# davidea97/Fisher-Nerf-customized

Hardware: AMD Instinct MI355X
Metric: candidate-views/sec (higher is better)
Workload: dtype f32

## Files before the change

### fisher-nerf-customized_amd/csrc/fisher_rast.hip

```cpp
#include <hip/hip_runtime.h>
#include <hip/hip_fp16.h>
#include <stdint.h>
#include <stdio.h>
#include <stdlib.h>
#include <string.h>
#include "fr_math.h"
#include "../../include/fisher_rast.h"
#include "fr_internal.h"

#define FR_THREADS 256
#define FR_G_MAX 32
#define FR_MAX_LDS_TILES 4096
#define FR_PART_MIN_DEFAULT 2048
#define FR_SORT_SMALL_KEYS 2048
#define FR_SORT_MID_KEYS 4096
#define FR_SORT_BIG_KEYS 16384
#define FR_VC_MAX 16
#define FR_BATCH 256
#define FR_BWD_BATCH 128

#include <vector>
#include <utility>
static thread_local char g_err[512] = "";
#if defined(FR_ABLATE) || defined(FR_LOOPSTATS)
// ... 374 lines not shown

__global__ __launch_bounds__(FR_THREADS) void k_tile_lists(const uint32_t* __restrict__ cnt, uint32_t* __restrict__ off, int N, int T, uint32_t tile_cap,
                                                           int* __restrict__ status, uint32_t* __restrict__ big_list,
                                                           uint32_t* __restrict__ view_work, uint32_t* __restrict__ view_perm, int ablate, uint32_t list_min)
{
	const int i0 = (blockIdx.x * FR_THREADS + threadIdx.x) * 4;
	__shared__ uint32_t s_vw[4 * FR_THREADS + 2];
	const int vfirst = (blockIdx.x * 4 * FR_THREADS) / T;
	const int ilast = min(N - 1, (int)(blockIdx.x * 4 * FR_THREADS) + 4 * FR_THREADS - 1);
	const int nvb = view_work ? ilast / T - vfirst + 1 : 0;
	for (int k = threadIdx.x; k < nvb; k += FR_THREADS) s_vw[k] = 0u;
	__syncthreads();
	uint32_t sum = 0, mx = 0;
#pragma unroll
	for (int q = 0; q < 4; q++)
	{
		const int i = i0 + q;
		if (i >= N) break;
		const uint32_t c = cnt[i];
		off[i] = (uint32_t)i * tile_cap;
		sum += c;
		mx = c > mx ? c : mx;
		if (c > list_min) big_list[16 + atomicAdd(&big_list[0], 1u)] = (uint32_t)i;
		if (view_work && c) atomicAdd(&s_vw[i / T - vfirst], c);
	}
	__syncthreads();
	for (int k = threadIdx.x; k < nvb; k += FR_THREADS) if (s_vw[k]) atomicAdd(&view_work[vfirst + k], s_vw[k]);
#pragma unroll
	for (int o = 32; o > 0; o >>= 1)
	{
		sum += (uint32_t)__shfl_xor((int)sum, o, 64);
		const uint32_t t = (uint32_t)__shfl_xor((int)mx, o, 64);
		mx = t > mx ? t : mx;
	}
	if ((threadIdx.x & 63) == 0)
	{
		if (sum) atomicAdd(&status[0], (int)sum);
		if (mx) atomicMax(&status[2], (int)mx);
		if (mx > tile_cap) { atomicOr(&status[1], 1); atomicOr(&status[3], 1); }
		FR_ABL(if (ablate >= 30) atomicOr(&status[1], 1);)
	}
	if (view_perm)
	{
		__shared__ bool s_last;
		__threadfence();
		__syncthreads();
		if (threadIdx.x == 0) s_last = atomicAdd(&big_list[1], 1u) == gridDim.x - 1;
		__syncthreads();
		if (s_last)
		{
			__threadfence();
			fr_deal_views((const uint32_t*)view_work, view_perm, N / T, threadIdx.x, FR_THREADS);
		}
	}
}

__global__ __launch_bounds__(FR_THREADS) void k_scatter_keys(FrParams p)
{
	extern __shared__ uint32_t fr_dyn_lds[];
	uint32_t* s_cnt = fr_dyn_lds;
	uint32_t* s_base = fr_dyn_lds + p.T;
	if (p.status[1]) return;
	const int tid = threadIdx.x;
	const int v = blockIdx.y;
	const size_t vP = (size_t)v * p.P;
	const uint32_t* off = p.tile_off + (size_t)v * p.T;
	uint32_t* fill = p.tile_fill + (size_t)v * p.T;
	const bool lds = p.T <= FR_MAX_LDS_TILES;
	if (lds && p.blk_base)
	{
		const uint32_t* bb = p.blk_base + ((size_t)v * gridDim.x + blockIdx.x) * p.T;
		for (int t = tid; t < p.T; t += FR_THREADS) { s_cnt[t] = 0; s_base[t] = off[t] + bb[t]; }
		__syncthreads();
	}
	else if (lds)
	{
		for (int t = tid; t < p.T; t += FR_THREADS) s_cnt[t] = 0;
		__syncthreads();
		for (int g = 0; g < p.G; g++)
		{
			const int i = (blockIdx.x * p.G + g) * FR_THREADS + tid;
			if (i >= p.P) break;
			const int rad = p.radii[vP + i];
			if (rad > 0)
			{
				const float2 xy = *(const float2*)(p.splat + vP + i);
				const fr_rect rc = fr_get_rect(xy.x, xy.y, rad, p.gx, p.gy);
				for (uint32_t y = rc.y0; y < rc.y1; y++)
					for (uint32_t x = rc.x0; x < rc.x1; x++)
						atomicAdd(&s_cnt[y * p.gx + x], 1u);
			}
		}
		__syncthreads();
		for (int t = tid; t < p.T; t += FR_THREADS)
		{
			const uint32_t c = s_cnt[t];
			if (c) s_base[t] = off[t] + atomicAdd(&fill[t], c);
			s_cnt[t] = 0;
		}
		__syncthreads();
	}
	constexpr int NB = 8;
	for (int g0 = 0; g0 < p.G; g0 += NB)
	{
		int rad[NB];
		float4 q0[NB];
		float dep[NB];
#pragma unroll
		for (int b = 0; b < NB; b++)
		{
			const int i = (blockIdx.x * p.G + g0 + b) * FR_THREADS + tid;
			rad[b] = (g0 + b < p.G && i < p.P) ? p.radii[vP + i] : 0;
		}
#pragma unroll
		for (int b = 0; b < NB; b++)
		{
			const int i = (blockIdx.x * p.G + g0 + b) * FR_THREADS + tid;
			if (rad[b] > 0)
			{
				const float4* sp = (const float4*)(p.splat + vP + i);
				q0[b] = sp[0];
				dep[b] = sp[1].z;
			}
		}
#pragma unroll
		for (int b = 0; b < NB; b++)
		{
			if (rad[b] > 0)
			{
				const int i = (blockIdx.x * p.G + g0 + b) * FR_THREADS + tid;
				const uint64_t hi = ((uint64_t)fr_as_u32(dep[b])) << 32;
				const fr_rect rc = fr_get_rect(q0[b].x, q0[b].y, rad[b], p.gx, p.gy);
				for (uint32_t y = rc.y0; y < rc.y1; y++)
					for (uint32_t x = rc.x0; x < rc.x1; x++)
					{
						const uint32_t t = y * p.gx + x;
						const uint32_t slot = lds ? (s_base[t] + atomicAdd(&s_cnt[t], 1u)) : (off[t] + atomicAdd(&fill[t], 1u));
						p.keys[slot] = hi | (uint32_t)i;
					}
			}
		}
	}
}

struct FrRecordArgs {
	const float* H_inv; long long hinv_stride; const float* packed; float4* recq;
	const float4* mt;
	const float4* grp;
	int early;
	float4* comp;
	uint32_t* slot_idx;
	int stride;
	float* slot_acc;
};
template <int C> struct FrPackSize { static constexpr int value = (C >= 11) ? 32 : 16; };
template <int C, bool REWRITE, bool FORM_A = false, bool FIVE = false, bool IDV = false>
__device__ __forceinline__ void fr_fisher_record_one(const FrParams& p, const float* __restrict__ H_inv, long long hinv_stride,
                                                     const float* __restrict__ packed, float4* __restrict__ recq, int v, uint32_t id,
                                                     const float* vm, const float* pm, const float* wm, bool has_w2c,
                                                     float4* out6 = nullptr, const float4* ab_src = nullptr);
template <int C, int AF, bool DK = false> struct FrRecStride { static constexpr int value = AF == 4 ? 3 : AF >= 2 ? (C >= 11 ? 13 : 7) : ((AF == 0 && DK) ? 5 : 6); };
template <int C, bool POSE = false>
__device__ __forceinline__ void fr_fisher_record_general(const FrParams& p, const float* __restrict__ packed, int v, uint32_t id,
                                                         const float* vm, const float* pm, const float* wm, bool has_w2c,
                                                         float4* out, const float4* ab_src);

template <int RC, bool PHASE_C>
__global__ __launch_bounds__(FR_THREADS) void k_preprocess_views(FrParams p, FrRecordArgs ra)
{
	extern __shared__ uint32_t fr_dyn_lds[];
	const int VC = p.VC;
	uint32_t* hist = fr_dyn_lds;
	uint32_t* pairs = hist + (size_t)VC * p.T;
	float* s_wm = (float*)(pairs + FR_THREADS * VC);
	const int W32 = 8 * p.G;
	uint32_t* s_bm = (uint32_t*)(s_wm + 12 * VC);
	uint32_t* s_pf = s_bm + VC * W32;
	const bool compact = RC != 0 && ra.comp != nullptr;
	__shared__ uint32_t s_np;
	__shared__ uint32_t s_n[FR_VC_MAX];
	__shared__ uint32_t s_ref[FR_VC_MAX];
	const int tid = threadIdx.x, lane = tid & 63;
	const int v0 = blockIdx.y * VC;
	const int nv = min(VC, p.V - v0);
	const uint32_t nblk = gridDim.x;
	const uint32_t cap = (uint32_t)(FR_THREADS * p.G);
	for (int t = tid; t < nv * p.T; t += FR_THREADS) hist[t] = 0;
	const bool has_w2c = p.w2c != nullptr;
	if (has_w2c) for (int t = tid; t < nv * 12; t += FR_THREADS) s_wm[t] = p.w2c[16 * (size_t)(v0 + t / 12) + (t % 12)];
	if (tid < FR_VC_MAX) { s_n[tid] = 0; s_ref[tid] = 0; }
	if (tid == 0) s_np = 0;
	if (compact) for (int t = tid; t < nv * W32; t += FR_THREADS) s_bm[t] = 0u;
	float vm[16], pm[16];
#pragma unroll
	for (int k = 0; k < 16; k++) { vm[k] = p.view[k]; pm[k] = p.proj[k]; }
	__syncthreads();
	for (int g = 0; g < p.G; g++)
	{
		const int i0 = (blockIdx.x * p.G + g) * FR_THREADS;
		if (i0 >= p.P) break;
		{
			const int i = i0 + tid;
			const bool live = i < p.P;
			fr_f3 pw = { 0.f, 0.f, 0.f };
			if (live) pw = fr_f3{ p.means3D[3 * (size_t)i], p.means3D[3 * (size_t)i + 1], p.means3D[3 * (size_t)i + 2] };
			const bool early = RC != 0 && ra.early != 0 && ra.mt != nullptr;
			float tr = 0.f;
			if (early && live) tr = ra.mt[i].w;
			const float lx = 1.3f * p.tanfovx, ly = 1.3f * p.tanfovy;
			float wn;
			{
				const float c0 = fabsf(vm[0]) + fabsf(vm[1]) + fabsf(vm[2]), c1 = fabsf(vm[4]) + fabsf(vm[5]) + fabsf(vm[6]), c2 = fabsf(vm[8]) + fabsf(vm[9]) + fabsf(vm[10]);
				const float r0 = fabsf(vm[0]) + fabsf(vm[4]) + fabsf(vm[8]), r1 = fabsf(vm[1]) + fabsf(vm[5]) + fabsf(vm[9]), r2 = fabsf(vm[2]) + fabsf(vm[6]) + fabsf(vm[10]);
				wn = fmaxf(c0, fmaxf(c1, c2)) * fmaxf(r0, fmaxf(r1, r2));
			}
			const float fx2 = 1.02f * wn * p.focal_x * p.focal_x, fy2 = 1.02f * wn * p.focal_y * p.focal_y;
			const float xmax = (float)(p.gx * FR_BLOCK_X + FR_BLOCK_X), ymax = (float)(p.gy * FR_BLOCK_Y + FR_BLOCK_Y);
			for (int vv = 0; vv < nv; vv++)
			{
				const fr_f3 po = has_w2c ? fr_world_to_cam(pw, s_wm + 12 * vv) : pw;
				const fr_f3 p_view = fr_xform4x3(po, vm);
				bool keep = live && !(p_view.z <= 0.001f);
				if (early)
				{
					const fr_f4 ph = fr_xform4x4(po, pm);
					const float p_w = 1.0f / (ph.w + 0.0000001f);
					const float px = ((ph.x * p_w + 1.0f) * (float)p.W - 1.0f) * 0.5f, py = ((ph.y * p_w + 1.0f) * (float)p.H - 1.0f) * 0.5f;
					const float iz = 1.0f / p_view.z;
					const float jx = fminf(fabsf(p_view.x * iz) * 1.001f, lx), jy = fminf(fabsf(p_view.y * iz) * 1.001f, ly);
					const float kc = fx2 * (1.0f + jx * jx) + fy2 * (1.0f + jy * jy);
					const float rb = 3.0f * sqrtf(kc * tr * (iz * iz) + 0.7f) + 2.0f;
					const bool outside = (px + rb < 0.f) || (px - rb > xmax) || (py + rb < 0.f) || (py - rb > ymax);
					keep = keep && !outside;
				}
				const unsigned long long m = __ballot(keep);
				if (m)
				{
					uint32_t base = 0;
					if (lane == 0) base = atomicAdd(&s_np, (uint32_t)__popcll(m));
					base = __builtin_amdgcn_readfirstlane(base);
					if (keep) pairs[base + __popcll(m & ((1ull << lane) - 1ull))] = (uint32_t)tid | ((uint32_t)vv << 8);
				}
			}
		}
		__syncthreads();
		const uint32_t np = s_np;
		for (uint32_t e = tid; e < np; e += FR_THREADS)
		{
			const uint32_t pr = pairs[e];
			const int i = i0 + (int)(pr & 255u);
			const int vv = (int)(pr >> 8);
			const int v = v0 + vv;
			fr_f3 pw;
			float c3[6];
			float cg = 0.f;
			if constexpr (RC != 0)
			{
				constexpr int PSB = FrPackSize<(RC < 0 ? -RC : RC)>::value;
				const float4* pk = (const float4*)(ra.packed + (size_t)i * PSB);
				const float4 t0 = pk[0], t1 = pk[1], t2 = pk[2];
				pw = fr_f3{ t0.x, t0.y, t0.z };
				c3[0] = t0.w; c3[1] = t1.x; c3[2] = t1.y; c3[3] = t1.z; c3[4] = t1.w; c3[5] = t2.x;
				cg = t2.y + t2.z + t2.w;
			}
			else
			{
				pw = fr_f3{ p.means3D[3 * (size_t)i], p.means3D[3 * (size_t)i + 1], p.means3D[3 * (size_t)i + 2] };
#pragma unroll
				for (int k = 0; k < 6; k++) c3[k] = p.cov3D[6 * (size_t)i + k];
			}
			float wm[12];
			if (has_w2c)
			{
#pragma unroll
				for (int k = 0; k < 12; k++) wm[k] = s_wm[12 * vv + k];
			}
			const fr_f3 po = has_w2c ? fr_world_to_cam(pw, wm) : pw;
			const fr_splat s = fr_preprocess_one(po, c3, vm, pm, p.W, p.H, p.tanfovx, p.tanfovy, p.focal_x, p.focal_y, p.gx, p.gy);
			if (s.radius > 0)
			{
				const float o = p.opac[i];
				const uint32_t ext = fr_alpha_extent(s.conx, s.cony, s.conz, o);
				const uint32_t slot = atomicAdd(&s_n[vv], 1u);
				float4* dst = (float4*)(p.splat + (size_t)v * p.P + i);
				if (compact)
				{
					dst = (float4*)(p.splat + ((size_t)v * nblk + blockIdx.x) * cap + slot);
					const uint32_t local = (uint32_t)(i - (int)(blockIdx.x * cap));
					atomicOr(&s_bm[vv * W32 + (int)(local >> 5)], 1u << (local & 31u));
				}
				if constexpr (RC != 0)
				{
					dst[0] = make_float4(s.px, s.py, __uint_as_float(ext), __builtin_amdgcn_logf(o));
					dst[1] = make_float4(-0.5f * s.conx, -s.cony, -0.5f * s.conz, cg);
				}
				else
				{
					dst[0] = make_float4(s.px, s.py, s.conx, s.cony);
					dst[1] = make_float4(s.conz, o, s.depth, __uint_as_float(ext));
				}
				uint32_t rx0 = s.rect.x0, rx1 = s.rect.x1, ry0 = s.rect.y0, ry1 = s.rect.y1;
				atomicAdd(&s_ref[vv], (rx1 - rx0) * (ry1 - ry0));
				{
					const float hx = __half2float(__ushort_as_half((unsigned short)(ext & 0xffffu)));
					const float hy = __half2float(__ushort_as_half((unsigned short)(ext >> 16)));
					if (hx < 0.f) { rx1 = rx0; ry1 = ry0; }
					else if (hx < 1e30f)
					{
						const float inv = 1.0f / (float)FR_BLOCK_X;
						const int tx0 = (int)floorf((s.px - hx) * inv), tx1 = (int)floorf((s.px + hx) * inv) + 1;
						const int ty0 = (int)floorf((s.py - hy) * inv), ty1 = (int)floorf((s.py + hy) * inv) + 1;
						rx0 = (uint32_t)max((int)rx0, tx0); rx1 = (uint32_t)max((int)rx0, min((int)rx1, tx1));
						ry0 = (uint32_t)max((int)ry0, ty0); ry1 = (uint32_t)max((int)ry0, min((int)ry1, ty1));
					}
				}
				uint32_t* h = hist + (size_t)vv * p.T;
				for (uint32_t y = ry0; y < ry1; y++)
					for (uint32_t x = rx0; x < rx1; x++)
						atomicAdd(&h[y * p.gx + x], 1u);
				FrVisEntry en;
				en.idx = (uint32_t)i; en.depth_bits = fr_as_u32(s.depth);
				en.xy0 = rx0 | (ry0 << 16); en.xy1 = rx1 | (ry1 << 16);
				*(uint4*)(p.vis_list + ((size_t)v * nblk + blockIdx.x) * cap + slot) = *(const uint4*)&en;
			}
		}
		__syncthreads();
		if (tid == 0) s_np = 0;
		__syncthreads();
	}
	for (int vv = 0; vv < nv; vv++)
	{
		const int v = v0 + vv;
		uint32_t* cnt = p.tile_cnt + (size_t)v * p.T;
		const uint32_t* h = hist + (size_t)vv * p.T;
		for (int t = tid; t < p.T; t += FR_THREADS)
		{
			const uint32_t c = h[t];
			if (c) p.blk_base[((size_t)v * nblk + blockIdx.x) * p.T + t] = atomicAdd(&cnt[t], c);
		}
	}
	if (tid < nv)
	{
		const int v = v0 + tid;
		p.vis_n[(size_t)v * nblk + blockIdx.x] = s_n[tid];
		if (p.vis_count && s_n[tid]) atomicAdd(&p.vis_count[v], (int)s_n[tid]);
		if (p.num_rendered && s_ref[tid]) atomicAdd(&p.num_rendered[v], (int)s_ref[tid]);
	}
	if constexpr (RC != 0 && PHASE_C)
	{
		__syncthreads();
		if (compact)
		{
			for (int t = tid; t < nv * W32; t += FR_THREADS)
			{
				const int vv = t / W32, w = t - vv * W32;
				uint32_t acc = 0;
				for (int u = 0; u < w; u++) acc += (uint32_t)__popc(s_bm[vv * W32 + u]);
				s_pf[t] = acc;
			}
			__syncthreads();
		}
		const size_t PV = (size_t)nblk * cap;
		for (int vv = 0; vv < nv; vv++)
		{
			const int v = v0 + vv;
			const uint32_t n = s_n[vv];
			FrVisEntry* list = p.vis_list + ((size_t)v * nblk + blockIdx.x) * cap;
			float wm[12];
#pragma unroll
			for (int k = 0; k < 12; k++) wm[k] = has_w2c ? s_wm[12 * vv + k] : 0.f;
			for (uint32_t e = tid; e < n; e += FR_THREADS)
			{
				const uint32_t idx = list[e].idx;
				if (compact)
				{
					const uint32_t local = idx - blockIdx.x * cap;
					const uint32_t rank = s_pf[vv * W32 + (int)(local >> 5)] + (uint32_t)__popc(s_bm[vv * W32 + (int)(local >> 5)] & ((1u << (local & 31u)) - 1u));
					const uint32_t slot = blockIdx.x * cap + rank;
					const float4* tmp = (const float4*)(p.splat + ((size_t)v * nblk + blockIdx.x) * cap + e);
					fr_fisher_record_one<(RC < 0 ? -RC : RC), false, (RC < 0)>(p, ra.H_inv, ra.hinv_stride, ra.packed, ra.recq, v, idx, vm, pm, wm, has_w2c,
					                                                           ra.comp + ((size_t)v * PV + slot) * 6, tmp);
					list[e].idx = slot;
					if constexpr (RC < 0) ra.slot_idx[(size_t)v * PV + slot] = idx;
				}
				else fr_fisher_record_one<(RC < 0 ? -RC : RC), false, (RC < 0)>(p, ra.H_inv, ra.hinv_stride, ra.packed, ra.recq, v, idx, vm, pm, wm, has_w2c);
			}
		}
	}
}

template <int C, int AF, bool DK, bool IDV = false, bool SLOTS = false>
__global__ __launch_bounds__(FR_THREADS) void k_preprocess_views_c(FrParams p, FrRecordArgs ra)
{
	static_assert(!SLOTS || (AF == 0 && !IDV), "the slot table is an option of the general score form (the out_H forms always write it)");
	static_assert((C == 4 || C == 11) && AF >= 0 && AF <= 4 && !((AF == 1 || AF >= 3) && C != 4), "records modes: score form, A-form (4 columns), general out_H form, pose form (4 columns), render form (4 columns)");
	static_assert(!IDV || (C == 4 && AF == 0 && DK), "the identity-view front end is the 4-column score form's with fixed key segments");
	constexpr int RS = FrRecStride<C, AF, DK>::value;
	extern __shared__ uint32_t fr_dyn_lds[];
	const int VC = p.VC;
	uint32_t* hist = fr_dyn_lds;
	uint32_t* pairs = hist + (size_t)VC * p.T;
	float* s_wm = (float*)(pairs + FR_THREADS * (VC + 1));
	uint32_t* park = (uint32_t*)(s_wm + 12 * VC);
	__shared__ uint32_t s_n[FR_VC_MAX];
	__shared__ uint32_t s_ref[FR_VC_MAX];
	__shared__ uint32_t s_ca[FR_VC_MAX * 4];
	__shared__ uint32_t s_wk2[2][FR_VC_MAX * 4];
	__shared__ uint32_t s_wtot2[2][4];
	uint32_t batch_no = 0;
	const int tid = threadIdx.x, lane = tid & 63;
	const int wave = __builtin_amdgcn_readfirstlane(tid >> 6);
	const int v0 = blockIdx.y * VC;
	const int nv = min(VC, p.V - v0);
	const uint32_t nblk = gridDim.x;
	const uint32_t cap = (uint32_t)(FR_THREADS * p.G);
	for (int t = tid; t < nv * p.T; t += FR_THREADS) hist[t] = 0;
	const bool has_w2c = p.w2c != nullptr;
	if (has_w2c) for (int t = tid; t < nv * 12; t += FR_THREADS) s_wm[t] = p.w2c[16 * (size_t)(v0 + t / 12) + (t % 12)];
	if (tid < FR_VC_MAX) { s_n[tid] = 0; s_ref[tid] = 0; }
	float vm[16], pm[16];
#pragma unroll
	for (int k = 0; k < 16; k++) { vm[k] = IDV ? (k % 5 == 0 ? 1.f : 0.f) : p.view[k]; pm[k] = p.proj[k]; }
	if constexpr (IDV)
	{
		bool id = true;
#pragma unroll
		for (int k = 0; k < 16; k++) id = id && p.view[k] == vm[k];
		if (!id && tid == 0) { atomicOr(&p.status[1], 1); atomicOr(&p.status[3], 2); }
	}
	const size_t PV = (size_t)nblk * cap;
	const unsigned long long lt = (1ull << lane) - 1ull;
	__syncthreads();
	const int iw = blockIdx.x * p.G * FR_THREADS;
	const bool early = ra.early != 0;
	const float lx = 1.3f * p.tanfovx, ly = 1.3f * p.tanfovy;
	float wn;
	{
		const float c0 = fabsf(vm[0]) + fabsf(vm[1]) + fabsf(vm[2]), c1 = fabsf(vm[4]) + fabsf(vm[5]) + fabsf(vm[6]), c2 = fabsf(vm[8]) + fabsf(vm[9]) + fabsf(vm[10]);
		const float r0 = fabsf(vm[0]) + fabsf(vm[4]) + fabsf(vm[8]), r1 = fabsf(vm[1]) + fabsf(vm[5]) + fabsf(vm[9]), r2 = fabsf(vm[2]) + fabsf(vm[6]) + fabsf(vm[10]);
		wn = fmaxf(c0, fmaxf(c1, c2)) * fmaxf(r0, fmaxf(r1, r2));
	}
	const float fx2 = 1.02f * wn * p.focal_x * p.focal_x, fy2 = 1.02f * wn * p.focal_y * p.focal_y;
	const float xmax = (float)(p.gx * FR_BLOCK_X + FR_BLOCK_X), ymax = (float)(p.gy * FR_BLOCK_Y + FR_BLOCK_Y);
	unsigned long long skipm = 0ull;
	if (early && ra.grp != nullptr && p.G * nv <= 64)
	{
		const float wrow = fabsf(pm[3] - vm[2]) + fabsf(pm[7] - vm[6]) + fabsf(pm[11] - vm[10]) + fabsf(pm[15] - vm[14]);
		const float wmag = fabsf(vm[2]) + fabsf(vm[6]) + fabsf(vm[10]) + fabsf(vm[14]);
		const bool pinhole = wrow <= 1e-6f * wmag;
		bool skip = false;
		const int g = lane / nv, vv = lane - g * nv;
		const int blk = blockIdx.x * p.G + g;
		if (pinhole && g < p.G && blk * FR_THREADS < p.P)
		{
#pragma clang fp contract(fast)
			const float4 b0 = ra.grp[2 * (size_t)blk], b1 = ra.grp[2 * (size_t)blk + 1];
			const fr_f3 cw = { 0.5f * (b0.x + b1.x), 0.5f * (b0.y + b1.y), 0.5f * (b0.z + b1.z) };
			const float ex = b1.x - cw.x, ey = b1.y - cw.y, ez = b1.z - cw.z;
			float R = 1.01f * __builtin_amdgcn_sqrtf(ex * ex + ey * ey + ez * ez) + 1e-6f;
			const fr_f3 c = has_w2c ? fr_world_to_cam(cw, s_wm + 12 * vv) : cw;
			if (has_w2c)
			{
				const float* m = s_wm + 12 * vv;
				const float g00 = m[0] * m[0] + m[4] * m[4] + m[8] * m[8], g11 = m[1] * m[1] + m[5] * m[5] + m[9] * m[9], g22 = m[2] * m[2] + m[6] * m[6] + m[10] * m[10];
				const float g01 = fabsf(m[0] * m[1] + m[4] * m[5] + m[8] * m[9]), g02 = fabsf(m[0] * m[2] + m[4] * m[6] + m[8] * m[10]), g12 = fabsf(m[1] * m[2] + m[5] * m[6] + m[9] * m[10]);
				R *= __builtin_amdgcn_sqrtf(fmaxf(g00 + g01 + g02, fmaxf(g01 + g11 + g12, g02 + g12 + g22))) * 1.00001f;
			}
			const float kcm = fx2 * (1.0f + lx * lx) + fy2 * (1.0f + ly * ly);
			const float a2 = 2.0f * 1.01f * 3.0f * __builtin_amdgcn_sqrtf(kcm * b0.w);
			const float c0 = 6.0f;
			const float Wf = (float)p.W, Hf = (float)p.H;
			const float zc = vm[2] * c.x + vm[6] * c.y + vm[10] * c.z + vm[14];
			const float zn = __builtin_amdgcn_sqrtf(vm[2] * vm[2] + vm[6] * vm[6] + vm[10] * vm[10]);
			auto side = [&](float sx, float sy, float sz, float sw, float kz, float add) -> bool {
				const float Ax = sx + kz * vm[2], Ay = sy + kz * vm[6], Az = sz + kz * vm[10];
				const float Lc = Ax * c.x + Ay * c.y + Az * c.z + (sw + kz * vm[14]) + add;
				return Lc + __builtin_amdgcn_sqrtf(Ax * Ax + Ay * Ay + Az * Az) * R < 0.f;
			};
			const bool left = side(Wf * pm[0], Wf * pm[4], Wf * pm[8], Wf * pm[12], Wf - 1.0f + 2.0f * c0, a2);
			const bool right = side(-Wf * pm[0], -Wf * pm[4], -Wf * pm[8], -Wf * pm[12], -(Wf - 1.0f - 2.0f * xmax - 2.0f * c0), a2);
			const bool top = side(Hf * pm[1], Hf * pm[5], Hf * pm[9], Hf * pm[13], Hf - 1.0f + 2.0f * c0, a2);
			const bool bottom = side(-Hf * pm[1], -Hf * pm[5], -Hf * pm[9], -Hf * pm[13], -(Hf - 1.0f - 2.0f * ymax - 2.0f * c0), a2);
			const bool behind = zc + zn * R <= 0.001f;
			skip = left || right || top || bottom || behind;
		}
		skipm = __builtin_amdgcn_ballot_w64(skip);
	}
	uint32_t pend = 0;
	for (int g = 0; g < p.G; g++)
	{
		const int i0 = iw + g * FR_THREADS;
		if (i0 >= p.P) break;
		const bool last_round = g == p.G - 1 || i0 + FR_THREADS >= p.P;
		uint32_t np = 0;
		const uint32_t skipv = (uint32_t)(skipm >> (g * nv)) & ((1u << nv) - 1u);
		if (skipv != (1u << nv) - 1u)
		{
			const int i = i0 + tid;
			const bool live = i < p.P;
			fr_f3 pw = { 0.f, 0.f, 0.f };
			float tr = 0.f;
			if (live) { const float4 m4 = ra.mt[i]; pw = fr_f3{ m4.x, m4.y, m4.z }; tr = m4.w; }
			uint32_t keepbits = 0;
			for (int vv = 0; vv < nv; vv++)
			{
				if ((skipv >> vv) & 1u) { if (lane == 0) s_ca[vv * 4 + wave] = 0u; continue; }
				const fr_f3 po = has_w2c ? fr_world_to_cam(pw, s_wm + 12 * vv) : pw;
				const fr_f3 p_view = IDV ? po : fr_xform4x3(po, vm);
				bool keep = live && !(p_view.z <= 0.001f);
				if (early)
				{
#pragma clang fp contract(fast)
					const float hx = __builtin_fmaf(pm[8], po.z, __builtin_fmaf(pm[4], po.y, __builtin_fmaf(pm[0], po.x, pm[12])));
					const float hy = __builtin_fmaf(pm[9], po.z, __builtin_fmaf(pm[5], po.y, __builtin_fmaf(pm[1], po.x, pm[13])));
					const float hw = __builtin_fmaf(pm[11], po.z, __builtin_fmaf(pm[7], po.y, __builtin_fmaf(pm[3], po.x, pm[15])));
					const float p_w = __builtin_amdgcn_rcpf(hw + 0.0000001f);
					const float px = ((hx * p_w + 1.0f) * (float)p.W - 1.0f) * 0.5f, py = ((hy * p_w + 1.0f) * (float)p.H - 1.0f) * 0.5f;
					const float iz = __builtin_amdgcn_rcpf(p_view.z);
					const float jx = fminf(fabsf(p_view.x * iz) * 1.001f, lx), jy = fminf(fabsf(p_view.y * iz) * 1.001f, ly);
					const float kc = fx2 * (1.0f + jx * jx) + fy2 * (1.0f + jy * jy);
					const float rb = 3.0f * __builtin_amdgcn_sqrtf(kc * tr * (iz * iz) + 0.7f) * 1.000001f + 2.0f;
					const bool outside = (px + rb < 0.f) || (px - rb > xmax) || (py + rb < 0.f) || (py - rb > ymax);
					keep = keep && !outside;
				}
				keepbits |= (keep ? 1u : 0u) << vv;
				const unsigned long long m = __builtin_amdgcn_ballot_w64(keep);
				if (lane == 0) s_ca[vv * 4 + wave] = (uint32_t)__popcll(m);
			}
			__syncthreads();
			uint32_t cnt_l = lane < 4 * nv ? s_ca[lane] : 0u;
			uint32_t inc = cnt_l;
#pragma unroll
			for (int d = 1; d < 64; d <<= 1)
			{
				const uint32_t y = (uint32_t)__shfl_up((int)inc, d, 64);
				if (lane >= d) inc += y;
			}
			const uint32_t exc = inc - cnt_l;
			np = (uint32_t)__builtin_amdgcn_readlane((int)inc, 63);
			for (int vv = 0; vv < nv; vv++)
			{
				const bool keep = (keepbits >> vv) & 1u;
				const unsigned long long m = __builtin_amdgcn_ballot_w64(keep);
				const uint32_t base = (uint32_t)__builtin_amdgcn_readlane((int)exc, vv * 4 + wave);
				if (keep) pairs[pend + base + (uint32_t)__popcll(m & lt)] = (uint32_t)(g * FR_THREADS + tid) | ((uint32_t)vv << 16);
			}
		}
		__syncthreads();
		FR_ABL(if (p.ablate == 35) np = 0;)
		pend += np;
		const uint32_t ndo = last_round ? pend : (pend & ~(uint32_t)(FR_THREADS - 1));
		for (uint32_t e0 = 0; e0 < ndo; e0 += FR_THREADS)
		{
			const uint32_t e = e0 + (uint32_t)tid;
			const bool active = e < ndo;
			int i = 0, vv = 0;
			fr_splat sp;
			sp.radius = 0;
			float o = 0.f, cg = 0.f;
			uint32_t ext = 0;
			if (active)
			{
					const uint32_t pr = pairs[e];
				i = iw + (int)(pr & 0xffffu);
				vv = (int)(pr >> 16);
				constexpr int PSB = FrPackSize<C>::value;
				const float4* pk = (const float4*)(ra.packed + (size_t)i * PSB);
				const float4 t0 = pk[0], t1 = pk[1], t2 = pk[2];
				const float o_pre = p.opac[p.order ? p.order[i] : (uint32_t)i];
				const fr_f3 pw = fr_f3{ t0.x, t0.y, t0.z };
				float c3[6];
				c3[0] = t0.w; c3[1] = t1.x; c3[2] = t1.y; c3[3] = t1.z; c3[4] = t1.w; c3[5] = t2.x;
				cg = t2.y + t2.z + t2.w;
				float wm[12];
				if (has_w2c)
				{
#pragma unroll
					for (int k = 0; k < 12; k++) wm[k] = s_wm[12 * vv + k];
				}
				const fr_f3 po = has_w2c ? fr_world_to_cam(pw, wm) : pw;
				sp = fr_preprocess_one<IDV>(po, c3, vm, pm, p.W, p.H, p.tanfovx, p.tanfovy, p.focal_x, p.focal_y, p.gx, p.gy);
				if (sp.radius > 0) { o = o_pre; ext = fr_alpha_extent(sp.conx, sp.cony, sp.conz, o); }
				if constexpr (AF == 4) cg = po.z;
			}
			const bool vis = sp.radius > 0;
			uint32_t* s_wk = s_wk2[batch_no & 1u];
			uint32_t* s_wtot = s_wtot2[batch_no & 1u];
			batch_no++;
			const unsigned long long mv = __builtin_amdgcn_ballot_w64(vis);
			if (lane == 0) s_wtot[wave] = (uint32_t)__popcll(mv);
			uint32_t below = 0;
			for (int k = 0; k < nv; k++)
			{
				const unsigned long long mk = __builtin_amdgcn_ballot_w64(vis && vv == k);
				if (lane == 0) s_wk[k * 4 + wave] = (uint32_t)__popcll(mk);
				if (vv == k) below = (uint32_t)__popcll(mk & lt);
			}
			__syncthreads();
			uint32_t rank = 0, pos = 0, nvis = 0;
			{
#pragma unroll
				for (int w = 0; w < 4; w++) { const uint32_t c = s_wtot[w]; nvis += c; pos += (w < wave) ? c : 0u; }
				pos += (uint32_t)__popcll(mv & lt);
			}
			if (vis)
			{
				rank = s_n[vv] + below;
				for (int w = 0; w < wave; w++) rank += s_wk[vv * 4 + w];
			}
			if (vis)
			{
				uint32_t rx0 = sp.rect.x0, rx1 = sp.rect.x1, ry0 = sp.rect.y0, ry1 = sp.rect.y1;
				atomicAdd(&s_ref[vv], (rx1 - rx0) * (ry1 - ry0));
				{
					const float hx = __half2float(__ushort_as_half((unsigned short)(ext & 0xffffu)));
					const float hy = __half2float(__ushort_as_half((unsigned short)(ext >> 16)));
					if (hx < 0.f) { rx1 = rx0; ry1 = ry0; }
					else if (hx < 1e30f)
					{
						const float inv = 1.0f / (float)FR_BLOCK_X;
						const int tx0 = (int)floorf((sp.px - hx) * inv), tx1 = (int)floorf((sp.px + hx) * inv) + 1;
						const int ty0 = (int)floorf((sp.py - hy) * inv), ty1 = (int)floorf((sp.py + hy) * inv) + 1;
						rx0 = (uint32_t)max((int)rx0, tx0); rx1 = (uint32_t)max((int)rx0, min((int)rx1, tx1));
						ry0 = (uint32_t)max((int)ry0, ty0); ry1 = (uint32_t)max((int)ry0, min((int)ry1, ty1));
					}
				}
				uint32_t* h = hist + (size_t)vv * p.T;
				if constexpr (DK)
				{
					const float hx = __half2float(__ushort_as_half((unsigned short)(ext & 0xffffu)));
					const float hy = __half2float(__ushort_as_half((unsigned short)(ext >> 16)));
					ry0 *= 4u; ry1 *= 4u;
					if (hx >= 0.f && hx < 1e30f && rx1 > rx0 && ry1 > ry0)
					{
						const int tx0 = (int)ceilf((sp.px - hx - 15.0f) * 0.0625f), sy0 = (int)ceilf((sp.py - hy - 3.0f) * 0.25f);
						const int sy1 = (int)floorf((sp.py + hy) * 0.25f) + 1;
						rx0 = (uint32_t)max((int)rx0, tx0); rx1 = max(rx0, rx1);
						ry0 = (uint32_t)max((int)ry0, sy0); ry1 = (uint32_t)max((int)ry0, min((int)ry1, sy1));
					}
					if (rx1 > rx0 && ry1 > ry0)
						for (uint32_t y = ry0 >> 2; y <= (ry1 - 1u) >> 2; y++)
							for (uint32_t x = rx0; x < rx1; x++)
								atomicAdd(&h[y * p.gx + x], 1u);
				}
				else
				for (uint32_t y = ry0; y < ry1; y++)
					for (uint32_t x = rx0; x < rx1; x++)
						atomicAdd(&h[y * p.gx + x], 1u);
				park[0 * FR_THREADS + pos] = __float_as_uint(sp.px);
				park[1 * FR_THREADS + pos] = __float_as_uint(sp.py);
				park[2 * FR_THREADS + pos] = ext;
				if constexpr (AF == 4)
				{
					park[3 * FR_THREADS + pos] = __float_as_uint(o);
					park[4 * FR_THREADS + pos] = __float_as_uint(sp.conx);
					park[5 * FR_THREADS + pos] = __float_as_uint(sp.cony);
					park[6 * FR_THREADS + pos] = __float_as_uint(sp.conz);
				}
				else
				{
					park[3 * FR_THREADS + pos] = __float_as_uint(__builtin_amdgcn_logf(o));
					park[4 * FR_THREADS + pos] = __float_as_uint(-0.5f * sp.conx);
					park[5 * FR_THREADS + pos] = __float_as_uint(-sp.cony);
					park[6 * FR_THREADS + pos] = __float_as_uint(-0.5f * sp.conz);
				}
				park[7 * FR_THREADS + pos] = __float_as_uint(cg);
				park[8 * FR_THREADS + pos] = (uint32_t)i;
				park[9 * FR_THREADS + pos] = fr_as_u32(sp.depth);
				park[10 * FR_THREADS + pos] = rx0 | (ry0 << 16);
				park[11 * FR_THREADS + pos] = rx1 | (ry1 << 16);
				park[12 * FR_THREADS + pos] = rank | ((uint32_t)vv << 16);
			}
			__syncthreads();
			if (tid < nv) s_n[tid] += (s_wk[tid * 4] + s_wk[tid * 4 + 1]) + (s_wk[tid * 4 + 2] + s_wk[tid * 4 + 3]);
			FR_ABL(if (p.ablate == 36) nvis = 0;)
			if ((uint32_t)tid < nvis)
			{
					const int r = tid;
				float4 ab[2];
				ab[0] = make_float4(__uint_as_float(park[0 * FR_THREADS + r]), __uint_as_float(park[1 * FR_THREADS + r]),
				                    __uint_as_float(park[2 * FR_THREADS + r]), __uint_as_float(park[3 * FR_THREADS + r]));
				ab[1] = make_float4(__uint_as_float(park[4 * FR_THREADS + r]), __uint_as_float(park[5 * FR_THREADS + r]),
				                    __uint_as_float(park[6 * FR_THREADS + r]), __uint_as_float(park[7 * FR_THREADS + r]));
				const uint32_t idx = park[8 * FR_THREADS + r];
				const uint32_t rk = park[12 * FR_THREADS + r];
				const int cvv = (int)(rk >> 16);
				const uint32_t slot = blockIdx.x * cap + (rk & 0xffffu);
				const int v = v0 + cvv;
				float wm[12];
#pragma unroll
				for (int k = 0; k < 12; k++) wm[k] = has_w2c ? s_wm[12 * cvv + k] : 0.f;
				float4* rec_out = ra.comp + ((size_t)v * PV + slot) * RS;
				FR_ABL(if (p.ablate == 37) rec_out = ra.comp + (size_t)tid * RS;)
				if constexpr (AF == 4)
				{
					const float4 t2 = ((const float4*)(ra.packed + (size_t)idx * FrPackSize<C>::value))[2];
					rec_out[0] = ab[0];
					rec_out[1] = make_float4(ab[1].x, ab[1].y, ab[1].z, __uint_as_float(park[9 * FR_THREADS + r]));
// ... 5214 lines not shown
	out[0] = L.geom_bytes; out[1] = L.bin_bytes; out[2] = L.img_bytes;
	return FR_OK;
}

extern "C" int fr_workspace_layout(int32_t P, int32_t W, int32_t H, int64_t max_rendered, size_t o[11])
{
	if (P < 0 || W <= 0 || H <= 0 || max_rendered < 0 || !o) return fr_fail(FR_EINVAL, "fr_workspace_layout: bad argument");
	FrLayout L = fr_layout(P, W, H, 1, max_rendered);
	o[0] = L.splat; o[1] = L.cov3D; o[2] = L.rgb; o[3] = L.clamped;
	o[4] = L.tile_cnt; o[5] = L.tile_off; o[6] = L.tile_fill; o[7] = L.final_T; o[8] = L.n_contrib; o[9] = L.status;
	o[10] = L.keys;
	return FR_OK;
}

extern "C" int fr_mark_visible(int32_t P, const float* means3D, const float* viewmatrix, const float* projmatrix,
                               uint8_t* present, fr_stream_t stream)
{
	(void)projmatrix;
	if (P < 0) return fr_fail(FR_EINVAL, "fr_mark_visible: P < 0");
	if (P == 0) return FR_OK;
	if (!means3D || !viewmatrix || !present) return fr_fail(FR_EINVAL, "fr_mark_visible: null pointer");
	hipLaunchKernelGGL(k_mark_visible, dim3((P + FR_THREADS - 1) / FR_THREADS), dim3(FR_THREADS), 0, (hipStream_t)stream,
	                   P, means3D, viewmatrix, present);
	return fr_check_launch("k_mark_visible");
}

static int fr_validate(const fr_raster_cfg* cfg, const fr_gaussians* g, const char* who, bool need_opacity = true)
{
	static thread_local char buf[256];
	if (!cfg || !g) { snprintf(buf, sizeof(buf), "%s: null cfg/gaussians", who); return fr_fail(FR_EINVAL, buf); }
	if (cfg->P < 0 || cfg->image_width <= 0 || cfg->image_height <= 0) { snprintf(buf, sizeof(buf), "%s: bad P/W/H", who); return fr_fail(FR_EINVAL, buf); }
	if (cfg->P == 0) return FR_OK;
	if (!g->means3D || (need_opacity && !g->opacities) || !cfg->bg || !cfg->viewmatrix || !cfg->projmatrix)
	{ snprintf(buf, sizeof(buf), "%s: null means3D/opacities/bg/viewmatrix/projmatrix", who); return fr_fail(FR_EINVAL, buf); }
	if ((g->colors_precomp == nullptr) == (g->shs == nullptr))
	{ snprintf(buf, sizeof(buf), "%s: provide exactly one of SHs or precomputed colors", who); return fr_fail(FR_EINVAL, buf); }
	if (g->shs && (!cfg->campos || cfg->sh_coeffs <= 0 || (cfg->sh_degree + 1) * (cfg->sh_degree + 1) > cfg->sh_coeffs || cfg->sh_degree > 3 || cfg->sh_degree < 0))
	{ snprintf(buf, sizeof(buf), "%s: bad SH degree / coefficient count / campos", who); return fr_fail(FR_EINVAL, buf); }
	const bool sr = g->scales && g->rotations;
	if ((sr ? 1 : 0) + (g->cov3D_precomp ? 1 : 0) != 1 || ((g->scales != nullptr) != (g->rotations != nullptr)))
	{ snprintf(buf, sizeof(buf), "%s: provide exactly one of scale/rotation pair or precomputed 3D covariance", who); return fr_fail(FR_EINVAL, buf); }
	return FR_OK;
}

static void fr_fill_params(FrParams& p, const fr_raster_cfg* cfg, const fr_gaussians* g, int V)
{
	memset(&p, 0, sizeof(p));
	p.P = cfg->P; p.V = V; p.W = cfg->image_width; p.H = cfg->image_height;
	p.gx = (uint32_t)((p.W + 15) / 16); p.gy = (uint32_t)((p.H + 15) / 16); p.T = (int)(p.gx * p.gy);
	p.tanfovx = cfg->tanfovx; p.tanfovy = cfg->tanfovy;
	p.focal_y = p.H / (2.0f * cfg->tanfovy);
	p.focal_x = p.W / (2.0f * cfg->tanfovx);
	p.mod = cfg->scale_modifier; p.D = cfg->sh_degree; p.M = cfg->sh_coeffs;
	p.prefiltered = cfg->prefiltered;
	p.bg = cfg->bg; p.view = cfg->viewmatrix; p.proj = cfg->projmatrix; p.campos = cfg->campos;
	p.means3D = g->means3D; p.colors = g->colors_precomp; p.shs = g->shs; p.opac = g->opacities;
	p.scales = g->scales; p.rots = g->rotations;
	p.VC = 1;
	p.small_max = FR_SORT_SMALL_KEYS;
	p.order = nullptr;
	p.legacy_sort = fr_debug_mode() == 6;
	FR_ABL(p.ablate = fr_debug_mode();)
}

#define FR_ZERO_MAX 12
struct FrZeroList { uint32_t* ptr[FR_ZERO_MAX]; unsigned long long end[FR_ZERO_MAX]; unsigned long long dwords[FR_ZERO_MAX]; int n; };
__global__ __launch_bounds__(FR_THREADS) void k_zero_many(FrZeroList z)
{
	const unsigned long long total = z.end[z.n - 1];
	for (unsigned long long i = (unsigned long long)blockIdx.x * FR_THREADS + threadIdx.x; i < total; i += (unsigned long long)gridDim.x * FR_THREADS)
	{
		int b = 0;
		while (i >= z.end[b]) b++;
		const unsigned long long u = i - (b ? z.end[b - 1] : 0ull);
		uint32_t* q = z.ptr[b] + 4 * u;
		if (4 * u + 4 <= z.dwords[b] && ((uintptr_t)q & 15u) == 0) *(uint4*)q = make_uint4(0u, 0u, 0u, 0u);
		else
			for (unsigned long long k = 4 * u; k < 4 * u + 4 && k < z.dwords[b]; k++) z.ptr[b][k] = 0u;
	}
}
struct FrZeroer {
	FrZeroList z; unsigned long long run = 0;
	FrZeroer() { z.n = 0; }
	void add(void* p, size_t bytes) { if (!p || bytes == 0) return; z.ptr[z.n] = (uint32_t*)p; z.dwords[z.n] = bytes / 4; run += (bytes / 4 + 3) / 4; z.end[z.n] = run; z.n++; }
	void launch(hipStream_t s)
	{
		if (z.n == 0) return;
		const unsigned long long blocks = (run + FR_THREADS * 4 - 1) / (FR_THREADS * 4);
		hipLaunchKernelGGL(k_zero_many, dim3((unsigned)(blocks > 4096 ? 4096 : (blocks < 1 ? 1 : blocks))), dim3(FR_THREADS), 0, s, z);
	}
};

struct FrSideStream {
	hipStream_t stream = nullptr; hipEvent_t fork = nullptr, join = nullptr; bool ok = false; int device = -1;
};
static FrSideStream& fr_side_stream(int which = 0)
{
	static thread_local FrSideStream sides[3];
	FrSideStream& ss = sides[which];
	int dev = -1;
	(void)hipGetDevice(&dev);
	if (ss.device != dev)
	{
		if (ss.ok) { (void)hipEventDestroy(ss.fork); (void)hipEventDestroy(ss.join); (void)hipStreamDestroy(ss.stream); }
#ifdef FR_AB
		static const int tile_prio = fr_env_int("FR_TILE_PRIO");
#else
		constexpr int tile_prio = 0;
#endif
		int lo = 0, hi = 0;
		(void)hipDeviceGetStreamPriorityRange(&lo, &hi);
		const int prio = (which == 2 && tile_prio > 0) ? lo : (which == 2 && tile_prio < 0) ? hi : 0;
		ss.ok = hipStreamCreateWithPriority(&ss.stream, hipStreamNonBlocking, prio) == hipSuccess
		     && hipEventCreateWithFlags(&ss.fork, hipEventDisableTiming) == hipSuccess
		     && hipEventCreateWithFlags(&ss.join, hipEventDisableTiming) == hipSuccess;
		ss.device = dev;
		(void)hipGetLastError();
	}
	return ss;
}

static int fr_cu_count()
{
	static thread_local int cus = 0, device = -1;
	int dev = -1;
	(void)hipGetDevice(&dev);
	if (device != dev || cus <= 0)
	{
		if (hipDeviceGetAttribute(&cus, hipDeviceAttributeMultiprocessorCount, dev) != hipSuccess || cus <= 0) cus = 256;
		device = dev;
		(void)hipGetLastError();
	}
	return cus;
}

struct FrJoinGuard {
	hipStream_t s; FrSideStream* side[2] = { nullptr, nullptr }; int n = 0;
	explicit FrJoinGuard(hipStream_t caller) : s(caller) {}
	void forked(FrSideStream* ss) { side[n++] = ss; }
	int join()
	{
		int rc = FR_OK;
		for (int i = 0; i < n; i++)
		{
			if (hipEventRecord(side[i]->join, side[i]->stream) != hipSuccess || hipStreamWaitEvent(s, side[i]->join, 0) != hipSuccess)
				rc = fr_fail(FR_ELAUNCH, "side stream join failed");
		}
		n = 0;
		return rc;
	}
	~FrJoinGuard() { if (n) { char keep[sizeof(g_err)]; memcpy(keep, g_err, sizeof(keep)); (void)join(); memcpy(g_err, keep, sizeof(keep)); } }
};

struct FrScorerPlan { int columns; bool form_a; FrRecordArgs ra; bool skip_pack = false; bool general = false; bool pose = false; bool view_identity = false; bool render = false; bool point = false; };
template <int C> __global__ void k_pack_static(FrParams p, const float* __restrict__ H_inv, float* __restrict__ packed, float4* __restrict__ mt, float4* __restrict__ grp);
template <int C, bool LIST, bool FORM_A> __global__ void k_fisher_records(FrParams p, FrRecordArgs ra);

static int fr_bin_pipeline(FrParams& p, const fr_gaussians* g, hipStream_t s, const FrScorerPlan* plan = nullptr)
{
	int rc;
	const int P = p.P;
	{
		FrZeroer z;
		z.add(p.tile_cnt, (size_t)p.V * p.T * 4); z.add(p.status, 16); z.add(p.big_list, 64);
		if (p.part_list) z.add(p.part_list, 4);
		if (p.view_work) z.add(p.view_work, (size_t)p.V * 4);
		if (p.vis_count) z.add(p.vis_count, (size_t)p.V * 4);
		if (p.num_rendered && p.vis_list != nullptr && p.T <= FR_MAX_LDS_TILES) z.add(p.num_rendered, (size_t)p.V * 4);
		z.launch(s);
	}
	const bool multi = p.vis_list != nullptr && p.T <= FR_MAX_LDS_TILES;
	if (g->cov3D_precomp) p.cov3D = g->cov3D_precomp;
	else if (plan && multi) p.cov3D = nullptr;
	else
	{
		hipLaunchKernelGGL(k_cov3d, dim3((P + FR_THREADS - 1) / FR_THREADS), dim3(FR_THREADS), 0, s, P, g->scales, p.mod, g->rotations, p.cov3D_out);
		if ((rc = fr_check_launch("k_cov3d"))) return rc;
		p.cov3D = p.cov3D_out;
	}
	p.G = multi ? fr_pick_G_views(P) : fr_pick_G(P, p.V);
	p.VC = fr_pick_VC(p.T);
	const int per_block = FR_THREADS * p.G;
	dim3 gridP((P + per_block - 1) / per_block, p.V);
	const size_t hist_lds = p.T <= FR_MAX_LDS_TILES ? (size_t)p.T * 4 : 16;
	if (plan && !plan->skip_pack)
	{
		const float* shared_hinv = plan->ra.hinv_stride ? nullptr : plan->ra.H_inv;
		dim3 gp((P + FR_THREADS - 1) / FR_THREADS);
		if (plan->columns == 4) hipLaunchKernelGGL((k_pack_static<4>), gp, dim3(FR_THREADS), 0, s, p, shared_hinv, (float*)plan->ra.packed, (float4*)plan->ra.mt, (float4*)plan->ra.grp);
		else hipLaunchKernelGGL((k_pack_static<11>), gp, dim3(FR_THREADS), 0, s, p, shared_hinv, (float*)plan->ra.packed, (float4*)plan->ra.mt, (float4*)plan->ra.grp);
		if ((rc = fr_check_launch("k_pack_static"))) return rc;
	}
	FrJoinGuard joins(s);
	if (multi)
	{
		const bool once = plan && plan->ra.comp != nullptr && fr_debug_mode() != 20;
		if (!once) p.tile_cap = 0;
		const bool wanted_fixed = p.tile_cap != 0;
		if (once) p.VC = fr_plan_views_c(p.T, p.VC, p.tile_cap);
		if (once && wanted_fixed && !p.tile_cap) return fr_fail(FR_EINVAL, "fr_bin_pipeline: fixed key segments planned, but they do not fit the LDS");
		auto lds_c_of = [&](int vc) { return fr_lds_views_c(vc, p.T, p.tile_cap != 0); };
		dim3 gridV(gridP.x, (p.V + p.VC - 1) / p.VC);
		const size_t lds = ((size_t)p.VC * p.T + (size_t)FR_THREADS * p.VC + 12 * (size_t)p.VC + 2 * (size_t)p.VC * 8 * (size_t)p.G) * 4;
		FrRecordArgs ra = plan ? plan->ra : FrRecordArgs{ nullptr, 0, nullptr, nullptr, nullptr, nullptr, 0, nullptr, nullptr, 6 };
		const bool dk = p.tile_cap != 0;
		const size_t lds_c = lds_c_of(p.VC);
		if (once && plan->render && dk) hipLaunchKernelGGL((k_preprocess_views_c<4, 4, true>), gridV, dim3(FR_THREADS), lds_c, s, p, ra);
		else if (once && plan->render) hipLaunchKernelGGL((k_preprocess_views_c<4, 4, false>), gridV, dim3(FR_THREADS), lds_c, s, p, ra);
		else if (once && plan->pose && dk) hipLaunchKernelGGL((k_preprocess_views_c<4, 3, true>), gridV, dim3(FR_THREADS), lds_c, s, p, ra);
		else if (once && plan->pose) hipLaunchKernelGGL((k_preprocess_views_c<4, 3, false>), gridV, dim3(FR_THREADS), lds_c, s, p, ra);
		else if (once && plan->general && plan->columns == 4 && dk) hipLaunchKernelGGL((k_preprocess_views_c<4, 2, true>), gridV, dim3(FR_THREADS), lds_c, s, p, ra);
		else if (once && plan->general && plan->columns == 4) hipLaunchKernelGGL((k_preprocess_views_c<4, 2, false>), gridV, dim3(FR_THREADS), lds_c, s, p, ra);
		else if (once && plan->general && dk) hipLaunchKernelGGL((k_preprocess_views_c<11, 2, true>), gridV, dim3(FR_THREADS), lds_c, s, p, ra);
		else if (once && plan->general) hipLaunchKernelGGL((k_preprocess_views_c<11, 2, false>), gridV, dim3(FR_THREADS), lds_c, s, p, ra);
		else if (once && plan->form_a && dk) hipLaunchKernelGGL((k_preprocess_views_c<4, 1, true>), gridV, dim3(FR_THREADS), lds_c, s, p, ra);
		else if (once && plan->form_a) hipLaunchKernelGGL((k_preprocess_views_c<4, 1, false>), gridV, dim3(FR_THREADS), lds_c, s, p, ra);
		else if (once && plan->point && plan->columns == 4 && dk) hipLaunchKernelGGL((k_preprocess_views_c<4, 0, true, false, true>), gridV, dim3(FR_THREADS), lds_c, s, p, ra);
		else if (once && plan->point && plan->columns == 4) hipLaunchKernelGGL((k_preprocess_views_c<4, 0, false, false, true>), gridV, dim3(FR_THREADS), lds_c, s, p, ra);
		else if (once && plan->point && dk) hipLaunchKernelGGL((k_preprocess_views_c<11, 0, true, false, true>), gridV, dim3(FR_THREADS), lds_c, s, p, ra);
		else if (once && plan->point) hipLaunchKernelGGL((k_preprocess_views_c<11, 0, false, false, true>), gridV, dim3(FR_THREADS), lds_c, s, p, ra);
		else if (once && plan->columns == 4 && dk && plan->view_identity) hipLaunchKernelGGL((k_preprocess_views_c<4, 0, true, true>), gridV, dim3(FR_THREADS), lds_c, s, p, ra);
		else if (once && plan->columns == 4 && dk) hipLaunchKernelGGL((k_preprocess_views_c<4, 0, true>), gridV, dim3(FR_THREADS), lds_c, s, p, ra);
		else if (once && plan->columns == 4) hipLaunchKernelGGL((k_preprocess_views_c<4, 0, false>), gridV, dim3(FR_THREADS), lds_c, s, p, ra);
		else if (once && dk) hipLaunchKernelGGL((k_preprocess_views_c<11, 0, true>), gridV, dim3(FR_THREADS), lds_c, s, p, ra);
		else if (once) hipLaunchKernelGGL((k_preprocess_views_c<11, 0, false>), gridV, dim3(FR_THREADS), lds_c, s, p, ra);
		else if (!plan) hipLaunchKernelGGL((k_preprocess_views<0, false>), gridV, dim3(FR_THREADS), lds, s, p, ra);
#ifdef FR_AB
		else if (plan->form_a) hipLaunchKernelGGL((k_preprocess_views<-4, true>), gridV, dim3(FR_THREADS), lds, s, p, ra);
		else if (plan->columns == 4) hipLaunchKernelGGL((k_preprocess_views<4, true>), gridV, dim3(FR_THREADS), lds, s, p, ra);
		else hipLaunchKernelGGL((k_preprocess_views<11, true>), gridV, dim3(FR_THREADS), lds, s, p, ra);
#else
		else return fr_fail(FR_EINVAL, "fr_bin_pipeline: a records plan of the multi-view front end needs compact records");
#endif
		if ((rc = fr_check_launch("k_preprocess_views"))) return rc;
	}
	else
	{
		p.tile_cap = 0;
		hipLaunchKernelGGL(k_preprocess, gridP, dim3(FR_THREADS), hist_lds, s, p);
		if ((rc = fr_check_launch("k_preprocess"))) return rc;
	}
	if (multi && p.tile_cap >= 2u * (uint32_t)FR_SORT_SMALL_KEYS + 128u && fr_debug_mode() != 32)
	{
		p.small_max = (uint32_t)FR_PART_MIN_DEFAULT;
		FR_AB_ONLY({ const int e = fr_env_int("FR_PART_MIN"); if (e >= 512 && e <= FR_SORT_SMALL_KEYS) p.small_max = (uint32_t)e; })
	}
	if (multi && p.tile_cap)
		hipLaunchKernelGGL(k_tile_lists, dim3((p.V * p.T + 4 * FR_THREADS - 1) / (4 * FR_THREADS)), dim3(FR_THREADS), 0, s, p.tile_cnt, p.tile_off, p.V * p.T, p.T,
		                   p.tile_cap, p.status, p.big_list, p.view_work, p.view_perm, p.ablate, p.small_max);
	else
	hipLaunchKernelGGL(k_scan_tiles, dim3(1), dim3(1024), 0, s, p.tile_cnt, p.tile_off, p.tile_fill, p.V * p.T, p.T, p.V,
	                   p.key_capacity, p.status, multi ? (int*)nullptr : p.num_rendered, p.big_list, p.view_work, p.view_perm);
	if ((rc = fr_check_launch("k_scan_tiles"))) return rc;
	if (multi && p.tile_cap) {  }
	else if (multi) hipLaunchKernelGGL(k_scatter_vis, gridP, dim3(FR_THREADS), 2 * hist_lds, s, p);
	else hipLaunchKernelGGL(k_scatter_keys, gridP, dim3(FR_THREADS), 2 * hist_lds, s, p);
	if ((rc = fr_check_launch("k_scatter_keys"))) return rc;
	if (plan && !multi)
	{
		FrSideStream& s2 = fr_side_stream(1);
		const bool forked2 = s2.ok && hipEventRecord(s2.fork, s) == hipSuccess && hipStreamWaitEvent(s2.stream, s2.fork, 0) == hipSuccess;
		hipStream_t rs = forked2 ? s2.stream : s;
		if (plan->form_a) hipLaunchKernelGGL((k_fisher_records<4, false, true>), gridP, dim3(FR_THREADS), 0, rs, p, plan->ra);
		else if (plan->columns == 4) hipLaunchKernelGGL((k_fisher_records<4, false, false>), gridP, dim3(FR_THREADS), 0, rs, p, plan->ra);
		else hipLaunchKernelGGL((k_fisher_records<11, false, false>), gridP, dim3(FR_THREADS), 0, rs, p, plan->ra);
		if (forked2) joins.forked(&s2);
		if ((rc = fr_check_launch("k_fisher_records"))) return rc;
	}
	FrSideStream& side = fr_side_stream();
	const bool part_all = p.tile_cap >= 32768u && fr_debug_mode() != 32;
	const bool want_fork = fr_debug_mode() != 7 && (!multi || p.V >= 8) && !part_all;
	const bool forked = want_fork && side.ok && hipEventRecord(side.fork, s) == hipSuccess && hipStreamWaitEvent(side.stream, side.fork, 0) == hipSuccess;
	const int big_blocks = p.T * p.V < 256 ? p.T * p.V : 256;
	if (forked) joins.forked(&side);
	uint32_t part_max = 0;
	if (p.part_list && p.tile_cap >= 2u * (uint32_t)FR_SORT_SMALL_KEYS + 128u && fr_debug_mode() != 32)
	{
		part_max = p.tile_cap / 2u - 64u;
		if (part_max > 16320u) part_max = 16320u;
	}
	hipLaunchKernelGGL(k_sort_big_tiles, dim3(big_blocks), dim3(1024), 0, forked ? side.stream : s, p, part_max);
	if ((rc = fr_check_launch("k_sort_big_tiles"))) return rc;
	const int mid_blocks = p.T * p.V < 2048 ? p.T * p.V : 2048;
	if (part_max)
	{
		uint32_t split_blocks = (4u * (uint32_t)fr_cu_count()) & ~7u;
		if (split_blocks < 8u) split_blocks = 8u;
		if (split_blocks > (uint32_t)(p.T * p.V)) split_blocks = (uint32_t)(p.T * p.V);
		FR_AB_ONLY({ const int e = fr_env_int("FR_SPLIT_BLOCKS"); if (e >= 8 && e <= 8192) split_blocks = (uint32_t)e & ~7u; })
		hipLaunchKernelGGL(k_sort_split, dim3(split_blocks + (uint32_t)(p.T * p.V)), dim3(FR_THREADS), 0, s, p, part_max, split_blocks);
		if ((rc = fr_check_launch("k_sort_split"))) return rc;
		uint32_t part_blocks = 8u * (uint32_t)fr_cu_count();
		FR_AB_ONLY({ const int e = fr_env_int("FR_PART_BLOCKS"); if (e >= 1 && e <= 65536) part_blocks = (uint32_t)e; })
		hipLaunchKernelGGL(k_sort_parts, dim3(part_blocks), dim3(FR_THREADS), 0, s, p);
		if ((rc = fr_check_launch("k_sort_parts"))) return rc;
	}
	else
	{
		hipLaunchKernelGGL(k_sort_tiles, dim3(p.T * p.V), dim3(FR_THREADS), 0, s, p);
		if ((rc = fr_check_launch("k_sort_tiles"))) return rc;
	}
	if (part_max < (uint32_t)FR_SORT_MID_KEYS)
	{
		hipLaunchKernelGGL(k_sort_mid_tiles, dim3(mid_blocks), dim3(FR_THREADS), 0, s, p, part_max);
		if ((rc = fr_check_launch("k_sort_mid_tiles"))) return rc;
	}
	return joins.join();
}

static void fr_carve_single(FrParams& p, const FrLayout& L, char* geom, char* bin, char* img)
{
	p.splat = (FrSplat*)(geom + L.splat);
	p.cov3D_out = (float*)(geom + L.cov3D);
	p.rgb = (float*)(geom + L.rgb);
	p.clamped = (uint8_t*)(geom + L.clamped);
	p.tile_cnt = (uint32_t*)(img + L.tile_cnt);
	p.tile_off = (uint32_t*)(img + L.tile_off);
	p.tile_fill = (uint32_t*)(img + L.tile_fill);
	p.status = (int*)(img + L.status);
	p.big_list = (uint32_t*)(img + L.big_list);
	p.blk_base = p.T <= FR_MAX_LDS_TILES ? (uint32_t*)(img + L.blk_base) : nullptr;
	p.keys = (uint64_t*)(bin + L.keys);
}

static int fr_forward_impl(const fr_raster_cfg* cfg, const fr_gaussians* g, const float* features2,
                           void* geom_ws, void* binning_ws, int64_t binning_capacity, void* image_ws,
                           float* out_color, float* out_features2, float* out_depth, int32_t* radii, int32_t* status, fr_stream_t stream)
{
	int rc = fr_validate(cfg, g, "fr_forward");
	if (rc) return rc;
	hipStream_t s = (hipStream_t)stream;
	const int P = cfg->P, W = cfg->image_width, H = cfg->image_height;
	if (!out_color || !out_depth || !status) return fr_fail(FR_EINVAL, "fr_forward: null output");
	if (P == 0)
	{
		(void)hipMemsetAsync(out_color, 0, (size_t)3 * W * H * 4, s);
		if (out_features2) (void)hipMemsetAsync(out_features2, 0, (size_t)3 * W * H * 4, s);
		(void)hipMemsetAsync(out_depth, 0, (size_t)W * H * 4, s);
		(void)hipMemsetAsync(status, 0, 16, s);
		return FR_OK;
	}
	if (!geom_ws || !binning_ws || !image_ws || !radii || binning_capacity < 0) return fr_fail(FR_EINVAL, "fr_forward: null workspace / radii");
	FrLayout L = fr_layout(P, W, H, 1, binning_capacity);
	FrParams p;
	fr_fill_params(p, cfg, g, 1);
	fr_carve_single(p, L, (char*)geom_ws, (char*)binning_ws, (char*)image_ws);
	p.radii = radii;
	p.key_capacity = binning_capacity;
	if ((rc = fr_bin_pipeline(p, g, s))) return rc;
	const float* feat = g->colors_precomp ? g->colors_precomp : p.rgb;
	FR_AB_ONLY(const bool bcast = fr_debug_mode() == 16;)
	float* fT = (float*)((char*)image_ws + L.final_T);
	uint32_t* nC = (uint32_t*)((char*)image_ws + L.n_contrib);
#ifdef FR_AB
	if (bcast && features2) hipLaunchKernelGGL((k_render_forward<6>), dim3(p.T, 1), dim3(FR_THREADS), 0, s, p, feat, 0, fT, nC, out_color, out_depth, features2, out_features2);
	else if (bcast) hipLaunchKernelGGL((k_render_forward<3>), dim3(p.T, 1), dim3(FR_THREADS), 0, s, p, feat, 0, fT, nC, out_color, out_depth, (const float*)nullptr, (float*)nullptr);
	else
#endif
	if (features2) hipLaunchKernelGGL((k_render_forward_walk<6>), dim3(p.T, 1), dim3(FR_THREADS), 0, s, p, feat, 0, fT, nC, out_color, out_depth, features2, out_features2);
// ... 216 lines not shown
	if (sr && sh) hipLaunchKernelGGL((k_backward_tile<true, true>), grid, block, 0, s, p, b);
	else if (sr) hipLaunchKernelGGL((k_backward_tile<true, false>), grid, block, 0, s, p, b);
	else if (sh) hipLaunchKernelGGL((k_backward_tile<false, true>), grid, block, 0, s, p, b);
	else hipLaunchKernelGGL((k_backward_tile<false, false>), grid, block, 0, s, p, b);
	if ((rc = fr_check_launch("k_backward_tile"))) return rc;
	if (sh)
	{
		hipLaunchKernelGGL(k_finish_sh, dim3((P + FR_THREADS - 1) / FR_THREADS), block, 0, s, p, (const float*)dL_dcolors, (int)power, dL_dsh);
		if ((rc = fr_check_launch("k_finish_sh"))) return rc;
	}
	return FR_OK;
}

extern "C" int fr_forward_features(const fr_raster_cfg* cfg, const float* features,
                                   const void* geom_ws, const void* binning_ws, void* image_ws,
                                   float* out_features, fr_stream_t stream)
{
	if (!cfg || cfg->P < 0 || cfg->image_width <= 0 || cfg->image_height <= 0) return fr_fail(FR_EINVAL, "fr_forward_features: bad cfg");
	hipStream_t s = (hipStream_t)stream;
	const int P = cfg->P, W = cfg->image_width, H = cfg->image_height;
	if (!out_features) return fr_fail(FR_EINVAL, "fr_forward_features: null output");
	if (P == 0)
	{
		(void)hipMemsetAsync(out_features, 0, (size_t)3 * W * H * 4, s);
		return FR_OK;
	}
	if (!features || !geom_ws || !binning_ws || !image_ws || !cfg->bg) return fr_fail(FR_EINVAL, "fr_forward_features: null pointer");
	FrLayout L = fr_layout(P, W, H, 1, 1);
	fr_gaussians g0;
	memset(&g0, 0, sizeof(g0));
	FrParams p;
	fr_fill_params(p, cfg, &g0, 1);
	fr_carve_single(p, L, (char*)geom_ws, (char*)binning_ws, (char*)image_ws);
#ifdef FR_AB
	if (fr_debug_mode() == 16)
		hipLaunchKernelGGL((k_render_forward<3>), dim3(p.T, 1), dim3(FR_THREADS), 0, s, p, features, 0,
		                   (float*)((char*)image_ws + L.final_T), (uint32_t*)((char*)image_ws + L.n_contrib), out_features, (float*)nullptr,
		                   (const float*)nullptr, (float*)nullptr);
	else
#endif
		hipLaunchKernelGGL((k_render_forward_walk<3>), dim3(p.T, 1), dim3(FR_THREADS), 0, s, p, features, 0,
		                   (float*)((char*)image_ws + L.final_T), (uint32_t*)((char*)image_ws + L.n_contrib), out_features, (float*)nullptr,
		                   (const float*)nullptr, (float*)nullptr);
	return fr_check_launch("k_render_forward(features)");
}

extern "C" int fr_backward_pair(const fr_raster_cfg* cfg, const fr_gaussians* g, const int32_t* radii,
                                const void* geom_ws, const void* binning_ws, const void* image_ws,
                                const float* dL_dout_color, const float* features, const float* dL_dout_features,
                                float* dL_dmeans2D, float* dL_dmeans2D_features, float* dL_dcolors, float* dL_dfeatures,
                                float* dL_dopacity, float* dL_dmeans3D, float* dL_dcov3D, float* dL_dscales,
                                float* dL_drotations, float* dL_dconic, fr_stream_t stream)
{
	return fr_backward_pair_ws(cfg, g, radii, geom_ws, binning_ws, image_ws, dL_dout_color, features, dL_dout_features, dL_dmeans2D,
	                           dL_dmeans2D_features, dL_dcolors, dL_dfeatures, dL_dopacity, dL_dmeans3D, dL_dcov3D, dL_dscales, dL_drotations,
	                           dL_dconic, 0, nullptr, 0, stream);
}

extern "C" int fr_backward_pair_ws(const fr_raster_cfg* cfg, const fr_gaussians* g, const int32_t* radii,
                                   const void* geom_ws, const void* binning_ws, const void* image_ws,
                                   const float* dL_dout_color, const float* features, const float* dL_dout_features,
                                   float* dL_dmeans2D, float* dL_dmeans2D_features, float* dL_dcolors, float* dL_dfeatures,
                                   float* dL_dopacity, float* dL_dmeans3D, float* dL_dcov3D, float* dL_dscales,
                                   float* dL_drotations, float* dL_dconic,
                                   int64_t num_rendered, void* scratch, size_t scratch_bytes, fr_stream_t stream)
{
	int rc = fr_validate(cfg, g, "fr_backward_pair", false);
	if (rc) return rc;
	hipStream_t s = (hipStream_t)stream;
	const int P = cfg->P, W = cfg->image_width, H = cfg->image_height;
	if (P == 0) return FR_OK;
	if (!g->colors_precomp || g->shs) return fr_fail(FR_EINVAL, "fr_backward_pair: needs colors_precomp (no SH)");
	if (!geom_ws || !binning_ws || !image_ws || !radii || !dL_dout_color || !features || !dL_dout_features || !dL_dmeans2D ||
	    !dL_dmeans2D_features || !dL_dcolors || !dL_dfeatures || !dL_dopacity || !dL_dmeans3D || !dL_dcov3D || !dL_dscales ||
	    !dL_drotations || !dL_dconic)
		return fr_fail(FR_EINVAL, "fr_backward_pair: null pointer");
	const int64_t T_img = ((int64_t)(W + 15) / 16) * ((int64_t)(H + 15) / 16);
	const size_t scratch_need = fr_backward_pair_scratch_bytes(P, W, H, num_rendered);
	const bool chunked = scratch && scratch_need > 0 && scratch_bytes >= scratch_need FR_AB_ONLY(&& fr_debug_mode() != 33 && fr_debug_mode() != 18);
	const FrSqScratch sq = fr_sq_scratch(T_img, chunked ? num_rendered : 1, 6);
	{
		FrZeroer z;
		z.add(dL_dmeans2D, (size_t)P * 3 * 4); z.add(dL_dmeans2D_features, (size_t)P * 3 * 4); z.add(dL_dcolors, (size_t)P * 3 * 4);
		z.add(dL_dfeatures, (size_t)P * 3 * 4); z.add(dL_dopacity, (size_t)P * 4); z.add(dL_dmeans3D, (size_t)P * 3 * 4);
		z.add(dL_dcov3D, (size_t)P * 6 * 4); z.add(dL_dscales, (size_t)P * 3 * 4); z.add(dL_drotations, (size_t)P * 4 * 4);
		z.add(dL_dconic, (size_t)P * 4 * 4);
		if (chunked) z.add((char*)scratch + sq.slot_map, sq.cnt - sq.slot_map);
		z.launch(s);
	}
	FrLayout L = fr_layout(P, W, H, 1, 1);
	FrParams p;
	fr_fill_params(p, cfg, g, 1);
	fr_carve_single(p, L, (char*)geom_ws, (char*)binning_ws, (char*)image_ws);
	p.radii = (int*)radii;
	p.cov3D = g->cov3D_precomp ? g->cov3D_precomp : p.cov3D_out;
	const bool sr = g->scales != nullptr;
	dim3 grid(p.T, 1), block(FR_THREADS);
	uint8_t* fallback = (uint8_t*)p.tile_fill;
	FrBwdArgs b;
	b.final_T = (const float*)((const char*)image_ws + L.final_T);
	b.n_contrib = (const uint32_t*)((const char*)image_ws + L.n_contrib);
	b.power = 1;
	b.dL_dconic = dL_dconic; b.dL_dopacity = dL_dopacity;
	b.dL_dmean3D = dL_dmeans3D; b.dL_dcov3D = dL_dcov3D; b.dL_dscale = dL_dscales; b.dL_drot = dL_drotations;
	b.dL_dmean2D_b = nullptr;
	b.dL_dpix = dL_dout_color; b.colors = g->colors_precomp; b.dL_dmean2D = dL_dmeans2D; b.dL_dcolors = dL_dcolors;
	b.dL_dpix2 = dL_dout_features; b.colors2 = features; b.dL_dmean2D_2 = dL_dmeans2D_features; b.dL_dcolors2 = dL_dfeatures;
	b.only_flagged = nullptr; b.u_only = 0;
	const bool pair_walk = fr_debug_mode() == 18 || chunked;
	if (chunked)
	{
		if ((rc = fr_launch_chunked<6>(p, b, sq, scratch, nullptr, s))) return rc;
	}
	else
#ifdef FR_AB
	if (pair_walk)
	{
		hipLaunchKernelGGL((k_backward_lin_walk<true>), dim3(p.T), block, 0, s, p, b);
		if ((rc = fr_check_launch("k_backward_lin_walk<pair>"))) return rc;
	}
	else
#endif
	hipLaunchKernelGGL((k_backward_lin_tile<true>), dim3(p.T), block, 0, s, p, b, fallback);
	if ((rc = fr_check_launch("k_backward_lin_tile<pair>"))) return rc;
	for (int pass = 0; pass < 2 && !pair_walk; pass++)
	{
		b.dL_dpix = pass ? dL_dout_features : dL_dout_color;
		b.colors = pass ? features : g->colors_precomp;
		b.dL_dmean2D = pass ? dL_dmeans2D_features : dL_dmeans2D;
		b.dL_dcolors = pass ? dL_dfeatures : dL_dcolors;
		b.only_flagged = fallback; b.u_only = 1;
		if (sr) hipLaunchKernelGGL((k_backward_tile<true, false>), grid, block, 0, s, p, b);
		else hipLaunchKernelGGL((k_backward_tile<false, false>), grid, block, 0, s, p, b);
		if ((rc = fr_check_launch("k_backward_tile(flagged)"))) return rc;
	}
	b.dL_dmean2D = dL_dmeans2D; b.dL_dmean2D_b = dL_dmeans2D_features;
	b.dL_dcolors = dL_dcolors; b.colors = g->colors_precomp;
	dim3 gp((P + FR_THREADS - 1) / FR_THREADS);
	if (sr) hipLaunchKernelGGL((k_backward_finish<true, false>), gp, block, 0, s, p, b, (float*)nullptr);
	else hipLaunchKernelGGL((k_backward_finish<false, false>), gp, block, 0, s, p, b, (float*)nullptr);
	return fr_check_launch("k_backward_finish");
}

#ifdef FR_AB
static int fr_debug_mode()
{
	static const int mode = fr_env_int("FR_DEBUG_MODE");
	return mode;
}
#endif

#define FR_MAX_GROUPS 4
struct FrFisherLayout {
	size_t radii, vis_n, splat, recq, slot_idx, packed, mt, grp, big_list, part_list, view_work, view_perm, blk_base, cov3D, tile_cnt, tile_off, tile_fill, tile_scores, w2c_inv, status, keys, fallback, seg_T, seg_C, seg_X, seg_list, total;
	size_t PV;
};
static FrFisherLayout fr_fisher_layout(int64_t P, int64_t W, int64_t H, int64_t V, int64_t max_rendered, int columns)
{
	FrFisherLayout L;
	const int64_t T = ((W + 15) / 16) * ((H + 15) / 16);
	size_t o = 0;
	const size_t nblk_v = (size_t)((P + FR_THREADS * fr_pick_G_views(P) - 1) / (FR_THREADS * fr_pick_G_views(P)));
	L.radii = o; o = fr_align(o + (size_t)V * nblk_v * (size_t)(FR_THREADS * fr_pick_G_views(P)) * sizeof(FrVisEntry));
	L.vis_n = o; o = fr_align(o + (size_t)V * nblk_v * 4);
	L.PV = nblk_v * (size_t)(FR_THREADS * fr_pick_G_views(P));
	const size_t VPV = (size_t)V * (L.PV > (size_t)P ? L.PV : (size_t)P);
	L.splat = o; o = fr_align(o + VPV * sizeof(FrSplat));
	L.recq = o; o = fr_align(o + VPV * (columns == 11 ? 208 : 112));
	L.slot_idx = o; o = fr_align(o + VPV * 4);
	L.packed = o; o = fr_align(o + (size_t)P * 4 * (size_t)(columns == 11 ? 32 : 16));
	L.mt = o; o = fr_align(o + (size_t)P * 16);
	L.grp = o; o = fr_align(o + (size_t)((P + FR_THREADS - 1) / FR_THREADS) * 32);
	L.big_list = o; o = fr_align(o + (size_t)(V * T) * 4 + 64 * FR_MAX_GROUPS);
	L.view_work = o; o = fr_align(o + (size_t)V * 4);
	L.view_perm = o; o = fr_align(o + (size_t)V * 4);
	L.blk_base = o; o = fr_align(o + (size_t)V * (size_t)fr_preprocess_blocks(P, V) * (size_t)T * 4);
	L.cov3D = o; o = fr_align(o + (size_t)P * 24);
	L.tile_cnt = o; o = fr_align(o + (size_t)(V * T) * 4);
	L.tile_off = o; o = fr_align(o + (size_t)(V * T) * 4);
	L.tile_fill = o; o = fr_align(o + (size_t)(V * T) * 4);
	L.tile_scores = o; o = fr_align(o + (size_t)(V * T) * 4);
	L.w2c_inv = o; o = fr_align(o + (size_t)V * 64);
	L.status = o; o = fr_align(o + 64);
	const size_t R = (size_t)(max_rendered > 0 ? max_rendered : 1);
	L.keys = o; o = fr_align(o + R * 8);
	L.fallback = o; o = fr_align(o + (size_t)(V * T));
	const size_t seg_tiles = (size_t)(V * T <= FR_SEG_TILES ? V * T : 0);
	L.seg_T = o; o = fr_align(o + FR_SEG_PER_TILE * seg_tiles * FR_THREADS * 4);
	L.seg_C = o; o = fr_align(o + FR_SEG_PER_TILE * seg_tiles * FR_THREADS * 8);
	L.seg_X = o; o = fr_align(o + seg_tiles * FR_THREADS * 8);
	L.seg_list = o; o = fr_align(o + (FR_SEG_PER_TILE * seg_tiles + 1) * 4);
	L.part_list = o; o = fr_align(o + (size_t)(V * T) * FR_PART_MAXP * 8 + 64 * FR_MAX_GROUPS);
	L.total = o;
	return L;
}

extern "C" int fr_fisher_workspace_layout(int32_t P, int32_t W, int32_t H, int32_t n_views, int64_t max_rendered, int32_t columns, size_t o[8])
{
	if (P < 0 || W <= 0 || H <= 0 || n_views <= 0 || max_rendered < 0 || (columns != 4 && columns != 11) || !o)
		return fr_fail(FR_EINVAL, "fr_fisher_workspace_layout: bad argument");
	const FrFisherLayout L = fr_fisher_layout(P, W, H, n_views, max_rendered, columns);
	o[0] = L.tile_cnt; o[1] = L.tile_off; o[2] = L.keys; o[3] = L.splat; o[4] = L.recq; o[5] = L.tile_scores; o[6] = L.status; o[7] = L.vis_n;
	return FR_OK;
}

extern "C" int fr_fisher_part_list_offset(int32_t P, int32_t W, int32_t H, int32_t n_views, int64_t max_rendered, int32_t columns, size_t* offset)
{
	if (P < 0 || W <= 0 || H <= 0 || n_views <= 0 || max_rendered < 0 || (columns != 4 && columns != 11) || !offset)
		return fr_fail(FR_EINVAL, "fr_fisher_part_list_offset: bad argument");
	*offset = fr_fisher_layout(P, W, H, n_views, max_rendered, columns).part_list;
	return FR_OK;
}

extern "C" int fr_init(void)
{
	if (!fr_side_stream(0).ok || !fr_side_stream(1).ok || !fr_side_stream(2).ok) return fr_fail(FR_ELAUNCH, "fr_init: could not create the side streams");
	return FR_OK;
}

extern "C" size_t fr_fisher_workspace_bytes(int32_t P, int32_t W, int32_t H, int32_t n_views, int64_t max_rendered, int32_t columns)
{
	if (P < 0 || W <= 0 || H <= 0 || n_views <= 0 || max_rendered < 0 || (columns != 4 && columns != 11)) return 0;
	return fr_fisher_layout(P, W, H, n_views, max_rendered, columns).total;
}

static void fr_launch_fisher_v3(FrParams& p, FrFisherArgs f, float4* recq, hipStream_t s)
{
	hipEvent_t ev0 = nullptr, ev1 = nullptr;
	if (g_prof_on)
	{
		(void)hipEventCreate(&ev0); (void)hipEventCreate(&ev1);
		(void)hipEventRecord(ev0, s);
	}
#ifdef FR_AB
	if (f.debug_mode == 8) hipLaunchKernelGGL((k_fisher_tile_v3<8, 8>), dim3(p.T * p.V), dim3(FR_THREADS), 0, s, p, f, (const float4*)recq);
	else if (f.debug_mode == 24) hipLaunchKernelGGL(k_fisher_tile_v3w, dim3(p.T * p.V), dim3(FR_THREADS), 0, s, p, f);
	else if (f.key_shift && f.debug_mode == 31) hipLaunchKernelGGL((k_fisher_tile_v3<16, 4, true>), dim3(p.T * p.V), dim3(FR_THREADS), 0, s, p, f, (const float4*)recq);
	else
#endif
	if (f.key_shift) hipLaunchKernelGGL(k_fisher_tile_v4, dim3(p.T * p.V), dim3(FR_THREADS), 0, s, p, f);
	else hipLaunchKernelGGL((k_fisher_tile_v3<16, 4>), dim3(p.T * p.V), dim3(FR_THREADS), 0, s, p, f, (const float4*)recq);
	if (g_prof_on)
	{
		(void)hipEventRecord(ev1, s);
		g_prof_events.push_back(std::make_pair(ev0, ev1));
	}
}

static void fr_launch_fisher_v3h(FrParams& p, FrFisherArgs f, float4* recq, FrSegArgs sg, hipStream_t s)
{
	hipEvent_t ev0 = nullptr, ev1 = nullptr;
	if (g_prof_on)
	{
		(void)hipEventCreate(&ev0); (void)hipEventCreate(&ev1);
		(void)hipEventRecord(ev0, s);
	}
	if (sg.snapT && p.T * p.V <= FR_SEG_TILES)
	{
		(void)hipMemsetAsync(sg.list, 0, 4, s);
		hipLaunchKernelGGL((k_fisher_tile_v3h<16, 4, 1>), dim3(p.T * p.V), dim3(FR_THREADS), 0, s, p, f, (const float4*)recq, sg);
		hipLaunchKernelGGL((k_fisher_tile_v3h<16, 4, 2>), dim3(FR_SEG_PER_TILE * p.T * p.V), dim3(FR_THREADS), 0, s, p, f, (const float4*)recq, sg);
	}
	else
	hipLaunchKernelGGL((k_fisher_tile_v3h<16, 4, 0>), dim3(p.T * p.V), dim3(FR_THREADS), 0, s, p, f, (const float4*)recq, sg);
	if (g_prof_on)
	{
		(void)hipEventRecord(ev1, s);
		g_prof_events.push_back(std::make_pair(ev0, ev1));
	}
}

static void fr_launch_fisher_v3g(FrParams& p, FrFisherArgs f, int columns, bool img, FrSegArgs sg, hipStream_t s)
{
	hipEvent_t ev0 = nullptr, ev1 = nullptr;
	if (g_prof_on)
	{
		(void)hipEventCreate(&ev0); (void)hipEventCreate(&ev1);
		(void)hipEventRecord(ev0, s);
	}
	dim3 grid(p.T * p.V), block(FR_THREADS);
	if (sg.snapT && p.T * p.V <= FR_SEG_TILES)
	{
		(void)hipMemsetAsync(sg.list, 0, 4, s);
		dim3 g2(FR_SEG_PER_TILE * p.T * p.V);
		if (columns == 11 && img) { hipLaunchKernelGGL((k_fisher_tile_v3g<11, true, 1>), grid, block, 0, s, p, f, sg); hipLaunchKernelGGL((k_fisher_tile_v3g<11, true, 2>), g2, block, 0, s, p, f, sg); }
		else if (columns == 11) { hipLaunchKernelGGL((k_fisher_tile_v3g<11, false, 1>), grid, block, 0, s, p, f, sg); hipLaunchKernelGGL((k_fisher_tile_v3g<11, false, 2>), g2, block, 0, s, p, f, sg); }
		else if (img) { hipLaunchKernelGGL((k_fisher_tile_v3g<4, true, 1>), grid, block, 0, s, p, f, sg); hipLaunchKernelGGL((k_fisher_tile_v3g<4, true, 2>), g2, block, 0, s, p, f, sg); }
		else { hipLaunchKernelGGL((k_fisher_tile_v3g<4, false, 1>), grid, block, 0, s, p, f, sg); hipLaunchKernelGGL((k_fisher_tile_v3g<4, false, 2>), g2, block, 0, s, p, f, sg); }
	}
	else if (columns == 11 && img) hipLaunchKernelGGL((k_fisher_tile_v3g<11, true, 0>), grid, block, 0, s, p, f, sg);
	else if (columns == 11) hipLaunchKernelGGL((k_fisher_tile_v3g<11, false, 0>), grid, block, 0, s, p, f, sg);
	else if (img) hipLaunchKernelGGL((k_fisher_tile_v3g<4, true, 0>), grid, block, 0, s, p, f, sg);
	else hipLaunchKernelGGL((k_fisher_tile_v3g<4, false, 0>), grid, block, 0, s, p, f, sg);
	if (g_prof_on)
	{
		(void)hipEventRecord(ev1, s);
		g_prof_events.push_back(std::make_pair(ev0, ev1));
	}
}

template <int C>
static void fr_launch_fisher(FrParams& p, FrFisherArgs f, float* packed, uint8_t* fallback, hipStream_t s)
{
	dim3 grid(p.T * p.V), block(FR_THREADS);
	const bool hi = f.H_inv != nullptr, ho = f.out_H != nullptr;
	const bool per_view = hi && f.hinv_stride != 0;
	f.only_flagged = nullptr;
	hipLaunchKernelGGL((k_pack_static<C>), dim3((p.P + FR_THREADS - 1) / FR_THREADS), block, 0, s, p, (hi && !per_view) ? f.H_inv : nullptr, packed, (float4*)nullptr, (float4*)nullptr);
	hipEvent_t ev0 = nullptr, ev1 = nullptr;
	if (g_prof_on)
	{
		(void)hipEventCreate(&ev0); (void)hipEventCreate(&ev1);
		(void)hipEventRecord(ev0, s);
	}
	if (hi && ho) hipLaunchKernelGGL((k_fisher_tile_v2<C, true, true>), grid, block, 0, s, p, f, (const float*)packed, fallback);
	else if (hi) hipLaunchKernelGGL((k_fisher_tile_v2<C, true, false>), grid, block, 0, s, p, f, (const float*)packed, fallback);
	else hipLaunchKernelGGL((k_fisher_tile_v2<C, false, true>), grid, block, 0, s, p, f, (const float*)packed, fallback);
	if (g_prof_on)
	{
		(void)hipEventRecord(ev1, s);
		g_prof_events.push_back(std::make_pair(ev0, ev1));
	}
	f.only_flagged = fallback;
	if (hi && ho) hipLaunchKernelGGL((k_fisher_tile<C, true, true>), grid, block, 0, s, p, f);
	else if (hi) hipLaunchKernelGGL((k_fisher_tile<C, true, false>), grid, block, 0, s, p, f);
	else hipLaunchKernelGGL((k_fisher_tile<C, false, true>), grid, block, 0, s, p, f);
}

extern "C" int fr_fisher_views(const fr_raster_cfg* cfg, const fr_gaussians* g, const fr_fisher_cfg* fc,
                               void* workspace, size_t workspace_bytes, int64_t max_rendered,
                               int32_t* status, fr_stream_t stream)
{
	int rc = fr_validate(cfg, g, "fr_fisher_views");
	if (rc) return rc;
	if (!fc || fc->n_views <= 0 || !fc->w2c || !status) return fr_fail(FR_EINVAL, "fr_fisher_views: bad fisher cfg");
	if (fc->columns != 4 && fc->columns != 11) return fr_fail(FR_EINVAL, "fr_fisher_views: columns must be 4 or 11");
	if (!g->colors_precomp) return fr_fail(FR_EINVAL, "fr_fisher_views: needs colors_precomp (the reference always passes rgb_colors)");
	if (fc->columns == 11 && !(g->scales && g->rotations)) return fr_fail(FR_EINVAL, "fr_fisher_views: columns=11 needs scales and rotations");
	if (fc->out_scores && !fc->H_inv) return fr_fail(FR_EINVAL, "fr_fisher_views: out_scores needs H_inv");
	if (!fc->H_inv && !fc->out_H) return fr_fail(FR_EINVAL, "fr_fisher_views: nothing to compute (no H_inv and no out_H)");
	if (fc->H_inv && !fc->out_scores) return fr_fail(FR_EINVAL, "fr_fisher_views: H_inv without out_scores");
	if (fc->dL_dpix_image && (fc->H_inv || !fc->out_H)) return fr_fail(FR_EINVAL, "fr_fisher_views: dL_dpix_image is for the out_H mode (no H_inv)");
	const int P = cfg->P, W = cfg->image_width, H = cfg->image_height, V = fc->n_views;
	hipStream_t s = (hipStream_t)stream;
	if (P == 0)
	{
		if (fc->out_scores) (void)hipMemsetAsync(fc->out_scores, 0, (size_t)V * 4, s);
		if (fc->out_vis_count) (void)hipMemsetAsync(fc->out_vis_count, 0, (size_t)V * 4, s);
		if (fc->out_num_rendered) (void)hipMemsetAsync(fc->out_num_rendered, 0, (size_t)V * 4, s);
		(void)hipMemsetAsync(status, 0, 16, s);
		return FR_OK;
	}
	FrFisherLayout L = fr_fisher_layout(P, W, H, V, max_rendered, fc->columns);
	if (!workspace || workspace_bytes < L.total) return fr_fail(FR_ENOSPACE, "fr_fisher_views: workspace smaller than fr_fisher_workspace_bytes()");
	char* ws = (char*)workspace;
	FrParams p;
	fr_fill_params(p, cfg, g, V);
	p.prefiltered = 0;
	p.w2c = fc->w2c;
	if (fc->poses_are_c2w)
	{
		float* inv = (float*)(ws + L.w2c_inv);
		hipLaunchKernelGGL(k_invert_poses, dim3((V + 63) / 64), dim3(64), 0, s, V, fc->w2c, inv);
		if ((rc = fr_check_launch("k_invert_poses"))) return rc;
		p.w2c = inv;
	}
	p.radii = (int*)(ws + L.radii);
	p.vis_list = (FrVisEntry*)(ws + L.radii);
	p.vis_n = (uint32_t*)(ws + L.vis_n);
	p.splat = (FrSplat*)(ws + L.splat);
	p.cov3D_out = (float*)(ws + L.cov3D);
	p.tile_cnt = (uint32_t*)(ws + L.tile_cnt);
	p.tile_off = (uint32_t*)(ws + L.tile_off);
	p.tile_fill = (uint32_t*)(ws + L.tile_fill);
	p.status = (int*)(ws + L.status);
	p.big_list = (uint32_t*)(ws + L.big_list);
	p.part_list = (uint32_t*)(ws + L.part_list);
	const bool deal = (V & 7) == 0 && V <= 1024 && fr_debug_mode() != 27;
	p.view_work = deal ? (uint32_t*)(ws + L.view_work) : nullptr;
	p.view_perm = deal ? (uint32_t*)(ws + L.view_perm) : nullptr;
	p.blk_base = (uint32_t*)(ws + L.blk_base);
	p.keys = (uint64_t*)(ws + L.keys);
	p.key_capacity = max_rendered;
	if (fc->tile_capacity < 0) return fr_fail(FR_EINVAL, "fr_fisher_views: negative tile_capacity");
	if (fc->tile_capacity > 0)
	{
		const long long need = (long long)V * p.T * (long long)fc->tile_capacity;
		if (need > max_rendered || need >= (1ll << 32)) return fr_fail(FR_EINVAL, "fr_fisher_views: n_views * tiles * tile_capacity exceeds max_rendered (or 2^32)");
		const long long nblk_c = (P + FR_THREADS * fr_pick_G_views(P) - 1) / (FR_THREADS * fr_pick_G_views(P));
		const bool slots_fit = nblk_c * FR_THREADS * fr_pick_G_views(P) < (1ll << 28);
		if (p.gx <= 255u && p.gy <= 63u && slots_fit && fr_debug_mode() != 8 && fr_debug_mode() != 24 && fr_debug_mode() != 20) p.tile_cap = (uint32_t)fc->tile_capacity;
	}
	p.vis_count = fc->out_vis_count;
	p.num_rendered = fc->out_num_rendered;
	FrFisherArgs f;
	f.dL = fc->dL_dpix;
	f.dL_img = fc->dL_dpix_image; f.dL_stride = fc->dL_image_view_stride;
	f.H_inv = fc->H_inv; f.hinv_stride = fc->H_inv_view_stride;
	f.out_H = fc->out_H; f.outH_stride = fc->out_H_view_stride;
	f.tile_scores = (float*)(ws + L.tile_scores);
	f.only_flagged = nullptr;
	f.debug_mode = fr_debug_mode();
	f.key_shift = 0;
	const bool v3 = fc->H_inv && !fc->out_H && !fc->dL_dpix_image && f.debug_mode != 1 && f.debug_mode != 9;
	const bool v3h = !fc->H_inv && fc->out_H && !fc->dL_dpix_image && fc->columns == 4 && f.debug_mode != 1 && f.debug_mode != 9;
	const bool multi_fe = p.vis_list != nullptr && p.T <= FR_MAX_LDS_TILES;
	const bool v3g = !fc->H_inv && fc->out_H && !v3h && multi_fe && !g->cov3D_precomp && f.debug_mode != 1 && f.debug_mode != 9 && f.debug_mode != 22 && f.debug_mode != 19;
	FrScorerPlan plan;
	plan.form_a = v3h;
	plan.general = v3g;
	plan.columns = fc->columns;
	plan.view_identity = fc->view_is_identity != 0;
	plan.ra.H_inv = fc->H_inv; plan.ra.hinv_stride = fc->H_inv_view_stride;
	plan.ra.packed = (const float*)(ws + L.packed); plan.ra.recq = (float4*)(ws + L.recq);
	const bool compact = (v3 || v3h || v3g) && multi_fe && f.debug_mode != 19;
	if (!compact) p.tile_cap = 0;
	else (void)fr_plan_views_c(p.T, fr_pick_VC(p.T), p.tile_cap);
	const int rstride = v3g ? (fc->columns == 11 ? 13 : 7) : ((v3 && p.tile_cap) ? 5 : 6);
	plan.ra.comp = compact ? (float4*)(ws + L.recq) : nullptr;
	plan.ra.stride = rstride;
	plan.ra.slot_idx = (compact && (v3h || v3g)) ? (uint32_t*)(ws + L.slot_idx) : nullptr;
	if (compact)
	{
		f.recA = plan.ra.comp; f.ab_view = (long long)L.PV * rstride; f.ab_stride = rstride;
		f.recQ = plan.ra.comp + 2; f.q_view = (long long)L.PV * rstride; f.q_stride = rstride;
		f.slot_idx = plan.ra.slot_idx; f.slot_view = (long long)L.PV;
	}
	else
	{
		f.recA = (const float4*)p.splat; f.ab_view = (long long)P * 2; f.ab_stride = 2;
		f.recQ = plan.ra.recq; f.q_view = (long long)P * 4; f.q_stride = 4;
		f.slot_idx = nullptr; f.slot_view = 0;
	}
	plan.ra.mt = (const float4*)(ws + L.mt);
	plan.ra.grp = (const float4*)(ws + L.grp);
	plan.ra.early = (g->cov3D_precomp || f.debug_mode == 15) ? 0 : 1;
	p.order = compact ? fc->order : nullptr;

	const bool multi = p.vis_list != nullptr && p.T <= FR_MAX_LDS_TILES;
	const int n_groups = (v3 && multi) ? fr_pick_groups(V) : 1;
	FrSideStream& tside = fr_side_stream(2);
	const bool use_side = n_groups > 1 && tside.ok;
	hipStream_t ts = use_side ? tside.stream : s;
	static thread_local hipEvent_t front_done[FR_MAX_GROUPS] = { nullptr, nullptr, nullptr, nullptr };
	const size_t nblk_v = (size_t)((P + FR_THREADS * fr_pick_G_views(P) - 1) / (FR_THREADS * fr_pick_G_views(P)));
	const size_t cap_v = (size_t)(FR_THREADS * fr_pick_G_views(P));
	const size_t rec_view = compact ? L.PV : (size_t)P;
	struct TileJoin {
		hipStream_t s; FrSideStream* side; bool on;
		~TileJoin() { if (on) { (void)hipEventRecord(side->join, side->stream); (void)hipStreamWaitEvent(s, side->join, 0); } }
	} tile_join{ s, &tside, false };
	for (int gi = 0; gi < n_groups; gi++)
	{
		const int per = n_groups > 1 ? ((V / n_groups + 7) / 8) * 8 : V;
		const int v0 = gi * per, Vg = (gi == n_groups - 1) ? V - v0 : per;
		if (Vg <= 0) break;
		FrParams pg = p;
		pg.V = Vg;
		pg.w2c = p.w2c + 16 * (size_t)v0;
		pg.radii = p.radii ? (int*)((char*)p.radii + (size_t)v0 * nblk_v * cap_v * sizeof(FrVisEntry)) : nullptr;
		pg.vis_list = p.vis_list + (size_t)v0 * nblk_v * cap_v;
		pg.vis_n = p.vis_n + (size_t)v0 * nblk_v;
		pg.splat = p.splat + (size_t)v0 * rec_view;
		pg.tile_cnt = p.tile_cnt + (size_t)v0 * p.T; pg.tile_off = p.tile_off + (size_t)v0 * p.T; pg.tile_fill = p.tile_fill + (size_t)v0 * p.T;
		pg.status = p.status + 4 * gi;
		pg.big_list = p.big_list + (size_t)v0 * p.T + 16 * gi;
		pg.part_list = p.part_list + (size_t)v0 * p.T * (2 * FR_PART_MAXP) + 16 * gi;
		if (p.view_perm && (Vg & 7) == 0) { pg.view_work = p.view_work + v0; pg.view_perm = p.view_perm + v0; }
		else { pg.view_work = nullptr; pg.view_perm = nullptr; }
		pg.blk_base = p.blk_base + (size_t)v0 * (size_t)fr_preprocess_blocks(P, V) * (size_t)p.T;
		pg.tile_cap = p.tile_cap;
		const long long k0 = (long long)((__int128)max_rendered * v0 / V), k1 = (long long)((__int128)max_rendered * (v0 + Vg) / V);
		pg.keys = p.keys + k0; pg.key_capacity = k1 - k0;
		pg.vis_count = p.vis_count ? p.vis_count + v0 : nullptr;
		pg.num_rendered = p.num_rendered ? p.num_rendered + v0 : nullptr;
		FrScorerPlan pl = plan;
		pl.skip_pack = gi > 0 || (fc->reuse_static != 0 && compact);
		if (pl.ra.hinv_stride) pl.ra.H_inv = plan.ra.H_inv + (size_t)v0 * plan.ra.hinv_stride;
		pl.ra.recq = plan.ra.recq + (size_t)v0 * rec_view * 4;
		if (pl.ra.comp) pl.ra.comp = plan.ra.comp + (size_t)v0 * L.PV * rstride;
		if (pl.ra.slot_idx) pl.ra.slot_idx = plan.ra.slot_idx + (size_t)v0 * L.PV;
		FrFisherArgs fg = f;
		fg.recA = f.recA + (size_t)v0 * f.ab_view; fg.recQ = f.recQ + (size_t)v0 * f.q_view;
		if (f.slot_idx) fg.slot_idx = f.slot_idx + (size_t)v0 * f.slot_view;
		fg.tile_scores = f.tile_scores + (size_t)v0 * p.T;
		if (f.H_inv && f.hinv_stride) fg.H_inv = f.H_inv + (size_t)v0 * f.hinv_stride;
		if (f.out_H && f.outH_stride) fg.out_H = f.out_H + (size_t)v0 * f.outH_stride;
		if (f.dL_img && f.dL_stride) fg.dL_img = f.dL_img + (size_t)v0 * f.dL_stride;

		if ((rc = fr_bin_pipeline(pg, g, s, (v3 || v3h || v3g) ? &pl : nullptr))) return rc;
		fg.key_shift = pg.tile_cap ? 4 : 0;
		if (use_side)
		{
			if (!front_done[gi] && hipEventCreateWithFlags(&front_done[gi], hipEventDisableTiming) != hipSuccess)
				return fr_fail(FR_ELAUNCH, "fr_fisher_views: hipEventCreate failed");
			if (hipEventRecord(front_done[gi], s) != hipSuccess || hipStreamWaitEvent(ts, front_done[gi], 0) != hipSuccess)
				return fr_fail(FR_ELAUNCH, "fr_fisher_views: fork to the tile stream failed");
			tile_join.on = true;
		}
		if (v3) fr_launch_fisher_v3(pg, fg, pl.ra.recq, ts);
		else if (v3h || v3g)
		{
			FrSegArgs sg;
			sg.snapT = (float*)(ws + L.seg_T); sg.snapC = (double*)(ws + L.seg_C); sg.X = (double*)(ws + L.seg_X);
			sg.list = (uint32_t*)(ws + L.seg_list);
			if (pg.V * pg.T > FR_SEG_TILES) sg.snapT = nullptr;
			if (v3h) fr_launch_fisher_v3h(pg, fg, pl.ra.recq, sg, ts);
			else fr_launch_fisher_v3g(pg, fg, fc->columns, fc->dL_dpix_image != nullptr, sg, ts);
		}
		else if (fc->columns == 4) fr_launch_fisher<4>(pg, fg, (float*)(ws + L.packed), (uint8_t*)(ws + L.fallback), ts);
		else fr_launch_fisher<11>(pg, fg, (float*)(ws + L.packed), (uint8_t*)(ws + L.fallback), ts);
		if ((rc = fr_check_launch("k_fisher_tile"))) return rc;
	}
	hipLaunchKernelGGL(k_reduce_scores, dim3(fc->out_scores ? V : 1), dim3(FR_THREADS), 0, ts, f.tile_scores, p.T, p.status, n_groups,
	                   fc->out_scores, status);
	if ((rc = fr_check_launch("k_reduce_scores"))) return rc;
	return FR_OK;
}

static size_t fr_pose_part_offset(int64_t P, int64_t W, int64_t H, int64_t V, int64_t max_rendered)
{
	return fr_fisher_layout(P, W, H, V, max_rendered, 4).total;
}
static size_t fr_pose_total(int64_t P, int64_t W, int64_t H, int64_t V, int64_t max_rendered)
{
	const int64_t T = ((W + 15) / 16) * ((H + 15) / 16);
	return fr_align(fr_pose_part_offset(P, W, H, V, max_rendered) + (size_t)(V * T) * 21 * 8);
}

extern "C" size_t fr_fisher_pose_workspace_bytes(int32_t P, int32_t W, int32_t H, int32_t n_views, int64_t max_rendered)
{
	if (P < 0 || W <= 0 || H <= 0 || n_views <= 0 || max_rendered < 0) return 0;
	return fr_pose_total(P, W, H, n_views, max_rendered);
}

extern "C" int fr_fisher_pose_workspace_layout(int32_t P, int32_t W, int32_t H, int32_t n_views, int64_t max_rendered, size_t o[9])
{
	if (P < 0 || W <= 0 || H <= 0 || n_views <= 0 || max_rendered < 0 || !o)
		return fr_fail(FR_EINVAL, "fr_fisher_pose_workspace_layout: bad argument");
	const FrFisherLayout L = fr_fisher_layout(P, W, H, n_views, max_rendered, 4);
	o[0] = L.tile_cnt; o[1] = L.tile_off; o[2] = L.keys; o[3] = L.splat; o[4] = L.recq; o[5] = L.tile_scores; o[6] = L.status; o[7] = L.vis_n;
	o[8] = fr_pose_part_offset(P, W, H, n_views, max_rendered);
	return FR_OK;
}

extern "C" int fr_fisher_pose_views(const fr_raster_cfg* cfg, const fr_gaussians* g, const fr_fisher_cfg* fc, float* out_pose_H,
                                    void* workspace, size_t workspace_bytes, int64_t max_rendered, int32_t* status, fr_stream_t stream)
{
	int rc = fr_validate(cfg, g, "fr_fisher_pose_views");
	if (rc) return rc;
	if (!fc || fc->n_views <= 0 || !fc->w2c || !status || !out_pose_H) return fr_fail(FR_EINVAL, "fr_fisher_pose_views: bad fisher cfg or null output");
	if (fc->H_inv || fc->out_scores) return fr_fail(FR_EINVAL, "fr_fisher_pose_views: H_inv / out_scores are for fr_fisher_views");
	if (fc->out_H) return fr_fail(FR_EINVAL, "fr_fisher_pose_views: out_H is for fr_fisher_views");
	if (fc->dL_dpix_image) return fr_fail(FR_EINVAL, "fr_fisher_pose_views: no per-pixel upstream-gradient images (constant dL_dpix only)");
	if (fc->reuse_static) return fr_fail(FR_EINVAL, "fr_fisher_pose_views: reuse_static is not supported");
	if (!g->colors_precomp) return fr_fail(FR_EINVAL, "fr_fisher_pose_views: needs colors_precomp");
	if (!(g->scales && g->rotations)) return fr_fail(FR_EINVAL, "fr_fisher_pose_views: needs scales and rotations");
	if (fc->tile_capacity < 0) return fr_fail(FR_EINVAL, "fr_fisher_pose_views: negative tile_capacity");
	const int P = cfg->P, W = cfg->image_width, H = cfg->image_height, V = fc->n_views;
	const long long Tt = (long long)((W + 15) / 16) * ((H + 15) / 16);
	if (Tt > FR_MAX_LDS_TILES) return fr_fail(FR_EINVAL, "fr_fisher_pose_views: images beyond 4096 tiles are not supported");
	if (fc->tile_capacity > 0)
	{
		const long long need = (long long)V * Tt * (long long)fc->tile_capacity;
		if (need > max_rendered || need >= (1ll << 32)) return fr_fail(FR_EINVAL, "fr_fisher_pose_views: n_views * tiles * tile_capacity exceeds max_rendered (or 2^32)");
	}
	hipStream_t s = (hipStream_t)stream;
	if (P == 0)
	{
		(void)hipMemsetAsync(out_pose_H, 0, (size_t)V * 36 * 4, s);
		if (fc->out_vis_count) (void)hipMemsetAsync(fc->out_vis_count, 0, (size_t)V * 4, s);
		if (fc->out_num_rendered) (void)hipMemsetAsync(fc->out_num_rendered, 0, (size_t)V * 4, s);
		(void)hipMemsetAsync(status, 0, 16, s);
		return fr_check_launch("fr_fisher_pose_views (no Gaussians)");
	}
	const FrFisherLayout L = fr_fisher_layout(P, W, H, V, max_rendered, 4);
	if (!workspace || workspace_bytes < fr_pose_total(P, W, H, V, max_rendered))
		return fr_fail(FR_ENOSPACE, "fr_fisher_pose_views: workspace smaller than fr_fisher_pose_workspace_bytes()");
	char* ws = (char*)workspace;
	FrParams p;
	fr_fill_params(p, cfg, g, V);
	p.prefiltered = 0;
	p.w2c = fc->w2c;
	if (fc->poses_are_c2w)
	{
		float* inv = (float*)(ws + L.w2c_inv);
		hipLaunchKernelGGL(k_invert_poses, dim3((V + 63) / 64), dim3(64), 0, s, V, fc->w2c, inv);
		if ((rc = fr_check_launch("k_invert_poses"))) return rc;
		p.w2c = inv;
	}
	p.radii = (int*)(ws + L.radii);
	p.vis_list = (FrVisEntry*)(ws + L.radii);
	p.vis_n = (uint32_t*)(ws + L.vis_n);
	p.splat = (FrSplat*)(ws + L.splat);
	p.cov3D_out = (float*)(ws + L.cov3D);
	p.tile_cnt = (uint32_t*)(ws + L.tile_cnt);
	p.tile_off = (uint32_t*)(ws + L.tile_off);
	p.tile_fill = (uint32_t*)(ws + L.tile_fill);
	p.status = (int*)(ws + L.status);
	p.big_list = (uint32_t*)(ws + L.big_list);
	p.part_list = (uint32_t*)(ws + L.part_list);
	const bool deal = (V & 7) == 0 && V <= 1024;
	p.view_work = deal ? (uint32_t*)(ws + L.view_work) : nullptr;
	p.view_perm = deal ? (uint32_t*)(ws + L.view_perm) : nullptr;
	p.blk_base = (uint32_t*)(ws + L.blk_base);
	p.keys = (uint64_t*)(ws + L.keys);
	p.key_capacity = max_rendered;
	if (fc->tile_capacity > 0)
	{
		const long long nblk_c = (P + FR_THREADS * fr_pick_G_views(P) - 1) / (FR_THREADS * fr_pick_G_views(P));
		const bool slots_fit = nblk_c * FR_THREADS * fr_pick_G_views(P) < (1ll << 28);
		if (p.gx <= 255u && p.gy <= 63u && slots_fit) p.tile_cap = (uint32_t)fc->tile_capacity;
	}
	(void)fr_plan_views_c(p.T, fr_pick_VC(p.T), p.tile_cap);
	p.vis_count = fc->out_vis_count;
	p.num_rendered = fc->out_num_rendered;
	p.order = fc->order;
	constexpr int rstride = FrRecStride<4, 3>::value;
	FrScorerPlan plan;
	plan.columns = 4;
	plan.form_a = false;
	plan.pose = true;
	plan.ra.H_inv = nullptr; plan.ra.hinv_stride = 0;
	plan.ra.packed = (const float*)(ws + L.packed); plan.ra.recq = (float4*)(ws + L.recq);
	plan.ra.comp = (float4*)(ws + L.recq);
	plan.ra.stride = rstride;
	plan.ra.slot_idx = nullptr;
	plan.ra.mt = (const float4*)(ws + L.mt);
	plan.ra.grp = (const float4*)(ws + L.grp);
	plan.ra.early = 1;
	FrFisherArgs f;
	memset(&f, 0, sizeof(f));
	f.dL = fc->dL_dpix;
	f.recA = plan.ra.comp; f.ab_view = (long long)L.PV * rstride; f.ab_stride = rstride;
	f.recQ = plan.ra.comp + 2; f.q_view = (long long)L.PV * rstride; f.q_stride = rstride;
	if ((rc = fr_bin_pipeline(p, g, s, &plan))) return rc;
	f.key_shift = p.tile_cap ? 4 : 0;
	double* part = (double*)(ws + fr_pose_part_offset(P, W, H, V, max_rendered));
	hipEvent_t ev0 = nullptr, ev1 = nullptr;
	if (g_prof_on)
	{
		(void)hipEventCreate(&ev0); (void)hipEventCreate(&ev1);
		(void)hipEventRecord(ev0, s);
	}
	hipLaunchKernelGGL(k_fisher_pose_tile, dim3(p.T * V), dim3(FR_THREADS), 0, s, p, f, part);
	if (g_prof_on)
	{
		(void)hipEventRecord(ev1, s);
		g_prof_events.push_back(std::make_pair(ev0, ev1));
	}
	if ((rc = fr_check_launch("k_fisher_pose_tile"))) return rc;
	hipLaunchKernelGGL(k_pose_reduce, dim3(V), dim3(64), 0, s, (const double*)part, p.T, (const int*)p.status, out_pose_H, status);
	return fr_check_launch("k_pose_reduce");
}

extern "C" size_t fr_render_views_workspace_bytes(int32_t P, int32_t W, int32_t H, int32_t n_views, int64_t max_rendered)
{
	if (P < 0 || W <= 0 || H <= 0 || n_views <= 0 || max_rendered < 0) return 0;
	if ((long long)((W + 15) / 16) * ((H + 15) / 16) > FR_MAX_LDS_TILES) return 0;
	return fr_fisher_layout(P, W, H, n_views, max_rendered, 4).total;
}

extern "C" int fr_render_views_workspace_layout(int32_t P, int32_t W, int32_t H, int32_t n_views, int64_t max_rendered, size_t o[8])
{
	if (P < 0 || W <= 0 || H <= 0 || n_views <= 0 || max_rendered < 0 || !o || (long long)((W + 15) / 16) * ((H + 15) / 16) > FR_MAX_LDS_TILES)
		return fr_fail(FR_EINVAL, "fr_render_views_workspace_layout: bad argument");
	const FrFisherLayout L = fr_fisher_layout(P, W, H, n_views, max_rendered, 4);
	o[0] = L.tile_cnt; o[1] = L.tile_off; o[2] = L.keys; o[3] = L.splat; o[4] = L.recq; o[5] = L.tile_scores; o[6] = L.status; o[7] = L.vis_n;
	return FR_OK;
}

extern "C" int fr_render_views(const fr_raster_cfg* cfg, const fr_gaussians* g, const fr_fisher_cfg* fc,
                               float* out_color, float* out_features, float* out_depth, float* out_final_T,
                               void* workspace, size_t workspace_bytes, int64_t max_rendered, int32_t* status, fr_stream_t stream)
{
	int rc = fr_validate(cfg, g, "fr_render_views");
	if (rc) return rc;
	if (!fc || fc->n_views <= 0 || !fc->w2c || !status) return fr_fail(FR_EINVAL, "fr_render_views: bad fisher cfg or null status");
	if (!out_color && !out_features && !out_depth && !out_final_T) return fr_fail(FR_EINVAL, "fr_render_views: no output requested");
	if (fc->H_inv || fc->out_scores) return fr_fail(FR_EINVAL, "fr_render_views: H_inv / out_scores are for fr_fisher_views");
	if (fc->out_H) return fr_fail(FR_EINVAL, "fr_render_views: out_H is for fr_fisher_views");
	if (fc->dL_dpix_image) return fr_fail(FR_EINVAL, "fr_render_views: no upstream-gradient images (there is no backward)");
	if (fc->reuse_static) return fr_fail(FR_EINVAL, "fr_render_views: reuse_static is not supported");
	if (g->shs || !g->colors_precomp) return fr_fail(FR_EINVAL, "fr_render_views: needs colors_precomp (no SH colours)");
	if (g->cov3D_precomp || !(g->scales && g->rotations)) return fr_fail(FR_EINVAL, "fr_render_views: needs scales and rotations (no cov3D_precomp)");
	if (fc->tile_capacity < 0) return fr_fail(FR_EINVAL, "fr_render_views: negative tile_capacity");
	if (max_rendered < 0) return fr_fail(FR_EINVAL, "fr_render_views: negative max_rendered");
	const int P = cfg->P, W = cfg->image_width, H = cfg->image_height, V = fc->n_views;
	const long long Tt = (long long)((W + 15) / 16) * ((H + 15) / 16);
	if (Tt > FR_MAX_LDS_TILES) return fr_fail(FR_EINVAL, "fr_render_views: images beyond 4096 tiles are not supported");
	if (fc->tile_capacity > 0)
	{
		const long long need = (long long)V * Tt * (long long)fc->tile_capacity;
		if (need > max_rendered || need >= (1ll << 32)) return fr_fail(FR_EINVAL, "fr_render_views: n_views * tiles * tile_capacity exceeds max_rendered (or 2^32)");
	}
	if (!cfg->bg) return fr_fail(FR_EINVAL, "fr_render_views: null bg");
	const FrFisherLayout L = fr_fisher_layout(P, W, H, V, max_rendered, 4);
	if (!workspace || workspace_bytes < L.total)
		return fr_fail(FR_ENOSPACE, "fr_render_views: workspace smaller than fr_render_views_workspace_bytes()");
	hipStream_t s = (hipStream_t)stream;
	char* ws = (char*)workspace;
	FrParams p;
	fr_fill_params(p, cfg, g, V);
	p.prefiltered = 0;
	p.tile_cnt = (uint32_t*)(ws + L.tile_cnt);
	p.tile_off = (uint32_t*)(ws + L.tile_off);
	p.status = (int*)(ws + L.status);
	p.keys = (uint64_t*)(ws + L.keys);
	FrFisherArgs f;
	memset(&f, 0, sizeof(f));
	constexpr int rstride = FrRecStride<4, 4>::value;
	f.recA = (const float4*)(ws + L.recq); f.ab_view = (long long)L.PV * rstride; f.ab_stride = rstride;
	if (P == 0)
	{
		(void)hipMemsetAsync(p.tile_cnt, 0, (size_t)V * p.T * 4, s);
		(void)hipMemsetAsync(p.tile_off, 0, (size_t)V * p.T * 4, s);
		(void)hipMemsetAsync(p.status, 0, 16, s);
		if (fc->out_vis_count) (void)hipMemsetAsync(fc->out_vis_count, 0, (size_t)V * 4, s);
		if (fc->out_num_rendered) (void)hipMemsetAsync(fc->out_num_rendered, 0, (size_t)V * 4, s);
	}
	else
	{
		p.w2c = fc->w2c;
		if (fc->poses_are_c2w)
		{
			float* inv = (float*)(ws + L.w2c_inv);
			hipLaunchKernelGGL(k_invert_poses, dim3((V + 63) / 64), dim3(64), 0, s, V, fc->w2c, inv);
			if ((rc = fr_check_launch("k_invert_poses"))) return rc;
			p.w2c = inv;
		}
		p.radii = (int*)(ws + L.radii);
		p.vis_list = (FrVisEntry*)(ws + L.radii);
		p.vis_n = (uint32_t*)(ws + L.vis_n);
		p.splat = (FrSplat*)(ws + L.splat);
		p.cov3D_out = (float*)(ws + L.cov3D);
		p.tile_fill = (uint32_t*)(ws + L.tile_fill);
		p.big_list = (uint32_t*)(ws + L.big_list);
		p.part_list = (uint32_t*)(ws + L.part_list);
		const bool deal = (V & 7) == 0 && V <= 1024;
		p.view_work = deal ? (uint32_t*)(ws + L.view_work) : nullptr;
		p.view_perm = deal ? (uint32_t*)(ws + L.view_perm) : nullptr;
		p.blk_base = (uint32_t*)(ws + L.blk_base);
		p.key_capacity = max_rendered;
		if (fc->tile_capacity > 0)
		{
			const long long nblk_c = (P + FR_THREADS * fr_pick_G_views(P) - 1) / (FR_THREADS * fr_pick_G_views(P));
			const bool slots_fit = nblk_c * FR_THREADS * fr_pick_G_views(P) < (1ll << 28);
			if (p.gx <= 255u && p.gy <= 63u && slots_fit) p.tile_cap = (uint32_t)fc->tile_capacity;
		}
		(void)fr_plan_views_c(p.T, fr_pick_VC(p.T), p.tile_cap);
		p.vis_count = fc->out_vis_count;
		p.num_rendered = fc->out_num_rendered;
		p.order = fc->order;
		FrScorerPlan plan;
		plan.columns = 4;
		plan.form_a = false;
		plan.render = true;
		plan.ra.H_inv = nullptr; plan.ra.hinv_stride = 0;
		plan.ra.packed = (const float*)(ws + L.packed); plan.ra.recq = (float4*)(ws + L.recq);
		plan.ra.comp = (float4*)(ws + L.recq);
		plan.ra.stride = rstride;
		plan.ra.slot_idx = nullptr;
		plan.ra.mt = (const float4*)(ws + L.mt);
		plan.ra.grp = (const float4*)(ws + L.grp);
		plan.ra.early = 1;
		if ((rc = fr_bin_pipeline(p, g, s, &plan))) return rc;
		f.key_shift = p.tile_cap ? 4 : 0;
	}
	if (out_features) hipLaunchKernelGGL((k_render_views_tile<6>), dim3(p.T * V), dim3(FR_THREADS), 0, s, p, f, out_color, out_features, out_depth, out_final_T, (int*)status);
	else hipLaunchKernelGGL((k_render_views_tile<3>), dim3(p.T * V), dim3(FR_THREADS), 0, s, p, f, out_color, out_features, out_depth, out_final_T, (int*)status);
	return fr_check_launch("k_render_views_tile");
}

static size_t fr_point_total(int64_t P, int64_t W, int64_t H, int64_t V, int64_t max_rendered, int columns)
{
	const FrFisherLayout L = fr_fisher_layout(P, W, H, V, max_rendered, columns);
	return fr_align(L.total + (size_t)V * L.PV * 4);
}

extern "C" size_t fr_fisher_point_workspace_bytes(int32_t P, int32_t W, int32_t H, int32_t n_views, int64_t max_rendered, int32_t columns)
{
	if (P < 0 || W <= 0 || H <= 0 || n_views <= 0 || max_rendered < 0 || (columns != 4 && columns != 11)) return 0;
	if ((long long)((W + 15) / 16) * ((H + 15) / 16) > FR_MAX_LDS_TILES) return 0;
	return fr_point_total(P, W, H, n_views, max_rendered, columns);
}

extern "C" int fr_fisher_point_workspace_layout(int32_t P, int32_t W, int32_t H, int32_t n_views, int64_t max_rendered, int32_t columns, size_t o[9])
{
	if (P < 0 || W <= 0 || H <= 0 || n_views <= 0 || max_rendered < 0 || (columns != 4 && columns != 11) || !o ||
	    (long long)((W + 15) / 16) * ((H + 15) / 16) > FR_MAX_LDS_TILES)
		return fr_fail(FR_EINVAL, "fr_fisher_point_workspace_layout: bad argument");
	const FrFisherLayout L = fr_fisher_layout(P, W, H, n_views, max_rendered, columns);
	o[0] = L.tile_cnt; o[1] = L.tile_off; o[2] = L.keys; o[3] = L.splat; o[4] = L.recq; o[5] = L.tile_scores; o[6] = L.status; o[7] = L.vis_n;
	o[8] = L.total;
	return FR_OK;
}

extern "C" int fr_fisher_point_views(const fr_raster_cfg* cfg, const fr_gaussians* g, const fr_fisher_cfg* fc,
                                     float* out_point_scores, float* out_point_max,
                                     void* workspace, size_t workspace_bytes, int64_t max_rendered, int32_t* status, fr_stream_t stream)
{
	int rc = fr_validate(cfg, g, "fr_fisher_point_views");
	if (rc) return rc;
	if (!fc || fc->n_views <= 0 || !fc->w2c || !status) return fr_fail(FR_EINVAL, "fr_fisher_point_views: bad fisher cfg or null status");
	if (fc->columns != 4 && fc->columns != 11) return fr_fail(FR_EINVAL, "fr_fisher_point_views: columns must be 4 or 11");
	if (fc->out_H) return fr_fail(FR_EINVAL, "fr_fisher_point_views: out_H is for fr_fisher_views");
	if (fc->dL_dpix_image) return fr_fail(FR_EINVAL, "fr_fisher_point_views: no per-pixel upstream-gradient images (constant dL_dpix only)");
	if (fc->reuse_static) return fr_fail(FR_EINVAL, "fr_fisher_point_views: reuse_static is not supported");
	if (!fc->H_inv) return fr_fail(FR_EINVAL, "fr_fisher_point_views: needs H_inv");
	if (!out_point_scores && !out_point_max) return fr_fail(FR_EINVAL, "fr_fisher_point_views: no output requested");
	if (!g->colors_precomp) return fr_fail(FR_EINVAL, "fr_fisher_point_views: needs colors_precomp");
	if (g->cov3D_precomp || !(g->scales && g->rotations)) return fr_fail(FR_EINVAL, "fr_fisher_point_views: needs scales and rotations (no cov3D_precomp)");
	if (fc->tile_capacity < 0) return fr_fail(FR_EINVAL, "fr_fisher_point_views: negative tile_capacity");
	if (max_rendered < 0) return fr_fail(FR_EINVAL, "fr_fisher_point_views: negative max_rendered");
	const int P = cfg->P, W = cfg->image_width, H = cfg->image_height, V = fc->n_views, C = fc->columns;
	const long long Tt = (long long)((W + 15) / 16) * ((H + 15) / 16);
	if (Tt > FR_MAX_LDS_TILES) return fr_fail(FR_EINVAL, "fr_fisher_point_views: images beyond 4096 tiles are not supported");
	if (fc->tile_capacity > 0)
	{
		const long long need = (long long)V * Tt * (long long)fc->tile_capacity;
		if (need > max_rendered || need >= (1ll << 32)) return fr_fail(FR_EINVAL, "fr_fisher_point_views: n_views * tiles * tile_capacity exceeds max_rendered (or 2^32)");
	}
	hipStream_t s = (hipStream_t)stream;
	if (P == 0)
	{
		if (fc->out_scores) (void)hipMemsetAsync(fc->out_scores, 0, (size_t)V * 4, s);
		if (fc->out_vis_count) (void)hipMemsetAsync(fc->out_vis_count, 0, (size_t)V * 4, s);
		if (fc->out_num_rendered) (void)hipMemsetAsync(fc->out_num_rendered, 0, (size_t)V * 4, s);
		(void)hipMemsetAsync(status, 0, 16, s);
		return fr_check_launch("fr_fisher_point_views (no Gaussians)");
	}
	const FrFisherLayout L = fr_fisher_layout(P, W, H, V, max_rendered, C);
	if (!workspace || workspace_bytes < fr_point_total(P, W, H, V, max_rendered, C))
		return fr_fail(FR_ENOSPACE, "fr_fisher_point_views: workspace smaller than fr_fisher_point_workspace_bytes()");
	const long long G = fr_pick_G_views(P);
	const long long nblk_c = (P + FR_THREADS * G - 1) / (FR_THREADS * G);
	if ((long long)V * nblk_c * G >= (1ll << 31)) return fr_fail(FR_EINVAL, "fr_fisher_point_views: too many (view, slot) groups for one launch");
	char* ws = (char*)workspace;
	FrParams p;
	fr_fill_params(p, cfg, g, V);
	p.prefiltered = 0;
	p.w2c = fc->w2c;
	if (fc->poses_are_c2w)
	{
		float* inv = (float*)(ws + L.w2c_inv);
		hipLaunchKernelGGL(k_invert_poses, dim3((V + 63) / 64), dim3(64), 0, s, V, fc->w2c, inv);
		if ((rc = fr_check_launch("k_invert_poses"))) return rc;
		p.w2c = inv;
	}
	p.radii = (int*)(ws + L.radii);
	p.vis_list = (FrVisEntry*)(ws + L.radii);
	p.vis_n = (uint32_t*)(ws + L.vis_n);
	p.splat = (FrSplat*)(ws + L.splat);
	p.cov3D_out = (float*)(ws + L.cov3D);
	p.tile_cnt = (uint32_t*)(ws + L.tile_cnt);
	p.tile_off = (uint32_t*)(ws + L.tile_off);
	p.tile_fill = (uint32_t*)(ws + L.tile_fill);
	p.status = (int*)(ws + L.status);
	p.big_list = (uint32_t*)(ws + L.big_list);
	p.part_list = (uint32_t*)(ws + L.part_list);
	const bool deal = (V & 7) == 0 && V <= 1024;
	p.view_work = deal ? (uint32_t*)(ws + L.view_work) : nullptr;
	p.view_perm = deal ? (uint32_t*)(ws + L.view_perm) : nullptr;
	p.blk_base = (uint32_t*)(ws + L.blk_base);
	p.keys = (uint64_t*)(ws + L.keys);
	p.key_capacity = max_rendered;
	if (fc->tile_capacity > 0)
	{
		const bool slots_fit = nblk_c * FR_THREADS * G < (1ll << 28);
		if (p.gx <= 255u && p.gy <= 63u && slots_fit) p.tile_cap = (uint32_t)fc->tile_capacity;
	}
	(void)fr_plan_views_c(p.T, fr_pick_VC(p.T), p.tile_cap);
	p.vis_count = fc->out_vis_count;
	p.num_rendered = fc->out_num_rendered;
	p.order = fc->order;
	const int rstride = p.tile_cap ? 5 : 6;
	float* slot_acc = (float*)(ws + L.total);
	FrScorerPlan plan;
	plan.columns = C;
	plan.form_a = false;
	plan.point = true;
	plan.ra.H_inv = fc->H_inv; plan.ra.hinv_stride = fc->H_inv_view_stride;
	plan.ra.packed = (const float*)(ws + L.packed); plan.ra.recq = (float4*)(ws + L.recq);
	plan.ra.comp = (float4*)(ws + L.recq);
	plan.ra.stride = rstride;
	plan.ra.slot_idx = (uint32_t*)(ws + L.slot_idx);
	plan.ra.slot_acc = slot_acc;
	plan.ra.mt = (const float4*)(ws + L.mt);
	plan.ra.grp = (const float4*)(ws + L.grp);
	plan.ra.early = 1;
	FrFisherArgs f;
	memset(&f, 0, sizeof(f));
	f.dL = fc->dL_dpix;
	f.tile_scores = (float*)(ws + L.tile_scores);
	f.debug_mode = fr_debug_mode();
	f.recA = plan.ra.comp; f.ab_view = (long long)L.PV * rstride; f.ab_stride = rstride;
	f.slot_idx = plan.ra.slot_idx; f.slot_view = (long long)L.PV;
	if ((rc = fr_bin_pipeline(p, g, s, &plan))) return rc;
	if ((p.tile_cap ? 5 : 6) != rstride) return fr_fail(FR_EINVAL, "fr_fisher_point_views: the front end left the planned key form");
	f.key_shift = p.tile_cap ? 4 : 0;
	hipEvent_t ev0 = nullptr, ev1 = nullptr;
	if (g_prof_on)
	{
		(void)hipEventCreate(&ev0); (void)hipEventCreate(&ev1);
		(void)hipEventRecord(ev0, s);
	}
	if (p.tile_cap) hipLaunchKernelGGL((k_fisher_point_tile<true>), dim3(p.T * V), dim3(FR_THREADS), 0, s, p, f, slot_acc);
	else hipLaunchKernelGGL((k_fisher_point_tile<false>), dim3(p.T * V), dim3(FR_THREADS), 0, s, p, f, slot_acc);
	if (g_prof_on)
	{
		(void)hipEventRecord(ev1, s);
		g_prof_events.push_back(std::make_pair(ev0, ev1));
	}
	if ((rc = fr_check_launch("k_fisher_point_tile"))) return rc;
	if (out_point_scores)
	{
		const unsigned long long n = (unsigned long long)V * (unsigned long long)P;
		const unsigned long long blocks = (n + FR_THREADS * 4 - 1) / (FR_THREADS * 4);
		hipLaunchKernelGGL(k_point_clear, dim3((unsigned)(blocks > 8192 ? 8192 : blocks)), dim3(FR_THREADS), 0, s, out_point_scores, n, (const int*)p.status);
		if ((rc = fr_check_launch("k_point_clear"))) return rc;
	}
	hipLaunchKernelGGL(k_point_finish, dim3((unsigned)((long long)V * nblk_c * G)), dim3(FR_THREADS), 0, s, P, V, (uint32_t)nblk_c, (uint32_t)(FR_THREADS * G),
	                   (const uint32_t*)p.vis_n, (const uint32_t*)plan.ra.slot_idx, (const float*)slot_acc, out_point_scores, (uint32_t*)out_point_max, (const int*)p.status);
	if ((rc = fr_check_launch("k_point_finish"))) return rc;
	hipLaunchKernelGGL(k_reduce_scores, dim3(fc->out_scores ? V : 1), dim3(FR_THREADS), 0, s, f.tile_scores, p.T, p.status, 1, fc->out_scores, status);
	return fr_check_launch("k_reduce_scores");
}

__global__ __launch_bounds__(FR_THREADS) void k_densify_stats(int P, const int* __restrict__ radii, const float* __restrict__ grad_means2D,
                                                              float* __restrict__ max_radius, float* __restrict__ grad_accum,
                                                              float* __restrict__ denom, uint8_t* __restrict__ seen)
{
	const int i = blockIdx.x * FR_THREADS + threadIdx.x;
	if (i >= P) return;
	const int r = radii[i];
	const bool vis = r > 0;
	if (seen) seen[i] = vis ? 1 : 0;
	if (!vis) return;
	if (max_radius) max_radius[i] = fmaxf((float)r, max_radius[i]);
	if (grad_means2D)
	{
		const float gx = grad_means2D[3 * (size_t)i], gy = grad_means2D[3 * (size_t)i + 1];
		grad_accum[i] += sqrtf(gx * gx + gy * gy);
		denom[i] += 1.0f;
	}
}

__device__ __forceinline__ float fr_max_scale(const float* __restrict__ log_scales, int scale_cols, int i)
{
	float m = fr_expf(log_scales[(size_t)i * scale_cols]);
	for (int k = 1; k < scale_cols; k++) m = fmaxf(m, fr_expf(log_scales[(size_t)i * scale_cols + k]));
	return m;
}

__global__ __launch_bounds__(FR_THREADS) void k_densify_masks(int P, const float* __restrict__ grad_accum, const float* __restrict__ denom,
                                                              const float* __restrict__ log_scales, int scale_cols, float grad_thresh,
                                                              float clone_max_scale, float split_min_scale,
                                                              uint8_t* __restrict__ to_clone, uint8_t* __restrict__ to_split)
{
	const int i = blockIdx.x * FR_THREADS + threadIdx.x;
	if (i >= P) return;
	float g = grad_accum[i] / denom[i];
	if (g != g) g = 0.0f;
	const float ms = fr_max_scale(log_scales, scale_cols, i);
	to_clone[i] = (g >= grad_thresh && ms <= clone_max_scale) ? 1 : 0;
	to_split[i] = (ms > split_min_scale) ? 1 : 0;
}

__global__ __launch_bounds__(FR_THREADS) void k_prune_mask(int P, const float* __restrict__ logit_opacities, const float* __restrict__ log_scales,
                                                           int scale_cols, float opacity_thresh, float big_thresh, uint8_t* __restrict__ to_remove)
{
	const int i = blockIdx.x * FR_THREADS + threadIdx.x;
	if (i >= P) return;
	const float op = 1.0f / (1.0f + fr_expf(-logit_opacities[i]));
	bool rm = op < opacity_thresh;
	if (big_thresh >= 0.0f) rm = rm || (fr_max_scale(log_scales, scale_cols, i) > big_thresh);
	to_remove[i] = rm ? 1 : 0;
}

extern "C" int fr_densify_stats(int32_t P, const int32_t* radii, const float* grad_means2D, float* max_2D_radius,
                                float* means2D_gradient_accum, float* denom, uint8_t* seen, fr_stream_t stream)
{
	if (P < 0) return fr_fail(FR_EINVAL, "fr_densify_stats: P < 0");
	if (P == 0) return FR_OK;
	if (!radii || (grad_means2D && (!means2D_gradient_accum || !denom))) return fr_fail(FR_EINVAL, "fr_densify_stats: null pointer");
	hipLaunchKernelGGL(k_densify_stats, dim3((P + FR_THREADS - 1) / FR_THREADS), dim3(FR_THREADS), 0, (hipStream_t)stream,
	                   P, radii, grad_means2D, max_2D_radius, means2D_gradient_accum, denom, seen);
	return fr_check_launch("k_densify_stats");
}

extern "C" int fr_densify_masks(int32_t P, const float* means2D_gradient_accum, const float* denom, const float* log_scales,
                                int32_t scale_cols, float grad_thresh, float clone_max_scale, float split_min_scale,
                                uint8_t* to_clone, uint8_t* to_split, fr_stream_t stream)
{
	if (P < 0 || (scale_cols != 1 && scale_cols != 3)) return fr_fail(FR_EINVAL, "fr_densify_masks: bad P / scale_cols");
	if (P == 0) return FR_OK;
	if (!means2D_gradient_accum || !denom || !log_scales || !to_clone || !to_split) return fr_fail(FR_EINVAL, "fr_densify_masks: null pointer");
	hipLaunchKernelGGL(k_densify_masks, dim3((P + FR_THREADS - 1) / FR_THREADS), dim3(FR_THREADS), 0, (hipStream_t)stream,
	                   P, means2D_gradient_accum, denom, log_scales, scale_cols, grad_thresh, clone_max_scale, split_min_scale, to_clone, to_split);
	return fr_check_launch("k_densify_masks");
}

extern "C" int fr_prune_mask(int32_t P, const float* logit_opacities, const float* log_scales, int32_t scale_cols,
                             float opacity_thresh, float big_thresh, uint8_t* to_remove, fr_stream_t stream)
{
	if (P < 0 || (scale_cols != 1 && scale_cols != 3)) return fr_fail(FR_EINVAL, "fr_prune_mask: bad P / scale_cols");
	if (P == 0) return FR_OK;
	if (!logit_opacities || !to_remove || (big_thresh >= 0.0f && !log_scales)) return fr_fail(FR_EINVAL, "fr_prune_mask: null pointer");
	hipLaunchKernelGGL(k_prune_mask, dim3((P + FR_THREADS - 1) / FR_THREADS), dim3(FR_THREADS), 0, (hipStream_t)stream,
	                   P, logit_opacities, log_scales, scale_cols, opacity_thresh, big_thresh, to_remove);
	return fr_check_launch("k_prune_mask");
}

#define FR_KNN_BOX 1024
#define FR_KNN_CHUNK 2048

__device__ __forceinline__ uint32_t fr_enc_f(float f)
{
	uint32_t u = fr_as_u32(f);
	return (u & 0x80000000u) ? ~u : (u | 0x80000000u);
}
__device__ __forceinline__ float fr_dec_f(uint32_t e)
{
	return fr_as_f32((e & 0x80000000u) ? (e & 0x7fffffffu) : ~e);
}

__global__ __launch_bounds__(FR_THREADS) void k_knn_minmax(int P, const float* __restrict__ pts, uint32_t* __restrict__ mm)
{
	__shared__ float s_lo[3][4], s_hi[3][4];
	float lo[3] = { INFINITY, INFINITY, INFINITY }, hi[3] = { -INFINITY, -INFINITY, -INFINITY };
	for (int i = blockIdx.x * FR_THREADS + threadIdx.x; i < P; i += gridDim.x * FR_THREADS)
#pragma unroll
		for (int a = 0; a < 3; a++) { float x = pts[3 * (size_t)i + a]; lo[a] = fminf(lo[a], x); hi[a] = fmaxf(hi[a], x); }
#pragma unroll
	for (int a = 0; a < 3; a++)
	{
#pragma unroll
		for (int o = 32; o > 0; o >>= 1) { lo[a] = fminf(lo[a], __shfl_xor(lo[a], o, 64)); hi[a] = fmaxf(hi[a], __shfl_xor(hi[a], o, 64)); }
		if ((threadIdx.x & 63) == 0) { s_lo[a][threadIdx.x >> 6] = lo[a]; s_hi[a][threadIdx.x >> 6] = hi[a]; }
	}
	__syncthreads();
	if (threadIdx.x < 3)
// ... 322 lines not shown
```

### fisher-nerf-customized_amd/fisher_rast/_lib.py

```python
import ctypes
import os

_HERE = os.path.dirname(os.path.abspath(__file__))
SO_PATH = os.environ.get("FISHER_RAST_SO", os.path.join(_HERE, "libfisher_rast.so"))

FR_OK, FR_EINVAL, FR_ELAUNCH, FR_ENOSPACE = 0, 1, 2, 3
FR_POPGS_TOPT, FR_POPGS_DOPT = 0, 1

_f32p = ctypes.c_void_p


class RasterCfg(ctypes.Structure):
    _fields_ = [
        ("P", ctypes.c_int32),
        ("image_height", ctypes.c_int32),
        ("image_width", ctypes.c_int32),
        ("tanfovx", ctypes.c_float),
        ("tanfovy", ctypes.c_float),
        ("scale_modifier", ctypes.c_float),
        ("sh_degree", ctypes.c_int32),
        ("sh_coeffs", ctypes.c_int32),
        ("prefiltered", ctypes.c_int32),
        ("bg", _f32p),
        ("viewmatrix", _f32p),
        ("projmatrix", _f32p),
        ("campos", _f32p),
    ]


class Gaussians(ctypes.Structure):
    _fields_ = [
        ("means3D", _f32p),
        ("colors_precomp", _f32p),
        ("shs", _f32p),
        ("opacities", _f32p),
        ("scales", _f32p),
        ("rotations", _f32p),
        ("cov3D_precomp", _f32p),
    ]


class FisherCfg(ctypes.Structure):
    _fields_ = [
        ("n_views", ctypes.c_int32),
        ("columns", ctypes.c_int32),
        ("dL_dpix", ctypes.c_float),
        ("w2c", _f32p),
        ("H_inv", _f32p),
        ("H_inv_view_stride", ctypes.c_int64),
        ("out_scores", _f32p),
        ("out_H", _f32p),
        ("out_H_view_stride", ctypes.c_int64),
        ("out_vis_count", ctypes.c_void_p),
        ("out_num_rendered", ctypes.c_void_p),
        ("dL_dpix_image", _f32p),
        ("dL_image_view_stride", ctypes.c_int64),
        ("tile_capacity", ctypes.c_int32),
        ("poses_are_c2w", ctypes.c_int32),
        ("reuse_static", ctypes.c_int32),
        ("order", ctypes.c_void_p),
        ("view_is_identity", ctypes.c_int32),
    ]


class OccCfg(ctypes.Structure):
    _fields_ = [
        ("grid_w", ctypes.c_int32),
        ("grid_h", ctypes.c_int32),
        ("cell_size", ctypes.c_float),
        ("center_x", ctypes.c_float),
        ("center_z", ctypes.c_float),
        ("height_lower", ctypes.c_float),
        ("height_upper", ctypes.c_float),
        ("far_distance", ctypes.c_float),
    ]


EXPORTS = (
    "fr_version", "fr_last_error", "fr_build_id", "fr_init", "fr_fisher_workspace_layout", "fr_fisher_part_list_offset", "fr_workspace_bytes", "fr_workspace_layout", "fr_mark_visible",
    "fr_forward", "fr_backward", "fr_backward_scratch_bytes", "fr_backward_ws", "fr_forward_pair", "fr_forward_features", "fr_backward_pair", "fr_backward_pair_scratch_bytes", "fr_backward_pair_ws", "fr_fisher_workspace_bytes", "fr_fisher_views",
    "fr_fisher_pose_workspace_bytes", "fr_fisher_pose_workspace_layout", "fr_fisher_pose_views",
    "fr_render_views_workspace_bytes", "fr_render_views_workspace_layout", "fr_render_views",
    "fr_fisher_point_workspace_bytes", "fr_fisher_point_workspace_layout", "fr_fisher_point_views",
    "fr_popgs_diag_criterion_workspace_bytes", "fr_popgs_diag_criterion",
    "fr_densify_stats", "fr_densify_masks", "fr_prune_mask", "fr_knn_workspace_bytes", "fr_knn_dist2", "fr_spatial_order_workspace_bytes", "fr_spatial_order", "fr_profile_enable", "fr_profile_fetch",
    "fr_occ_workspace_bytes", "fr_occ_update", "fr_occ_freespace", "fr_occ_frontiers", "fr_occ_erode", "fr_occ_cells_of",
    "fr_occ_ring_candidates", "fr_occ_free_candidates",
)

_lib = None

_CSRC = os.path.join(os.path.dirname(_HERE), "csrc")
_INCLUDE = os.path.join(os.path.dirname(os.path.dirname(_HERE)), "include")
SOURCES = [os.path.join(_CSRC, n) for n in ("fisher_rast.hip", "fisher_occ.hip", "fr_popgs.hip", "fr_math.h", "fr_internal.h")] + \
          [os.path.join(_INCLUDE, n) for n in ("fisher_rast.h", "fisher_occ.h")]


def source_hash():
    import hashlib
    h = hashlib.sha256()
    for f in SOURCES:
        if not os.path.exists(f):
            return None
        h.update(open(f, "rb").read())
    return h.hexdigest()[:16]


class FisherRastError(RuntimeError):
    pass


def load():
    global _lib
    if _lib is not None:
        return _lib
    if not os.path.exists(SO_PATH):
        raise FisherRastError(
            f"{SO_PATH} is missing: the HIP extension has not been built "
            "(run `python -c \"import __graft_entry__ as g; g.build()\"` at the repo root). "
            "There is no CPU fallback for this path.")
    import torch
    lib = ctypes.CDLL(SO_PATH)
    ab_build = "FISHER_RAST_SO" in os.environ
    for name in EXPORTS:
        if not hasattr(lib, name) and not ab_build:
            raise FisherRastError(f"{SO_PATH} does not export {name}")
    lib.fr_version.restype = ctypes.c_int
    lib.fr_last_error.restype = ctypes.c_char_p
    lib.fr_build_id.restype = ctypes.c_char_p
    lib.fr_init.restype = ctypes.c_int
    lib.fr_fisher_workspace_layout.restype = ctypes.c_int
    lib.fr_fisher_workspace_layout.argtypes = [ctypes.c_int32, ctypes.c_int32, ctypes.c_int32, ctypes.c_int32,
                                               ctypes.c_int64, ctypes.c_int32, ctypes.POINTER(ctypes.c_size_t)]
    if hasattr(lib, "fr_fisher_part_list_offset"):
        lib.fr_fisher_part_list_offset.restype = ctypes.c_int
        lib.fr_fisher_part_list_offset.argtypes = lib.fr_fisher_workspace_layout.argtypes
    want = source_hash()
    got = lib.fr_build_id().decode().split(":")[-1]
    if "FISHER_RAST_SO" not in os.environ and want is not None and got != want:
        raise FisherRastError(f"{SO_PATH} was built from other sources (build id {got}, sources {want}): "
                              "run `python -c \"import __graft_entry__ as g; g.build()\"`")
    lib.fr_workspace_bytes.restype = ctypes.c_int
    lib.fr_workspace_bytes.argtypes = [ctypes.c_int32, ctypes.c_int32, ctypes.c_int32, ctypes.c_int64,
                                       ctypes.POINTER(ctypes.c_size_t)]
    lib.fr_workspace_layout.restype = ctypes.c_int
    lib.fr_workspace_layout.argtypes = [ctypes.c_int32, ctypes.c_int32, ctypes.c_int32, ctypes.c_int64,
                                        ctypes.POINTER(ctypes.c_size_t)]
    lib.fr_mark_visible.restype = ctypes.c_int
    lib.fr_mark_visible.argtypes = [ctypes.c_int32, _f32p, _f32p, _f32p, ctypes.c_void_p, ctypes.c_void_p]
    lib.fr_forward.restype = ctypes.c_int
    lib.fr_forward.argtypes = [ctypes.POINTER(RasterCfg), ctypes.POINTER(Gaussians),
                               ctypes.c_void_p, ctypes.c_void_p, ctypes.c_int64, ctypes.c_void_p,
                               _f32p, _f32p, ctypes.c_void_p, ctypes.c_void_p, ctypes.c_void_p]
    lib.fr_backward.restype = ctypes.c_int
    lib.fr_backward.argtypes = [ctypes.POINTER(RasterCfg), ctypes.POINTER(Gaussians), ctypes.c_void_p,
                                ctypes.c_void_p, ctypes.c_void_p, ctypes.c_void_p,
                                _f32p, ctypes.c_int32] + [_f32p] * 9 + [ctypes.c_void_p]
    lib.fr_backward_scratch_bytes.restype = ctypes.c_size_t
    lib.fr_backward_scratch_bytes.argtypes = [ctypes.c_int32] * 4 + [ctypes.c_int64]
    lib.fr_backward_ws.restype = ctypes.c_int
    lib.fr_backward_ws.argtypes = [ctypes.POINTER(RasterCfg), ctypes.POINTER(Gaussians), ctypes.c_void_p,
                                   ctypes.c_void_p, ctypes.c_void_p, ctypes.c_void_p,
                                   _f32p, ctypes.c_int32] + [_f32p] * 9 + [ctypes.c_int64, ctypes.c_void_p, ctypes.c_size_t, ctypes.c_void_p]
    lib.fr_forward_pair.restype = ctypes.c_int
    lib.fr_forward_pair.argtypes = [ctypes.POINTER(RasterCfg), ctypes.POINTER(Gaussians), _f32p,
                                    ctypes.c_void_p, ctypes.c_void_p, ctypes.c_int64, ctypes.c_void_p,
                                    _f32p, _f32p, _f32p, ctypes.c_void_p, ctypes.c_void_p, ctypes.c_void_p]
    lib.fr_forward_features.restype = ctypes.c_int
    lib.fr_forward_features.argtypes = [ctypes.POINTER(RasterCfg), _f32p, ctypes.c_void_p, ctypes.c_void_p, ctypes.c_void_p,
                                        _f32p, ctypes.c_void_p]
    lib.fr_backward_pair.restype = ctypes.c_int
    lib.fr_backward_pair.argtypes = [ctypes.POINTER(RasterCfg), ctypes.POINTER(Gaussians), ctypes.c_void_p,
                                     ctypes.c_void_p, ctypes.c_void_p, ctypes.c_void_p,
                                     _f32p, _f32p, _f32p] + [_f32p] * 10 + [ctypes.c_void_p]
    lib.fr_backward_pair_scratch_bytes.restype = ctypes.c_size_t
    lib.fr_backward_pair_scratch_bytes.argtypes = [ctypes.c_int32] * 3 + [ctypes.c_int64]
    lib.fr_backward_pair_ws.restype = ctypes.c_int
    lib.fr_backward_pair_ws.argtypes = [ctypes.POINTER(RasterCfg), ctypes.POINTER(Gaussians), ctypes.c_void_p,
                                        ctypes.c_void_p, ctypes.c_void_p, ctypes.c_void_p,
                                        _f32p, _f32p, _f32p] + [_f32p] * 10 + [ctypes.c_int64, ctypes.c_void_p, ctypes.c_size_t, ctypes.c_void_p]
    lib.fr_fisher_workspace_bytes.restype = ctypes.c_size_t
    lib.fr_fisher_workspace_bytes.argtypes = [ctypes.c_int32, ctypes.c_int32, ctypes.c_int32, ctypes.c_int32,
                                              ctypes.c_int64, ctypes.c_int32]
    lib.fr_fisher_views.restype = ctypes.c_int
    lib.fr_fisher_views.argtypes = [ctypes.POINTER(RasterCfg), ctypes.POINTER(Gaussians),
                                    ctypes.POINTER(FisherCfg), ctypes.c_void_p, ctypes.c_size_t, ctypes.c_int64,
                                    ctypes.c_void_p, ctypes.c_void_p]
    lib.fr_fisher_pose_workspace_bytes.restype = ctypes.c_size_t
    lib.fr_fisher_pose_workspace_bytes.argtypes = [ctypes.c_int32, ctypes.c_int32, ctypes.c_int32, ctypes.c_int32, ctypes.c_int64]
    lib.fr_fisher_pose_workspace_layout.restype = ctypes.c_int
    lib.fr_fisher_pose_workspace_layout.argtypes = [ctypes.c_int32, ctypes.c_int32, ctypes.c_int32, ctypes.c_int32, ctypes.c_int64,
                                                    ctypes.POINTER(ctypes.c_size_t)]
    lib.fr_fisher_pose_views.restype = ctypes.c_int
    lib.fr_fisher_pose_views.argtypes = [ctypes.POINTER(RasterCfg), ctypes.POINTER(Gaussians), ctypes.POINTER(FisherCfg), _f32p,
                                         ctypes.c_void_p, ctypes.c_size_t, ctypes.c_int64, ctypes.c_void_p, ctypes.c_void_p]
    if hasattr(lib, "fr_render_views"):
        lib.fr_render_views_workspace_bytes.restype = ctypes.c_size_t
        lib.fr_render_views_workspace_bytes.argtypes = [ctypes.c_int32, ctypes.c_int32, ctypes.c_int32, ctypes.c_int32, ctypes.c_int64]
        lib.fr_render_views_workspace_layout.restype = ctypes.c_int
        lib.fr_render_views_workspace_layout.argtypes = [ctypes.c_int32, ctypes.c_int32, ctypes.c_int32, ctypes.c_int32, ctypes.c_int64,
                                                         ctypes.POINTER(ctypes.c_size_t)]
        lib.fr_render_views.restype = ctypes.c_int
        lib.fr_render_views.argtypes = [ctypes.POINTER(RasterCfg), ctypes.POINTER(Gaussians), ctypes.POINTER(FisherCfg),
                                        _f32p, _f32p, _f32p, _f32p,
                                        ctypes.c_void_p, ctypes.c_size_t, ctypes.c_int64, ctypes.c_void_p, ctypes.c_void_p]
    if hasattr(lib, "fr_fisher_point_views"):
        lib.fr_fisher_point_workspace_bytes.restype = ctypes.c_size_t
        lib.fr_fisher_point_workspace_bytes.argtypes = [ctypes.c_int32, ctypes.c_int32, ctypes.c_int32, ctypes.c_int32, ctypes.c_int64,
                                                        ctypes.c_int32]
        lib.fr_fisher_point_workspace_layout.restype = ctypes.c_int
        lib.fr_fisher_point_workspace_layout.argtypes = [ctypes.c_int32, ctypes.c_int32, ctypes.c_int32, ctypes.c_int32, ctypes.c_int64,
                                                         ctypes.c_int32, ctypes.POINTER(ctypes.c_size_t)]
        lib.fr_fisher_point_views.restype = ctypes.c_int
        lib.fr_fisher_point_views.argtypes = [ctypes.POINTER(RasterCfg), ctypes.POINTER(Gaussians), ctypes.POINTER(FisherCfg), _f32p, _f32p,
                                              ctypes.c_void_p, ctypes.c_size_t, ctypes.c_int64, ctypes.c_void_p, ctypes.c_void_p]
    if hasattr(lib, "fr_popgs_diag_criterion"):
        lib.fr_popgs_diag_criterion_workspace_bytes.restype = ctypes.c_size_t
        lib.fr_popgs_diag_criterion_workspace_bytes.argtypes = [ctypes.c_int32, ctypes.c_int64]
        lib.fr_popgs_diag_criterion.restype = ctypes.c_int
        lib.fr_popgs_diag_criterion.argtypes = [ctypes.c_int32, ctypes.c_int32, ctypes.c_int64, _f32p, _f32p, ctypes.c_int64, _f32p,
                                                ctypes.c_void_p, ctypes.c_void_p, ctypes.c_float, ctypes.c_int32, ctypes.c_void_p,
                                                ctypes.c_void_p, ctypes.c_size_t, ctypes.c_void_p]
    lib.fr_densify_stats.restype = ctypes.c_int
    lib.fr_densify_stats.argtypes = [ctypes.c_int32, ctypes.c_void_p, _f32p, _f32p, _f32p, _f32p, ctypes.c_void_p, ctypes.c_void_p]
    lib.fr_densify_masks.restype = ctypes.c_int
    lib.fr_densify_masks.argtypes = [ctypes.c_int32, _f32p, _f32p, _f32p, ctypes.c_int32, ctypes.c_float, ctypes.c_float, ctypes.c_float,
                                     ctypes.c_void_p, ctypes.c_void_p, ctypes.c_void_p]
    lib.fr_prune_mask.restype = ctypes.c_int
    lib.fr_prune_mask.argtypes = [ctypes.c_int32, _f32p, _f32p, ctypes.c_int32, ctypes.c_float, ctypes.c_float, ctypes.c_void_p, ctypes.c_void_p]
    lib.fr_knn_workspace_bytes.restype = ctypes.c_size_t
    lib.fr_knn_workspace_bytes.argtypes = [ctypes.c_int32]
    lib.fr_knn_dist2.restype = ctypes.c_int
    lib.fr_knn_dist2.argtypes = [ctypes.c_int32, _f32p, _f32p, ctypes.c_void_p, ctypes.c_size_t, ctypes.c_void_p]
    lib.fr_spatial_order_workspace_bytes.restype = ctypes.c_size_t
    lib.fr_spatial_order_workspace_bytes.argtypes = [ctypes.c_int32]
    lib.fr_spatial_order.restype = ctypes.c_int
    lib.fr_spatial_order.argtypes = [ctypes.c_int32, _f32p, ctypes.c_void_p, ctypes.c_void_p, ctypes.c_size_t, ctypes.c_void_p]
    lib.fr_profile_enable.restype = ctypes.c_int
    lib.fr_profile_enable.argtypes = [ctypes.c_int]
    lib.fr_profile_fetch.restype = ctypes.c_int
    lib.fr_profile_fetch.argtypes = [ctypes.POINTER(ctypes.c_float), ctypes.c_int]
    occp = ctypes.POINTER(OccCfg)
    f4, f16 = ctypes.c_float * 4, ctypes.c_float * 16
    lib.fr_occ_workspace_bytes.restype = ctypes.c_size_t
    lib.fr_occ_workspace_bytes.argtypes = [occp]
    lib.fr_occ_update.restype = ctypes.c_int
    lib.fr_occ_update.argtypes = [occp, _f32p, ctypes.c_int32, ctypes.c_int32, ctypes.c_int32, ctypes.POINTER(f4), ctypes.POINTER(f16),
                                  ctypes.POINTER(ctypes.c_float), ctypes.c_int32, ctypes.c_int32, ctypes.c_int32, _f32p,
                                  ctypes.c_void_p, ctypes.c_size_t, ctypes.c_void_p]
    lib.fr_occ_freespace.restype = ctypes.c_int
    lib.fr_occ_freespace.argtypes = [occp, _f32p, _f32p, ctypes.c_int32, ctypes.c_void_p, ctypes.c_void_p, ctypes.c_size_t, ctypes.c_void_p]
    lib.fr_occ_frontiers.restype = ctypes.c_int
    lib.fr_occ_frontiers.argtypes = [occp, _f32p, ctypes.c_void_p, ctypes.c_int32, ctypes.c_int32, ctypes.c_int32, ctypes.c_int32,
                                     ctypes.c_void_p, ctypes.c_void_p, ctypes.c_void_p, ctypes.c_int32, ctypes.c_void_p,
                                     ctypes.c_void_p, ctypes.c_size_t, ctypes.c_void_p]
    lib.fr_occ_erode.restype = ctypes.c_int
    lib.fr_occ_erode.argtypes = [occp, ctypes.c_void_p, ctypes.c_void_p, ctypes.c_int32, ctypes.c_void_p]
    lib.fr_occ_ring_candidates.restype = ctypes.c_int
    lib.fr_occ_ring_candidates.argtypes = [occp, _f32p, ctypes.c_int32, ctypes.c_int32, ctypes.c_float, ctypes.c_float, ctypes.c_float,
                                           ctypes.c_uint32, ctypes.c_void_p, ctypes.c_int32, _f32p, ctypes.c_void_p, ctypes.c_void_p]
    lib.fr_occ_free_candidates.restype = ctypes.c_int
    lib.fr_occ_free_candidates.argtypes = [occp, ctypes.c_void_p, ctypes.c_float, ctypes.c_uint32, _f32p, ctypes.c_int32,
                                           ctypes.c_void_p, ctypes.c_void_p, ctypes.c_size_t, ctypes.c_void_p]
    lib.fr_occ_cells_of.restype = ctypes.c_int
    lib.fr_occ_cells_of.argtypes = [occp, _f32p, ctypes.c_int32, ctypes.c_void_p, ctypes.c_void_p]
    _lib = lib
    return lib


def check(rc, what):
    if rc != FR_OK:
        msg = load().fr_last_error().decode("utf-8", "replace")
        raise FisherRastError(f"{what} failed (code {rc}): {msg}")
```

### include/fisher_rast.h

```cpp
#ifndef FISHER_RAST_H_INCLUDED
#define FISHER_RAST_H_INCLUDED

#include <stddef.h>
#include <stdint.h>

#ifdef __cplusplus
extern "C" {
#endif

#define FR_VERSION 100

enum {
	FR_OK = 0,
	FR_EINVAL = 1,
	FR_ELAUNCH = 2,
	FR_ENOSPACE = 3
};

#define FR_STATUS_WORDS 4

typedef void* fr_stream_t;

typedef struct fr_raster_cfg {
	int32_t P;
	int32_t image_height;
	int32_t image_width;
	float tanfovx;
	float tanfovy;
	float scale_modifier;
	int32_t sh_degree;
	int32_t sh_coeffs;
	int32_t prefiltered;
	const float* bg;
	const float* viewmatrix;
	const float* projmatrix;
	const float* campos;
} fr_raster_cfg;

typedef struct fr_gaussians {
	const float* means3D;
	const float* colors_precomp;
	const float* shs;
	const float* opacities;
	const float* scales;
	const float* rotations;
	const float* cov3D_precomp;
} fr_gaussians;

int fr_version(void);
const char* fr_last_error(void);
const char* fr_build_id(void);
int fr_init(void);


int fr_workspace_bytes(int32_t P, int32_t W, int32_t H, int64_t max_rendered, size_t out[3]);

int fr_workspace_layout(int32_t P, int32_t W, int32_t H, int64_t max_rendered, size_t offsets[11]);

int fr_mark_visible(int32_t P, const float* means3D, const float* viewmatrix, const float* projmatrix,
                    uint8_t* present, fr_stream_t stream);

int fr_forward(const fr_raster_cfg* cfg, const fr_gaussians* g,
               void* geom_ws, void* binning_ws, int64_t binning_capacity, void* image_ws,
               float* out_color, float* out_depth, int32_t* radii, int32_t* status, fr_stream_t stream);

int fr_backward(const fr_raster_cfg* cfg, const fr_gaussians* g, const int32_t* radii,
                const void* geom_ws, const void* binning_ws, const void* image_ws,
                const float* dL_dout_color, int32_t power,
                float* dL_dmeans2D, float* dL_dcolors, float* dL_dopacity, float* dL_dmeans3D,
                float* dL_dcov3D, float* dL_dsh, float* dL_dscales, float* dL_drotations, float* dL_dconic,
                fr_stream_t stream);

size_t fr_backward_scratch_bytes(int32_t P, int32_t W, int32_t H, int32_t power, int64_t num_rendered);
int fr_backward_ws(const fr_raster_cfg* cfg, const fr_gaussians* g, const int32_t* radii,
                   const void* geom_ws, const void* binning_ws, const void* image_ws,
                   const float* dL_dout_color, int32_t power,
                   float* dL_dmeans2D, float* dL_dcolors, float* dL_dopacity, float* dL_dmeans3D,
                   float* dL_dcov3D, float* dL_dsh, float* dL_dscales, float* dL_drotations, float* dL_dconic,
                   int64_t num_rendered, void* scratch, size_t scratch_bytes, fr_stream_t stream);

int fr_forward_pair(const fr_raster_cfg* cfg, const fr_gaussians* g, const float* features,
                    void* geom_ws, void* binning_ws, int64_t binning_capacity, void* image_ws,
                    float* out_color, float* out_features, float* out_depth, int32_t* radii, int32_t* status,
                    fr_stream_t stream);
int fr_forward_features(const fr_raster_cfg* cfg, const float* features,
                        const void* geom_ws, const void* binning_ws, void* image_ws,
                        float* out_features, fr_stream_t stream);
int fr_backward_pair(const fr_raster_cfg* cfg, const fr_gaussians* g, const int32_t* radii,
                     const void* geom_ws, const void* binning_ws, const void* image_ws,
                     const float* dL_dout_color, const float* features, const float* dL_dout_features,
                     float* dL_dmeans2D, float* dL_dmeans2D_features, float* dL_dcolors, float* dL_dfeatures,
                     float* dL_dopacity, float* dL_dmeans3D, float* dL_dcov3D, float* dL_dscales,
                     float* dL_drotations, float* dL_dconic, fr_stream_t stream);

size_t fr_backward_pair_scratch_bytes(int32_t P, int32_t W, int32_t H, int64_t num_rendered);
int fr_backward_pair_ws(const fr_raster_cfg* cfg, const fr_gaussians* g, const int32_t* radii,
                        const void* geom_ws, const void* binning_ws, const void* image_ws,
                        const float* dL_dout_color, const float* features, const float* dL_dout_features,
                        float* dL_dmeans2D, float* dL_dmeans2D_features, float* dL_dcolors, float* dL_dfeatures,
                        float* dL_dopacity, float* dL_dmeans3D, float* dL_dcov3D, float* dL_dscales,
                        float* dL_drotations, float* dL_dconic,
                        int64_t num_rendered, void* scratch, size_t scratch_bytes, fr_stream_t stream);


typedef struct fr_fisher_cfg {
	int32_t n_views;
	int32_t columns;
	float dL_dpix;
	const float* w2c;
	const float* H_inv;
	int64_t H_inv_view_stride;
	float* out_scores;
	float* out_H;
	int64_t out_H_view_stride;
	int32_t* out_vis_count;
	int32_t* out_num_rendered;
	const float* dL_dpix_image;
	int64_t dL_image_view_stride;
	int32_t tile_capacity;
	int32_t poses_are_c2w;
	int32_t reuse_static;
	const uint32_t* order;
	int32_t view_is_identity;
} fr_fisher_cfg;

size_t fr_spatial_order_workspace_bytes(int32_t P);
int fr_spatial_order(int32_t P, const float* means3D, uint32_t* order_out, void* workspace, size_t workspace_bytes, fr_stream_t stream);

size_t fr_fisher_workspace_bytes(int32_t P, int32_t W, int32_t H, int32_t n_views, int64_t max_rendered, int32_t columns);
int fr_fisher_workspace_layout(int32_t P, int32_t W, int32_t H, int32_t n_views, int64_t max_rendered, int32_t columns,
                               size_t offsets[8]);
int fr_fisher_part_list_offset(int32_t P, int32_t W, int32_t H, int32_t n_views, int64_t max_rendered, int32_t columns, size_t* offset);

int fr_fisher_views(const fr_raster_cfg* cfg, const fr_gaussians* g, const fr_fisher_cfg* cfg_f,
                    void* workspace, size_t workspace_bytes, int64_t max_rendered,
                    int32_t* status, fr_stream_t stream);

size_t fr_fisher_pose_workspace_bytes(int32_t P, int32_t W, int32_t H, int32_t n_views, int64_t max_rendered);
int fr_fisher_pose_workspace_layout(int32_t P, int32_t W, int32_t H, int32_t n_views, int64_t max_rendered, size_t offsets[9]);
int fr_fisher_pose_views(const fr_raster_cfg* cfg, const fr_gaussians* g, const fr_fisher_cfg* cfg_f, float* out_pose_H,
                         void* workspace, size_t workspace_bytes, int64_t max_rendered, int32_t* status, fr_stream_t stream);

size_t fr_render_views_workspace_bytes(int32_t P, int32_t W, int32_t H, int32_t n_views, int64_t max_rendered);
int fr_render_views_workspace_layout(int32_t P, int32_t W, int32_t H, int32_t n_views, int64_t max_rendered, size_t offsets[8]);
int fr_render_views(const fr_raster_cfg* cfg, const fr_gaussians* g, const fr_fisher_cfg* cfg_f,
                    float* out_color, float* out_features, float* out_depth, float* out_final_T,
                    void* workspace, size_t workspace_bytes, int64_t max_rendered, int32_t* status, fr_stream_t stream);

size_t fr_fisher_point_workspace_bytes(int32_t P, int32_t W, int32_t H, int32_t n_views, int64_t max_rendered, int32_t columns);
int fr_fisher_point_workspace_layout(int32_t P, int32_t W, int32_t H, int32_t n_views, int64_t max_rendered, int32_t columns,
                                     size_t offsets[9]);
int fr_fisher_point_views(const fr_raster_cfg* cfg, const fr_gaussians* g, const fr_fisher_cfg* cfg_f,
                          float* out_point_scores, float* out_point_max,
                          void* workspace, size_t workspace_bytes, int64_t max_rendered, int32_t* status, fr_stream_t stream);

enum { FR_POPGS_TOPT = 0, FR_POPGS_DOPT = 1 };
#define FR_POPGS_CLAMP 1e-12f
size_t fr_popgs_diag_criterion_workspace_bytes(int32_t V, int64_t E);
int fr_popgs_diag_criterion(int32_t V, int32_t K, int64_t E, const float* rows, const float* prior_in, int64_t prior_in_view_stride,
                            float* prior_out, const uint8_t* accumulate, const int32_t* vis_count, float lam, int32_t criterion,
                            double* scores, void* workspace, size_t workspace_bytes, fr_stream_t stream);


int fr_densify_stats(int32_t P, const int32_t* radii, const float* grad_means2D, float* max_2D_radius,
                     float* means2D_gradient_accum, float* denom, uint8_t* seen, fr_stream_t stream);

int fr_densify_masks(int32_t P, const float* means2D_gradient_accum, const float* denom, const float* log_scales,
                     int32_t scale_cols, float grad_thresh, float clone_max_scale, float split_min_scale,
                     uint8_t* to_clone, uint8_t* to_split, fr_stream_t stream);

int fr_prune_mask(int32_t P, const float* logit_opacities, const float* log_scales, int32_t scale_cols,
                  float opacity_thresh, float big_thresh, uint8_t* to_remove, fr_stream_t stream);


size_t fr_knn_workspace_bytes(int32_t P);
int fr_knn_dist2(int32_t P, const float* points, float* out, void* workspace, size_t workspace_bytes,
                 fr_stream_t stream);


int fr_profile_enable(int on);
int fr_profile_fetch(float* ms, int max_n);

#ifdef __cplusplus
}
#endif
#endif
```

Before: 47580.

## Split per-view frustum culling into a separate all-views bitmask kernel

Adds a k_cull_views kernel that, for every Gaussian and up to 32 views per launch row, computes the frustum and early-out keep test once and writes a per-view keep bitmask into a new workspace region. The preprocess front end now reads these bits instead of doing the projection test per view inside its LDS-heavy loop, and skips the prefix scan when a group has no survivors. The aim is to run culling with full thread parallelism and no LDS pressure, taking it off the serialized per-view loop. The cost is an extra kernel launch, a larger workspace, and an extra global mask write and read.

```diff
diff --git a/fisher-nerf-customized_amd/csrc/fisher_rast.hip b/fisher-nerf-customized_amd/csrc/fisher_rast.hip
--- a/fisher-nerf-customized_amd/csrc/fisher_rast.hip
+++ b/fisher-nerf-customized_amd/csrc/fisher_rast.hip
@@ -550,6 +550,9 @@
 	uint32_t* slot_idx;
 	int stride;
 	float* slot_acc;
+	uint32_t* cull;
+	int cull_stride;
+	int cull_v0;
 };
 template <int C> struct FrPackSize { static constexpr int value = (C >= 11) ? 32 : 16; };
 template <int C, bool REWRITE, bool FORM_A = false, bool FIVE = false, bool IDV = false>
@@ -787,6 +790,111 @@
 	}
 }
 
+template <bool IDV>
+__global__ __launch_bounds__(FR_THREADS) void k_cull_views(FrParams p, FrRecordArgs ra, uint32_t* __restrict__ out)
+{
+	const int tid = threadIdx.x, lane = tid & 63;
+	const int i = blockIdx.x * FR_THREADS + tid;
+	const int vb = blockIdx.y * 32;
+	const int nv = min(32, p.V - vb);
+	const bool has_w2c = p.w2c != nullptr;
+	const float* __restrict__ w2c = p.w2c + 16 * (size_t)vb;
+	float vm[16], pm[16];
+#pragma unroll
+	for (int k = 0; k < 16; k++) { vm[k] = IDV ? (k % 5 == 0 ? 1.f : 0.f) : p.view[k]; pm[k] = p.proj[k]; }
+	const bool early = ra.early != 0;
+	const float lx = 1.3f * p.tanfovx, ly = 1.3f * p.tanfovy;
+	float wn;
+	{
+		const float c0 = fabsf(vm[0]) + fabsf(vm[1]) + fabsf(vm[2]), c1 = fabsf(vm[4]) + fabsf(vm[5]) + fabsf(vm[6]), c2 = fabsf(vm[8]) + fabsf(vm[9]) + fabsf(vm[10]);
+		const float r0 = fabsf(vm[0]) + fabsf(vm[4]) + fabsf(vm[8]), r1 = fabsf(vm[1]) + fabsf(vm[5]) + fabsf(vm[9]), r2 = fabsf(vm[2]) + fabsf(vm[6]) + fabsf(vm[10]);
+		wn = fmaxf(c0, fmaxf(c1, c2)) * fmaxf(r0, fmaxf(r1, r2));
+	}
+	const float fx2 = 1.02f * wn * p.focal_x * p.focal_x, fy2 = 1.02f * wn * p.focal_y * p.focal_y;
+	const float xmax = (float)(p.gx * FR_BLOCK_X + FR_BLOCK_X), ymax = (float)(p.gy * FR_BLOCK_Y + FR_BLOCK_Y);
+	uint32_t skipv = 0u;
+	if (early && ra.grp != nullptr && blockIdx.x * FR_THREADS < p.P)
+	{
+		const float wrow = fabsf(pm[3] - vm[2]) + fabsf(pm[7] - vm[6]) + fabsf(pm[11] - vm[10]) + fabsf(pm[15] - vm[14]);
+		const float wmag = fabsf(vm[2]) + fabsf(vm[6]) + fabsf(vm[10]) + fabsf(vm[14]);
+		const bool pinhole = wrow <= 1e-6f * wmag;
+		bool skip = false;
+		const int vv = lane;
+		if (pinhole && vv < nv)
+		{
+#pragma clang fp contract(fast)
+			const float4 b0 = ra.grp[2 * (size_t)blockIdx.x], b1 = ra.grp[2 * (size_t)blockIdx.x + 1];
+			const fr_f3 cw = { 0.5f * (b0.x + b1.x), 0.5f * (b0.y + b1.y), 0.5f * (b0.z + b1.z) };
+			const float ex = b1.x - cw.x, ey = b1.y - cw.y, ez = b1.z - cw.z;
+			float R = 1.01f * __builtin_amdgcn_sqrtf(ex * ex + ey * ey + ez * ez) + 1e-6f;
+			float m[12];
+#pragma unroll
+			for (int k = 0; k < 12; k++) m[k] = has_w2c ? w2c[16 * vv + k] : 0.f;
+			const fr_f3 c = has_w2c ? fr_world_to_cam(cw, m) : cw;
+			if (has_w2c)
+			{
+				const float g00 = m[0] * m[0] + m[4] * m[4] + m[8] * m[8], g11 = m[1] * m[1] + m[5] * m[5] + m[9] * m[9], g22 = m[2] * m[2] + m[6] * m[6] + m[10] * m[10];
+				const float g01 = fabsf(m[0] * m[1] + m[4] * m[5] + m[8] * m[9]), g02 = fabsf(m[0] * m[2] + m[4] * m[6] + m[8] * m[10]), g12 = fabsf(m[1] * m[2] + m[5] * m[6] + m[9] * m[10]);
+				R *= __builtin_amdgcn_sqrtf(fmaxf(g00 + g01 + g02, fmaxf(g01 + g11 + g12, g02 + g12 + g22))) * 1.00001f;
+			}
+			const float kcm = fx2 * (1.0f + lx * lx) + fy2 * (1.0f + ly * ly);
+			const float a2 = 2.0f * 1.01f * 3.0f * __builtin_amdgcn_sqrtf(kcm * b0.w);
+			const float c0 = 6.0f;
+			const float Wf = (float)p.W, Hf = (float)p.H;
+			const float zc = vm[2] * c.x + vm[6] * c.y + vm[10] * c.z + vm[14];
+			const float zn = __builtin_amdgcn_sqrtf(vm[2] * vm[2] + vm[6] * vm[6] + vm[10] * vm[10]);
+			auto side = [&](float sx, float sy, float sz, float sw, float kz, float add) -> bool {
+				const float Ax = sx + kz * vm[2], Ay = sy + kz * vm[6], Az = sz + kz * vm[10];
+				const float Lc = Ax * c.x + Ay * c.y + Az * c.z + (sw + kz * vm[14]) + add;
+				return Lc + __builtin_amdgcn_sqrtf(Ax * Ax + Ay * Ay + Az * Az) * R < 0.f;
+			};
+			const bool left = side(Wf * pm[0], Wf * pm[4], Wf * pm[8], Wf * pm[12], Wf - 1.0f + 2.0f * c0, a2);
+			const bool right = side(-Wf * pm[0], -Wf * pm[4], -Wf * pm[8], -Wf * pm[12], -(Wf - 1.0f - 2.0f * xmax - 2.0f * c0), a2);
+			const bool top = side(Hf * pm[1], Hf * pm[5], Hf * pm[9], Hf * pm[13], Hf - 1.0f + 2.0f * c0, a2);
+			const bool bottom = side(-Hf * pm[1], -Hf * pm[5], -Hf * pm[9], -Hf * pm[13], -(Hf - 1.0f - 2.0f * ymax - 2.0f * c0), a2);
+			const bool behind = zc + zn * R <= 0.001f;
+			skip = left || right || top || bottom || behind;
+		}
+		skipv = (uint32_t)__builtin_amdgcn_ballot_w64(skip);
+	}
+	const bool live = i < p.P;
+	fr_f3 pw = { 0.f, 0.f, 0.f };
+	float tr = 0.f;
+	if (live) { const float4 m4 = ra.mt[i]; pw = fr_f3{ m4.x, m4.y, m4.z }; tr = m4.w; }
+	auto keep_in = [&](const float* __restrict__ w) -> bool {
+		const fr_f3 po = has_w2c ? fr_world_to_cam(pw, w) : pw;
+		const fr_f3 p_view = IDV ? po : fr_xform4x3(po, vm);
+		bool keep = live && !(p_view.z <= 0.001f);
+		if (early)
+		{
+#pragma clang fp contract(fast)
+			const float hx = __builtin_fmaf(pm[8], po.z, __builtin_fmaf(pm[4], po.y, __builtin_fmaf(pm[0], po.x, pm[12])));
+			const float hy = __builtin_fmaf(pm[9], po.z, __builtin_fmaf(pm[5], po.y, __builtin_fmaf(pm[1], po.x, pm[13])));
+			const float hw = __builtin_fmaf(pm[11], po.z, __builtin_fmaf(pm[7], po.y, __builtin_fmaf(pm[3], po.x, pm[15])));
+			const float p_w = __builtin_amdgcn_rcpf(hw + 0.0000001f);
+			const float px = ((hx * p_w + 1.0f) * (float)p.W - 1.0f) * 0.5f, py = ((hy * p_w + 1.0f) * (float)p.H - 1.0f) * 0.5f;
+			const float iz = __builtin_amdgcn_rcpf(p_view.z);
+			const float jx = fminf(fabsf(p_view.x * iz) * 1.001f, lx), jy = fminf(fabsf(p_view.y * iz) * 1.001f, ly);
+			const float kc = fx2 * (1.0f + jx * jx) + fy2 * (1.0f + jy * jy);
+			const float rb = 3.0f * __builtin_amdgcn_sqrtf(kc * tr * (iz * iz) + 0.7f) * 1.000001f + 2.0f;
+			const bool outside = (px + rb < 0.f) || (px - rb > xmax) || (py + rb < 0.f) || (py - rb > ymax);
+			keep = keep && !outside;
+		}
+		return keep;
+	};
+	uint32_t bits = 0u;
+	for (int vv = 0; vv < nv; vv += 2)
+	{
+		const bool two = vv + 1 < nv;
+		const bool sa = (skipv >> vv) & 1u, sb = !two || ((skipv >> (vv + 1)) & 1u);
+		if (sa && sb) continue;
+		const bool ka = keep_in(w2c + 16 * vv), kb = keep_in(w2c + 16 * (two ? vv + 1 : vv));
+		bits |= ((ka && !sa) ? 1u : 0u) << vv;
+		bits |= ((kb && !sb) ? 2u : 0u) << vv;
+	}
+	out[(size_t)blockIdx.y * ((size_t)gridDim.x * FR_THREADS) + i] = bits;
+}
+
 template <int C, int AF, bool DK, bool IDV = false, bool SLOTS = false>
 __global__ __launch_bounds__(FR_THREADS) void k_preprocess_views_c(FrParams p, FrRecordArgs ra)
 {
@@ -830,60 +938,9 @@
 	const unsigned long long lt = (1ull << lane) - 1ull;
 	__syncthreads();
 	const int iw = blockIdx.x * p.G * FR_THREADS;
-	const bool early = ra.early != 0;
-	const float lx = 1.3f * p.tanfovx, ly = 1.3f * p.tanfovy;
-	float wn;
-	{
-		const float c0 = fabsf(vm[0]) + fabsf(vm[1]) + fabsf(vm[2]), c1 = fabsf(vm[4]) + fabsf(vm[5]) + fabsf(vm[6]), c2 = fabsf(vm[8]) + fabsf(vm[9]) + fabsf(vm[10]);
-		const float r0 = fabsf(vm[0]) + fabsf(vm[4]) + fabsf(vm[8]), r1 = fabsf(vm[1]) + fabsf(vm[5]) + fabsf(vm[9]), r2 = fabsf(vm[2]) + fabsf(vm[6]) + fabsf(vm[10]);
-		wn = fmaxf(c0, fmaxf(c1, c2)) * fmaxf(r0, fmaxf(r1, r2));
-	}
-	const float fx2 = 1.02f * wn * p.focal_x * p.focal_x, fy2 = 1.02f * wn * p.focal_y * p.focal_y;
-	const float xmax = (float)(p.gx * FR_BLOCK_X + FR_BLOCK_X), ymax = (float)(p.gy * FR_BLOCK_Y + FR_BLOCK_Y);
-	unsigned long long skipm = 0ull;
-	if (early && ra.grp != nullptr && p.G * nv <= 64)
-	{
-		const float wrow = fabsf(pm[3] - vm[2]) + fabsf(pm[7] - vm[6]) + fabsf(pm[11] - vm[10]) + fabsf(pm[15] - vm[14]);
-		const float wmag = fabsf(vm[2]) + fabsf(vm[6]) + fabsf(vm[10]) + fabsf(vm[14]);
-		const bool pinhole = wrow <= 1e-6f * wmag;
-		bool skip = false;
-		const int g = lane / nv, vv = lane - g * nv;
-		const int blk = blockIdx.x * p.G + g;
-		if (pinhole && g < p.G && blk * FR_THREADS < p.P)
-		{
-#pragma clang fp contract(fast)
-			const float4 b0 = ra.grp[2 * (size_t)blk], b1 = ra.grp[2 * (size_t)blk + 1];
-			const fr_f3 cw = { 0.5f * (b0.x + b1.x), 0.5f * (b0.y + b1.y), 0.5f * (b0.z + b1.z) };
-			const float ex = b1.x - cw.x, ey = b1.y - cw.y, ez = b1.z - cw.z;
-			float R = 1.01f * __builtin_amdgcn_sqrtf(ex * ex + ey * ey + ez * ez) + 1e-6f;
-			const fr_f3 c = has_w2c ? fr_world_to_cam(cw, s_wm + 12 * vv) : cw;
-			if (has_w2c)
-			{
-				const float* m = s_wm + 12 * vv;
-				const float g00 = m[0] * m[0] + m[4] * m[4] + m[8] * m[8], g11 = m[1] * m[1] + m[5] * m[5] + m[9] * m[9], g22 = m[2] * m[2] + m[6] * m[6] + m[10] * m[10];
-				const float g01 = fabsf(m[0] * m[1] + m[4] * m[5] + m[8] * m[9]), g02 = fabsf(m[0] * m[2] + m[4] * m[6] + m[8] * m[10]), g12 = fabsf(m[1] * m[2] + m[5] * m[6] + m[9] * m[10]);
-				R *= __builtin_amdgcn_sqrtf(fmaxf(g00 + g01 + g02, fmaxf(g01 + g11 + g12, g02 + g12 + g22))) * 1.00001f;
-			}
-			const float kcm = fx2 * (1.0f + lx * lx) + fy2 * (1.0f + ly * ly);
-			const float a2 = 2.0f * 1.01f * 3.0f * __builtin_amdgcn_sqrtf(kcm * b0.w);
-			const float c0 = 6.0f;
-			const float Wf = (float)p.W, Hf = (float)p.H;
-			const float zc = vm[2] * c.x + vm[6] * c.y + vm[10] * c.z + vm[14];
-			const float zn = __builtin_amdgcn_sqrtf(vm[2] * vm[2] + vm[6] * vm[6] + vm[10] * vm[10]);
-			auto side = [&](float sx, float sy, float sz, float sw, float kz, float add) -> bool {
-				const float Ax = sx + kz * vm[2], Ay = sy + kz * vm[6], Az = sz + kz * vm[10];
-				const float Lc = Ax * c.x + Ay * c.y + Az * c.z + (sw + kz * vm[14]) + add;
-				return Lc + __builtin_amdgcn_sqrtf(Ax * Ax + Ay * Ay + Az * Az) * R < 0.f;
-			};
-			const bool left = side(Wf * pm[0], Wf * pm[4], Wf * pm[8], Wf * pm[12], Wf - 1.0f + 2.0f * c0, a2);
-			const bool right = side(-Wf * pm[0], -Wf * pm[4], -Wf * pm[8], -Wf * pm[12], -(Wf - 1.0f - 2.0f * xmax - 2.0f * c0), a2);
-			const bool top = side(Hf * pm[1], Hf * pm[5], Hf * pm[9], Hf * pm[13], Hf - 1.0f + 2.0f * c0, a2);
-			const bool bottom = side(-Hf * pm[1], -Hf * pm[5], -Hf * pm[9], -Hf * pm[13], -(Hf - 1.0f - 2.0f * ymax - 2.0f * c0), a2);
-			const bool behind = zc + zn * R <= 0.001f;
-			skip = left || right || top || bottom || behind;
-		}
-		skipm = __builtin_amdgcn_ballot_w64(skip);
-	}
+	const int gv = ra.cull_v0 + v0;
+	const uint32_t* __restrict__ cull_lo = ra.cull + (size_t)(gv >> 5) * (size_t)ra.cull_stride;
+	const bool cull_two = (gv & 31) + nv > 32;
 	uint32_t pend = 0;
 	for (int g = 0; g < p.G; g++)
 	{
@@ -891,57 +948,36 @@
 		if (i0 >= p.P) break;
 		const bool last_round = g == p.G - 1 || i0 + FR_THREADS >= p.P;
 		uint32_t np = 0;
-		const uint32_t skipv = (uint32_t)(skipm >> (g * nv)) & ((1u << nv) - 1u);
-		if (skipv != (1u << nv) - 1u)
 		{
 			const int i = i0 + tid;
-			const bool live = i < p.P;
-			fr_f3 pw = { 0.f, 0.f, 0.f };
-			float tr = 0.f;
-			if (live) { const float4 m4 = ra.mt[i]; pw = fr_f3{ m4.x, m4.y, m4.z }; tr = m4.w; }
-			uint32_t keepbits = 0;
+			unsigned long long cw = cull_lo[i];
+			if (cull_two) cw |= (unsigned long long)cull_lo[(size_t)ra.cull_stride + i] << 32;
+			const uint32_t keepbits = (uint32_t)(cw >> (gv & 31)) & ((1u << nv) - 1u);
 			for (int vv = 0; vv < nv; vv++)
 			{
-				if ((skipv >> vv) & 1u) { if (lane == 0) s_ca[vv * 4 + wave] = 0u; continue; }
-				const fr_f3 po = has_w2c ? fr_world_to_cam(pw, s_wm + 12 * vv) : pw;
-				const fr_f3 p_view = IDV ? po : fr_xform4x3(po, vm);
-				bool keep = live && !(p_view.z <= 0.001f);
-				if (early)
-				{
-#pragma clang fp contract(fast)
-					const float hx = __builtin_fmaf(pm[8], po.z, __builtin_fmaf(pm[4], po.y, __builtin_fmaf(pm[0], po.x, pm[12])));
-					const float hy = __builtin_fmaf(pm[9], po.z, __builtin_fmaf(pm[5], po.y, __builtin_fmaf(pm[1], po.x, pm[13])));
-					const float hw = __builtin_fmaf(pm[11], po.z, __builtin_fmaf(pm[7], po.y, __builtin_fmaf(pm[3], po.x, pm[15])));
-					const float p_w = __builtin_amdgcn_rcpf(hw + 0.0000001f);
-					const float px = ((hx * p_w + 1.0f) * (float)p.W - 1.0f) * 0.5f, py = ((hy * p_w + 1.0f) * (float)p.H - 1.0f) * 0.5f;
-					const float iz = __builtin_amdgcn_rcpf(p_view.z);
-					const float jx = fminf(fabsf(p_view.x * iz) * 1.001f, lx), jy = fminf(fabsf(p_view.y * iz) * 1.001f, ly);
-					const float kc = fx2 * (1.0f + jx * jx) + fy2 * (1.0f + jy * jy);
-					const float rb = 3.0f * __builtin_amdgcn_sqrtf(kc * tr * (iz * iz) + 0.7f) * 1.000001f + 2.0f;
-					const bool outside = (px + rb < 0.f) || (px - rb > xmax) || (py + rb < 0.f) || (py - rb > ymax);
-					keep = keep && !outside;
-				}
-				keepbits |= (keep ? 1u : 0u) << vv;
-				const unsigned long long m = __builtin_amdgcn_ballot_w64(keep);
+				const unsigned long long m = __builtin_amdgcn_ballot_w64((keepbits >> vv) & 1u);
 				if (lane == 0) s_ca[vv * 4 + wave] = (uint32_t)__popcll(m);
 			}
 			__syncthreads();
 			uint32_t cnt_l = lane < 4 * nv ? s_ca[lane] : 0u;
-			uint32_t inc = cnt_l;
-#pragma unroll
-			for (int d = 1; d < 64; d <<= 1)
-			{
-				const uint32_t y = (uint32_t)__shfl_up((int)inc, d, 64);
-				if (lane >= d) inc += y;
-			}
-			const uint32_t exc = inc - cnt_l;
-			np = (uint32_t)__builtin_amdgcn_readlane((int)inc, 63);
-			for (int vv = 0; vv < nv; vv++)
-			{
-				const bool keep = (keepbits >> vv) & 1u;
-				const unsigned long long m = __builtin_amdgcn_ballot_w64(keep);
-				const uint32_t base = (uint32_t)__builtin_amdgcn_readlane((int)exc, vv * 4 + wave);
-				if (keep) pairs[pend + base + (uint32_t)__popcll(m & lt)] = (uint32_t)(g * FR_THREADS + tid) | ((uint32_t)vv << 16);
+			if (__builtin_amdgcn_ballot_w64(cnt_l != 0u) != 0ull)
+			{
+				uint32_t inc = cnt_l;
+#pragma unroll
+				for (int d = 1; d < 64; d <<= 1)
+				{
+					const uint32_t y = (uint32_t)__shfl_up((int)inc, d, 64);
+					if (lane >= d) inc += y;
+				}
+				const uint32_t exc = inc - cnt_l;
+				np = (uint32_t)__builtin_amdgcn_readlane((int)inc, 63);
+				for (int vv = 0; vv < nv; vv++)
+				{
+					const bool keep = (keepbits >> vv) & 1u;
+					const unsigned long long m = __builtin_amdgcn_ballot_w64(keep);
+					const uint32_t base = (uint32_t)__builtin_amdgcn_readlane((int)exc, vv * 4 + wave);
+					if (keep) pairs[pend + base + (uint32_t)__popcll(m & lt)] = (uint32_t)(g * FR_THREADS + tid) | ((uint32_t)vv << 16);
+				}
 			}
 		}
 		__syncthreads();
@@ -6462,7 +6498,7 @@
 	~FrJoinGuard() { if (n) { char keep[sizeof(g_err)]; memcpy(keep, g_err, sizeof(keep)); (void)join(); memcpy(g_err, keep, sizeof(keep)); } }
 };
 
-struct FrScorerPlan { int columns; bool form_a; FrRecordArgs ra; bool skip_pack = false; bool general = false; bool pose = false; bool view_identity = false; bool render = false; bool point = false; };
+struct FrScorerPlan { int columns; bool form_a; FrRecordArgs ra; bool skip_pack = false; bool general = false; bool pose = false; bool view_identity = false; bool render = false; bool point = false; int cull_V = 0; const float* cull_w2c = nullptr; };
 template <int C> __global__ void k_pack_static(FrParams p, const float* __restrict__ H_inv, float* __restrict__ packed, float4* __restrict__ mt, float4* __restrict__ grp);
 template <int C, bool LIST, bool FORM_A> __global__ void k_fisher_records(FrParams p, FrRecordArgs ra);
 
@@ -6515,6 +6551,17 @@
 		FrRecordArgs ra = plan ? plan->ra : FrRecordArgs{ nullptr, 0, nullptr, nullptr, nullptr, nullptr, 0, nullptr, nullptr, 6 };
 		const bool dk = p.tile_cap != 0;
 		const size_t lds_c = lds_c_of(p.VC);
+		if (once && plan->cull_V >= 0)
+		{
+			if (!ra.cull || (size_t)ra.cull_stride != (size_t)gridP.x * per_block) return fr_fail(FR_EINVAL, "fr_bin_pipeline: the cull masks do not fit the front end's grid");
+			FrParams pc = p;
+			if (plan->cull_V > 0) { pc.V = plan->cull_V; pc.w2c = plan->cull_w2c; }
+			const dim3 gridC(gridP.x * p.G, (pc.V + 31) / 32);
+			const bool idv = plan->view_identity && plan->columns == 4 && dk && !plan->render && !plan->pose && !plan->general && !plan->form_a && !plan->point;
+			if (idv) hipLaunchKernelGGL((k_cull_views<true>), gridC, dim3(FR_THREADS), 0, s, pc, ra, ra.cull);
+			else hipLaunchKernelGGL((k_cull_views<false>), gridC, dim3(FR_THREADS), 0, s, pc, ra, ra.cull);
+			if ((rc = fr_check_launch("k_cull_views"))) return rc;
+		}
 		if (once && plan->render && dk) hipLaunchKernelGGL((k_preprocess_views_c<4, 4, true>), gridV, dim3(FR_THREADS), lds_c, s, p, ra);
 		else if (once && plan->render) hipLaunchKernelGGL((k_preprocess_views_c<4, 4, false>), gridV, dim3(FR_THREADS), lds_c, s, p, ra);
 		else if (once && plan->pose && dk) hipLaunchKernelGGL((k_preprocess_views_c<4, 3, true>), gridV, dim3(FR_THREADS), lds_c, s, p, ra);
@@ -7037,7 +7084,7 @@
 
 #define FR_MAX_GROUPS 4
 struct FrFisherLayout {
-	size_t radii, vis_n, splat, recq, slot_idx, packed, mt, grp, big_list, part_list, view_work, view_perm, blk_base, cov3D, tile_cnt, tile_off, tile_fill, tile_scores, w2c_inv, status, keys, fallback, seg_T, seg_C, seg_X, seg_list, total;
+	size_t radii, vis_n, splat, recq, slot_idx, packed, mt, grp, big_list, part_list, view_work, view_perm, blk_base, cov3D, tile_cnt, tile_off, tile_fill, tile_scores, w2c_inv, status, keys, fallback, seg_T, seg_C, seg_X, seg_list, cull, total;
 	size_t PV;
 };
 static FrFisherLayout fr_fisher_layout(int64_t P, int64_t W, int64_t H, int64_t V, int64_t max_rendered, int columns)
@@ -7076,6 +7123,7 @@
 	L.seg_X = o; o = fr_align(o + seg_tiles * FR_THREADS * 8);
 	L.seg_list = o; o = fr_align(o + (FR_SEG_PER_TILE * seg_tiles + 1) * 4);
 	L.part_list = o; o = fr_align(o + (size_t)(V * T) * FR_PART_MAXP * 8 + 64 * FR_MAX_GROUPS);
+	L.cull = o; o = fr_align(o + (size_t)((V + 31) / 32) * L.PV * 4);
 	L.total = o;
 	return L;
 }
@@ -7094,6 +7142,17 @@
 	if (P < 0 || W <= 0 || H <= 0 || n_views <= 0 || max_rendered < 0 || (columns != 4 && columns != 11) || !offset)
 		return fr_fail(FR_EINVAL, "fr_fisher_part_list_offset: bad argument");
 	*offset = fr_fisher_layout(P, W, H, n_views, max_rendered, columns).part_list;
+	return FR_OK;
+}
+
+extern "C" int fr_fisher_cull_mask_offset(int32_t P, int32_t W, int32_t H, int32_t n_views, int64_t max_rendered, int32_t columns, size_t* offset, int32_t* words_stride)
+{
+	if (P < 0 || W <= 0 || H <= 0 || n_views <= 0 || max_rendered < 0 || (columns != 4 && columns != 11) || !offset || !words_stride)
+		return fr_fail(FR_EINVAL, "fr_fisher_cull_mask_offset: bad argument");
+	const FrFisherLayout L = fr_fisher_layout(P, W, H, n_views, max_rendered, columns);
+	if (L.PV > 0x7fffffffull) return fr_fail(FR_EINVAL, "fr_fisher_cull_mask_offset: bad argument (too many Gaussians)");
+	*offset = L.cull;
+	*words_stride = (int32_t)L.PV;
 	return FR_OK;
 }
 
@@ -7319,6 +7378,7 @@
 	}
 	plan.ra.mt = (const float4*)(ws + L.mt);
 	plan.ra.grp = (const float4*)(ws + L.grp);
+	plan.ra.cull = (uint32_t*)(ws + L.cull); plan.ra.cull_stride = (int)L.PV; plan.ra.cull_v0 = 0;
 	plan.ra.early = (g->cov3D_precomp || f.debug_mode == 15) ? 0 : 1;
 	p.order = compact ? fc->order : nullptr;
 
@@ -7361,6 +7421,8 @@
 		pg.num_rendered = p.num_rendered ? p.num_rendered + v0 : nullptr;
 		FrScorerPlan pl = plan;
 		pl.skip_pack = gi > 0 || (fc->reuse_static != 0 && compact);
+		pl.ra.cull_v0 = v0;
+		pl.cull_V = gi == 0 ? V : -1; pl.cull_w2c = p.w2c;
 		if (pl.ra.hinv_stride) pl.ra.H_inv = plan.ra.H_inv + (size_t)v0 * plan.ra.hinv_stride;
 		pl.ra.recq = plan.ra.recq + (size_t)v0 * rec_view * 4;
 		if (pl.ra.comp) pl.ra.comp = plan.ra.comp + (size_t)v0 * L.PV * rstride;
@@ -7513,6 +7575,7 @@
 	plan.ra.slot_idx = nullptr;
 	plan.ra.mt = (const float4*)(ws + L.mt);
 	plan.ra.grp = (const float4*)(ws + L.grp);
+	plan.ra.cull = (uint32_t*)(ws + L.cull); plan.ra.cull_stride = (int)L.PV; plan.ra.cull_v0 = 0;
 	plan.ra.early = 1;
 	FrFisherArgs f;
 	memset(&f, 0, sizeof(f));
@@ -7648,6 +7711,7 @@
 		plan.ra.slot_idx = nullptr;
 		plan.ra.mt = (const float4*)(ws + L.mt);
 		plan.ra.grp = (const float4*)(ws + L.grp);
+		plan.ra.cull = (uint32_t*)(ws + L.cull); plan.ra.cull_stride = (int)L.PV; plan.ra.cull_v0 = 0;
 		plan.ra.early = 1;
 		if ((rc = fr_bin_pipeline(p, g, s, &plan))) return rc;
 		f.key_shift = p.tile_cap ? 4 : 0;
@@ -7773,6 +7837,7 @@
 	plan.ra.slot_acc = slot_acc;
 	plan.ra.mt = (const float4*)(ws + L.mt);
 	plan.ra.grp = (const float4*)(ws + L.grp);
+	plan.ra.cull = (uint32_t*)(ws + L.cull); plan.ra.cull_stride = (int)L.PV; plan.ra.cull_v0 = 0;
 	plan.ra.early = 1;
 	FrFisherArgs f;
 	memset(&f, 0, sizeof(f));
diff --git a/fisher-nerf-customized_amd/fisher_rast/_lib.py b/fisher-nerf-customized_amd/fisher_rast/_lib.py
--- a/fisher-nerf-customized_amd/fisher_rast/_lib.py
+++ b/fisher-nerf-customized_amd/fisher_rast/_lib.py
@@ -77,7 +77,7 @@
 
 
 EXPORTS = (
-    "fr_version", "fr_last_error", "fr_build_id", "fr_init", "fr_fisher_workspace_layout", "fr_fisher_part_list_offset", "fr_workspace_bytes", "fr_workspace_layout", "fr_mark_visible",
+    "fr_version", "fr_last_error", "fr_build_id", "fr_init", "fr_fisher_workspace_layout", "fr_fisher_part_list_offset", "fr_fisher_cull_mask_offset", "fr_workspace_bytes", "fr_workspace_layout", "fr_mark_visible",
     "fr_forward", "fr_backward", "fr_backward_scratch_bytes", "fr_backward_ws", "fr_forward_pair", "fr_forward_features", "fr_backward_pair", "fr_backward_pair_scratch_bytes", "fr_backward_pair_ws", "fr_fisher_workspace_bytes", "fr_fisher_views",
     "fr_fisher_pose_workspace_bytes", "fr_fisher_pose_workspace_layout", "fr_fisher_pose_views",
     "fr_render_views_workspace_bytes", "fr_render_views_workspace_layout", "fr_render_views",
@@ -135,6 +135,9 @@
     if hasattr(lib, "fr_fisher_part_list_offset"):
         lib.fr_fisher_part_list_offset.restype = ctypes.c_int
         lib.fr_fisher_part_list_offset.argtypes = lib.fr_fisher_workspace_layout.argtypes
+    if hasattr(lib, "fr_fisher_cull_mask_offset"):
+        lib.fr_fisher_cull_mask_offset.restype = ctypes.c_int
+        lib.fr_fisher_cull_mask_offset.argtypes = lib.fr_fisher_workspace_layout.argtypes + [ctypes.POINTER(ctypes.c_int32)]
     want = source_hash()
     got = lib.fr_build_id().decode().split(":")[-1]
     if "FISHER_RAST_SO" not in os.environ and want is not None and got != want:
diff --git a/include/fisher_rast.h b/include/fisher_rast.h
--- a/include/fisher_rast.h
+++ b/include/fisher_rast.h
@@ -131,6 +131,8 @@
 int fr_fisher_workspace_layout(int32_t P, int32_t W, int32_t H, int32_t n_views, int64_t max_rendered, int32_t columns,
                                size_t offsets[8]);
 int fr_fisher_part_list_offset(int32_t P, int32_t W, int32_t H, int32_t n_views, int64_t max_rendered, int32_t columns, size_t* offset);
+int fr_fisher_cull_mask_offset(int32_t P, int32_t W, int32_t H, int32_t n_views, int64_t max_rendered, int32_t columns, size_t* offset,
+                               int32_t* words_stride);
 
 int fr_fisher_views(const fr_raster_cfg* cfg, const fr_gaussians* g, const fr_fisher_cfg* cfg_f,
                     void* workspace, size_t workspace_bytes, int64_t max_rendered,
```

New measurement: 46670. -1.9%, worse.
